# tomasjakab/imm

Hardware: AMD Instinct MI355X
Metric: training images/sec at 128x128 K=10 (higher is better)
Workload: dtype bf16; 1 GPU; BASELINE configs[1] (N>1: configs[2]): CelebA-shape 128x128 K=10 IMM training step (fwd + VGG16 perceptual loss + bwd + clip + Adam), batch 32 per GPU; global_batch=32, image_size=128, n_maps=10, parallelism=dp1, hip_graph=True, weights=seeded random init; synthetic VGG16 (vgg16.caffemodel.h5 unavailable offline)

## Files before the change

### imm_amd/_lib.py

```python
import ctypes as C
import os

import torch

_HERE = os.path.dirname(os.path.abspath(__file__))
LIB_PATH = os.environ.get('IMM_HIP_LIB') or os.path.join(_HERE, 'libimm_hip.so')

IMM_BF16, IMM_F16, IMM_F32 = 0, 1, 2
CONV_BIAS, CONV_RELU, CONV_STATS, CONV_MASK, CONV_OUT_F32 = 1, 2, 4, 8, 16
SSE_BLOCKS = 512
OPTIMIZERS = {'adam': 0, 'adadelta': 1, 'adagrad': 2}
GAUSS_MODES = {'rot': 0, 'flat': 1, 'ankush': 2}
ABI_VERSION = 35


class ImmHipError(RuntimeError):
    pass


class ConvDesc(C.Structure):
    _fields_ = [(n, C.c_int32) for n in (
        'batch', 'hi', 'wi', 'ci', 'ldx', 'ho', 'wo', 'co', 'ldy', 'kh', 'kw', 'stride', 'pad_t', 'pad_l',
        'updiv', 'kpad', 'flags', 'ldmask', 'out_scale', 'out_off_y', 'out_off_x')]


class WgradJob(C.Structure):
    _fields_ = [('desc', ConvDesc), ('x', C.c_void_p), ('dy', C.c_void_p), ('slab', C.c_void_p), ('lddy', C.c_int32),
                ('nsplit', C.c_int32), ('x_scale', C.c_void_p), ('x_shift', C.c_void_p), ('x_relu', C.c_int32),
                ('reserved', C.c_int32)]


class OptHParams(C.Structure):
    _fields_ = [('lr_start', C.c_float), ('lr_decay', C.c_float), ('lr_step', C.c_int32), ('lr_multiple', C.c_float),
                ('beta1', C.c_float), ('beta2', C.c_float), ('eps', C.c_float), ('clip', C.c_float),
                ('grad_scale', C.c_float), ('optim', C.c_int32),
                ('scale_growth_interval', C.c_int32), ('scale_max', C.c_float)]


class KeypointDesc(C.Structure):
    _fields_ = [('w', C.c_void_p), ('b', C.c_void_p), ('geom', C.c_void_p), ('keypoints', C.c_void_p), ('m', C.c_int32),
                ('image_size', C.c_int32)]


_P, _I, _L, _F, _D = C.c_void_p, C.c_int, C.c_int64, C.c_float, C.c_double
ABI = {}


def _header(name, sigs):
    ABI[name] = {n: s if isinstance(s, tuple) else (C.c_int, s) for n, s in sigs.items()}


_header('imm_hip.h', {
    'imm_abi_version': [],
    'imm_last_error': (C.c_char_p, []),
    'imm_source_digest': (C.c_char_p, []),
    'imm_device_info': [_P],
    'imm_set_cu_limit': [_I],
    'imm_get_cu_limit': [],
    'imm_graph_begin': [_P],
    'imm_graph_end': [_P, C.POINTER(C.c_void_p)],
    'imm_graph_launch': [_P, _P],
    'imm_graph_destroy': [_P],
    'imm_pack_weights': [_P, _P, _I, _I, _I, _I, _I, _I, _I, _I, _I, _P],
    'imm_pack_weights_multi': [_P, _P, _I, _I, _I, _P],
    'imm_pack_weights_multi_blocks': [_I, _I, _I],
    'imm_wgrad_reduce_multi': [_P, _P, _I, _I, _P],
    'imm_conv2d': [C.POINTER(ConvDesc), _I, _P, _P, _P, _P, _P, _P, _P],
    'imm_conv_stats_blocks': [C.POINTER(ConvDesc)],
    'imm_conv2d_variant': [C.POINTER(ConvDesc), _I],
    'imm_conv2d_tap_supported': [C.POINTER(ConvDesc)],
    'imm_conv2d_tap': [C.POINTER(ConvDesc), _I, _P, _P, _P, _P, _P, _I, _P, _I, _P, _I, _I, _P],
    'imm_conv2d_wgrad': [C.POINTER(ConvDesc), _I, _P, _P, _I, _P, _I, _P],
    'imm_conv2d_wgrad_splits': [C.POINTER(ConvDesc), _I],
    'imm_conv2d_wgrad_variant': [C.POINTER(ConvDesc), _I, _I, C.POINTER(C.c_int), C.POINTER(C.c_int), C.POINTER(C.c_int)],
    'imm_conv2d_wgrad_multi_plan': [_P, _I, _I, _P],
    'imm_conv2d_wgrad_multi': [_P, _P, _P],
    'imm_conv2d_wgrad_reduce': [_P, _I, _I, _I, _I, _I, _I, _I, _P, _P],
    'imm_colsum': [_P, _I, _L, _I, _I, _I, _P, _P, _P],
    'imm_colsum_blocks': [_L, _I],
    'imm_bn_finalize': [_P, _I, _I, _L, _P, _P, _F, _F, _I, _P, _P, _P, _P, _P, _P, _P],
    'imm_bn_apply_relu': [_P, _I, _L, _I, _I, _P, _P, _I, _P, _I, _P],
    'imm_bn_apply_fused': [_P, _I, _I, _L, _P, _P, _F, _F, _I, _P, _P, _P, _P, _P, _P, _P, _I, _I, _I, _P, _I, _P, _I, _I, _I, _P],
    'imm_bn_bwd_apply_fused': [_P, _I, _I, _L, _P, _P, _I, _P, _I, _I, _P, _P, _P, _P, _I, _P, _P, _P, _I, _P],
    'imm_rows_reduce': [_P, _I, _I, _I, _P, _P],
    'imm_bn_bwd_reduce': [_P, _I, _P, _I, _I, _L, _I, _P, _P, _P, _P, _I, _P, _P],
    'imm_bn_bwd_blocks': [_L, _I],
    'imm_bn_bwd_reduce_up': [_P, _I, _P, _I, _P, _I, _I, _I, _I, _I, _I, _P, _P, _P, _P, _I, _P, _P],
    'imm_bn_bwd_finalize': [_P, _I, _I, _I, _L, _P, _P, _P, _I, _P, _P, _P, _P],
    'imm_bn_bwd_apply': [_P, _I, _P, _I, _I, _L, _I, _P, _P, _P, _P, _I, _P, _P, _I, _P],
    'imm_upsample2x_fwd': [_P, _P, _I, _I, _I, _I, _I, _I, _I, _P],
    'imm_upsample2x_bwd': [_P, _P, _I, _I, _I, _I, _I, _I, _I, _P],
    'imm_resize_ac_fwd': [_P, _P, _I, _I, _I, _I, _I, _I, _I, _I, _I, _P],
    'imm_resize_ac_bwd': [_P, _P, _I, _I, _I, _I, _I, _I, _I, _I, _I, _P],
    'imm_maxpool2_fwd': [_P, _P, _I, _I, _I, _I, _I, _P],
    'imm_maxpool2_bwd': [_P, _P, _P, _I, _I, _I, _I, _I, _I, _P],
    'imm_pack_image': [_P, _P, _I, _L, _P],
    'imm_pack_image_taps': [_P, _P, _I, _I, _I, _I, _I, _I, _I, _P],
    'imm_softargmax_gauss_fwd': [_P, _I, _I, _I, _I, _I, _F, _I, _P, _P, _P, _P, _I, _I, _I, _P],
    'imm_softargmax_gauss_bwd': [_P, _I, _I, _I, _I, _I, _I, _F, _I, _P, _P, _P, _P, _I, _I, _P],
    'imm_gauss_render_f32': [_P, _I, _I, _F, _I, _P, _I, _P],
    'imm_pose_head_fwd': [_P, _I, _I, _P, _I, _P, _I, _I, _I, _I, _I, _F, _I, _P, _I, _P, _P, _P, _P, _I, _I,
                          C.POINTER(KeypointDesc), _P],
    'imm_pose_head_bwd': [_P, _I, _I, _I, _I, _I, _I, _F, _I, _P, _P, _P, _P, _I, _I, _P, _I, _I, _P, _I, _P, _P],
    'imm_vgg_conv1_1_fwd': [_P, _P, _I, _I, _I, _P, _P, _P, _I, _I, _P],
    'imm_vgg_head_supported': [_I, _I, _I],
    'imm_vgg_head_fwd': [_P, _P, _I, _I, _I, _P, _P, _P, _I, _P, _P, _I, _P, _P, _I, _P],
    'imm_vgg_conv1_1_bwd': [_P, _I, _I, _I, _P, _P, _P, _I, _P, _P, _I, _I, _P, _I, _P],
    'imm_image_loss_grad': [_P, _P, _I, _I, _I, _P, _P, _I, _I, _P, _I, _I, _P],
    'imm_copy_f32': [_P, _P, _L, _P],
    'imm_debug_stamp': [_P, _I, _P],
    'imm_tps_warp': [_P, _I, _I, _I, _I, _I, _P, _I, _P, _P, _I, _P, _P, _I, _P],
    'imm_tps_warp_pad': [_P, _I, _I, _I, _I, _I, _I, _I, _I, _I, _I, _I, _I, _I, _P, _I, _P, _P, _I, _P],
    'imm_conv2d_group': [_P, _I, _I, _P, _P, _P, _P, _P, _P],
    'imm_conv_first_supported': [_I, _I, _I, _I],
    'imm_conv_first_stats_blocks': [_I, _I],
    'imm_conv_first': [_P, _P, _I, _P, _P, _I, _P, _I, _I, _I, _I, _I, _P],
    'imm_conv2d_nol_supported': [C.POINTER(ConvDesc)],
    'imm_conv2d_nol_stats_blocks': [C.POINTER(ConvDesc)],
    'imm_conv2d_nol': [C.POINTER(ConvDesc), _I, _P, _P, _P, _I, _P, _P, _P, _P, _P],
    'imm_conv2d_dgrad_s2_supported': [_I, _I, _I, _I, _I, _I],
    'imm_conv2d_dgrad_s2': [_P, _I, _P, _I, _P, _I, _I, _I, _I, _I, _I, _P],
    'imm_conv2d_group_stats_blocks': [_P, _I],
    'imm_upsample2x_bwd_bn': [_P, _P, _I, _I, _I, _I, _I, _I, _I, _P, _I, _P, _P],
    'imm_upsample2x_bwd_bn_blocks': [_I, _I, _I, _I],
    'imm_crc32c': [_P, C.c_uint64, C.POINTER(C.c_uint32)],
    'imm_rccl_unique_id': [_P],
    'imm_rccl_init': [_I, _I, _P, C.POINTER(C.c_void_p)],
    'imm_rccl_allreduce': [_P, _P, _L, _P],
    'imm_rccl_destroy': [_P],
    'imm_resize_crop_u8': [_P, _P, _P, _P, _I, _I, _I, _I, _I, _I, _I, _I, _P, _I, _P],
    'imm_unpool_tap_grad': [_P, _P, _P, _P, _I, _I, _I, _I, _P, _I, _P, _I, _P],
    'imm_masked_sse_pool': [_P, _P, _I, _I, _I, _I, _P, _I, _P, _P, _P, _P],
    'imm_masked_sse_multi': [_I, _P, _P, _P, _P, _P, _I, _I, _P, _I, _I, _P],
    'imm_masked_sse_all': [_I, _P, _P, _P, _P, _P, _I, _I, _P, _I, _I, _P, _I, _P, _I, _I, _P, _P],
    'imm_masked_sse': [_P, _P, _I, _I, _I, _I, _P, _I, _I, _P, _P],
    'imm_masked_sse_f32': [_P, _I, _P, _I, _I, _I, _I, _P, _I, _P, _P],
    'imm_perceptual_finalize': [_P, _I, _P, _P, _I, _P, _I, _I, _P, _P, _P],
    'imm_cost_ema': [_P, _P, _F, _P],
    'imm_rms16': [_P, _L, _I, _P, _I, _P, _P],
    'imm_tap_grad': [_P, _I, _P, _P, _I, _I, _I, _I, _P, _I, _P, _I, _I, _I, _P],
    'imm_weight_decay_loss': [_P, _P, _P, _P, _I, _P, _P, _P, _P],
    'imm_clip_adam_step': [_P, _P, _P, _P, _P, _P, _P, _I, _I, _P, _P, _P, _P, _P, _P, _P, C.POINTER(OptHParams), _P, _P],
    'imm_conv2d_workspace_bytes': (_L, [C.POINTER(ConvDesc)]),
    'imm_conv2d_group_workspace_bytes': (_L, [_P, _I]),
    'imm_conv2d_wgrad_workspace_bytes': (_L, [C.POINTER(ConvDesc), _I, _I]),
    'imm_conv2d_wgrad_multi_table_bytes': (_L, [_I]),
    'imm_colsum_workspace_bytes': (_L, [_L, _I]),
    'imm_bn_bwd_workspace_bytes': (_L, [_L, _I]),
    'imm_upsample2x_bwd_bn_workspace_bytes': (_L, [_I, _I, _I, _I]),
    'imm_masked_sse_workspace_bytes': (_L, [_I]),
    'imm_vgg_head_scratch_bytes': (_L, [_I, _I]),
})

_header('imm_align.h', {
    'imm_align_coeffs': [_P, _P, _I, _I, _I, _P, _P],
    'imm_align_warp_u8': [_P, _I, _P, _P, _I, _P, _P, _P, _P, _I, _I, _I, _I, _P, _I, _P],
})

_header('imm_compose.h', {
    'imm_compose_u8': [_P, _P, _P, _I, _P, _P, _P, _P, _I, _I, _I, _I, _P],
})

_header('imm_unalign.h', {
    'imm_unalign_maps': [_P, _P, _P, _P, _I, _I, _I, _I, _P, _P, _P],
    'imm_unalign_u8': [_P, _P, _P, _I, _P, _P, _P, _P, _F, _P, _I, _I, _I, _I, _P],
})

_header('imm_track.h', {
    'imm_track_step': [_P, _P, _P, _P, _I, _I, _I, _I, _I, _I, _D, _D, _D, _D, _D, _D, _I, _P, _P, _P, _P, _P, _P],
})

_header('imm_retarget.h', {
    'imm_retarget': [_P, _P, _P, _P, _P, _I, _I, _I, _I, _I, _D, _P, _P, _P],
})

_header('imm_warp.h', {
    'imm_warp_fit': [_P, _P, _P, _I, _I, _I, _D, _D, _P, _P, _P, _P],
    'imm_warp_u8': [_P, _P, _P, _P, _I, _P, _P, _P, _P, _P, _I, _I, _I, _P],
})

_header('imm_morph.h', {
    'imm_morph_poses': [_P, _P, _P, _I, _I, _P, _P, _P],
    'imm_morph_u8': [_P, _P, _P, _P, _I, _P, _P, _P, _I, _P, _P, _P, _P, _P, _P, _P, _P, _I, _I, _I, _P],
})

_header('imm_colour.h', {
    'imm_colour_stats_u8': [_P, _P, _P, _I, _P, _I, _I, _P, _P],
    'imm_colour_gain': [_P, _P, _P, _D, _I, _P, _P, _P],
    'imm_morph_colour_u8': [_P, _P, _P, _P, _I, _P, _P, _P, _I, _P, _P, _P, _P, _P, _P, _P, _P, _P, _I, _I, _I, _P],
})

_header('imm_hull.h', {
    'imm_hull_fit': [_P, _P, _P, _I, _I, _P, _P, _P],
    'imm_morph_hull_u8': [_P, _P, _P, _P, _I, _P, _P, _P, _I, _P, _P, _P, _P, _P, _P, _P, _P, _P, _P, _P, _I, _I, _I, _I, _P],
})

_header('imm_seam.h', {
    'imm_seam_fit': [_P, _P, _P, _P, _P, _P, _P, _P, _P, _I, _P, _P, _P, _I, _P, _P, _P, _P, _P, _P, _I, _I, _I, _I, _P, _P, _P, _P],
    'imm_morph_seam_u8': [_P, _P, _P, _P, _I, _P, _P, _P, _I, _P, _P, _P, _P, _P, _P, _P, _P, _P, _P, _P, _P, _P, _P, _I, _I, _I, _I, _I, _P],
})

_header('imm_clip.h', {
    'imm_clip_rows': [_P, _P, _P, _P, _I, _I, _I, _D, _P, _P, _P, _P, _P],
    'imm_clip_ema': [_P, _P, _P, _P, _P, _I, _I, _F, _P],
})

_lib = None


def symbols(header=None):
    return sorted(ABI[header]) if header else sorted(n for block in ABI.values() for n in block)


def signature(name):
    for block in ABI.values():
        if name in block:
            return block[name]
    raise KeyError(name)


def load():
    global _lib
    if _lib is not None:
        return _lib
    if not os.path.exists(LIB_PATH):
        raise ImmHipError('libimm_hip.so not found at %s: build it with `python imm_amd/build.py` '
                          '(there is no CPU fallback for the product path)' % LIB_PATH)
    if 'IMM_HIP_LIB' not in os.environ and os.path.isdir(os.path.join(_HERE, 'csrc')):
        from . import build as _b
        want, have = _b.source_digest(), _b.library_digest(LIB_PATH)
        if want != have:
            if not _b.have_compiler():
                raise ImmHipError('libimm_hip.so is stale (built from sources %s.., checkout is %s..) and hipcc is not '
                                  'available to rebuild it' % (have[:12] or '?', want[:12]))
            _b.build(verbose=False)
    lib = C.CDLL(LIB_PATH)
    for block in ABI.values():
        for name, (restype, argtypes) in block.items():
            fn = getattr(lib, name)
            fn.restype, fn.argtypes = restype, argtypes
    v = lib.imm_abi_version()
    if v != ABI_VERSION:
        raise ImmHipError('libimm_hip.so ABI %d != expected %d' % (v, ABI_VERSION))
    _lib = lib
    return lib


def call(name, *args):
    rc = getattr(load(), name)(*args)
    if rc != 0:
        raise ImmHipError('%s failed (%d): %s' % (name, rc, load().imm_last_error().decode()))
```

### imm_amd/csrc/conv_wgrad.hip

```cpp
#include "common.h"
#include "conv_dispatch.h"
#include "gfx950.h"
#include <stdlib.h>
#include <string.h>

struct WgradArgs {
  const uint16_t* x;
  const uint16_t* dy;
  float* slab;
  int P;
  int hi, wi, ci8, ldx;
  int ho, wo, co, lddy;
  int kh, kw, stride, pad_t, pad_l;
  int kpad, ntaps;
  int n_kblk, n_nblk, nsplit, p_per_split;
  uint32_t x_bytes, dy_bytes;
};

template <int PSUB>
__device__ __forceinline__ int wg_swz(int row) { return PSUB == 1 ? (((row >> 3) & 1) * 3) : (row & (4 * PSUB - 1)); }
template <int PSUB>
__device__ __forceinline__ int wg_dword_idx(int row, int u, int pp) {
  return row * (16 * PSUB) + (((u * 4 + (pp >> 2)) ^ wg_swz<PSUB>(row)) << 2) + (pp & 3);
}
// ... 130 lines not shown
          Bb[wg_dword_idx<PSUB>(row, u, pp)] = (lo[j] & 0xffffu) | (hi[j] << 16);
          Bb[wg_dword_idx<PSUB>(row + 1, u, pp)] = (lo[j] >> 16) | (hi[j] & 0xffff0000u);
        }
      }
    }
  };

  f32x4_t acc[KT_][NT];
#pragma unroll
  for (int i = 0; i < KT_; ++i)
#pragma unroll
    for (int j = 0; j < NT; ++j) acc[i][j] = f32x4_t{0.f, 0.f, 0.f, 0.f};

  const int nsteps = (p_end - p_begin + 32 * PSUB - 1) / (32 * PSUB);
  if (nsteps > 0) {
    load_tile();
    store_tile(0);
  }
  __syncthreads();
  const int frow = lane & 15, fchunk = lane >> 4;
  for (int st = 0; st < nsteps; ++st) {
    const int buf = st & 1;
    const bool more = (st + 1) < nsteps;
    if (more) load_tile();
    const uint4* Ab = smem + buf * BUF;
    const uint4* Bb = Ab + BK * 4 * PSUB;
#pragma unroll
    for (int u = 0; u < PSUB; ++u) {
      uint4 af[KT_], bf[NT];
#pragma unroll
      for (int i = 0; i < KT_; ++i) af[i] = Ab[wg_chunk_idx<PSUB>(wk * TK + i * 16 + frow, u * 4 + fchunk)];
#pragma unroll
      for (int j = 0; j < NT; ++j) bf[j] = Bb[wg_chunk_idx<PSUB>(wn * TN + j * 16 + frow, u * 4 + fchunk)];
#pragma unroll
      for (int i = 0; i < KT_; ++i)
#pragma unroll
        for (int j = 0; j < NT; ++j) acc[i][j] = ET::mfma(bf[j], af[i], acc[i][j]);
    }
    if (more) store_tile(buf ^ 1);
    __syncthreads();
  }

  float* out = a.slab + (int64_t)split * a.kpad * a.co;
#pragma unroll
  for (int i = 0; i < KT_; ++i) {
    const int kk = k0 + wk * TK + i * 16 + (lane & 15);
    if (kk >= a.kpad) continue;
#pragma unroll
    for (int j = 0; j < NT; ++j) {
      const int n = n0 + wn * TN + j * 16 + 4 * (lane >> 4);
      float* op = out + (int64_t)kk * a.co + n;
      if (n + 3 < a.co && (a.co & 3) == 0) {
        *(float4*)op = make_float4(acc[i][j][0], acc[i][j][1], acc[i][j][2], acc[i][j][3]);
      } else {
#pragma unroll
        for (int r = 0; r < 4; ++r) if (n + r < a.co) op[r] = acc[i][j][r];
      }
    }
  }
}

template <typename ET, int BK, int BN, int WGK, int WGN, bool FAST, int PSUB>
static void wg_launch_one(const WgradArgs& a, hipStream_t s) {
  constexpr int lds = 2 * (BK + BN) * 64 * PSUB;
  imm_launch<conv_wgrad_kernel<ET, BK, BN, WGK, WGN, FAST, PSUB>>(dim3(a.n_kblk * a.n_nblk * a.nsplit), dim3(256), lds, s, a);
}

template <typename ET, int BK, int BN, int WGK, int WGN>
static void wg_launch_cfg(const WgradArgs& a, bool fast, int psub, hipStream_t s) {
  if (fast && psub == 4) wg_launch_one<ET, BK, BN, WGK, WGN, true, 4>(a, s);
  else if (fast) wg_launch_one<ET, BK, BN, WGK, WGN, true, 1>(a, s);
  else wg_launch_one<ET, BK, BN, WGK, WGN, false, 1>(a, s);
}

static int wgrad_bn(int co) { return co > 64 ? 128 : co > 32 ? 64 : co > 16 ? 32 : 16; }

template <typename ET>
static int wgrad_launch(const imm_conv_desc* d, const void* x, const void* dy, int lddy, float* slab, int nsplit,
                        hipStream_t s) {
  WgradArgs a;
  a.x = (const uint16_t*)x; a.dy = (const uint16_t*)dy; a.slab = slab;
  a.P = d->batch * d->ho * d->wo;
  a.hi = d->hi; a.wi = d->wi; a.ci8 = d->ci / 8; a.ldx = d->ldx;
  a.ho = d->ho; a.wo = d->wo; a.co = d->co; a.lddy = lddy;
  a.kh = d->kh; a.kw = d->kw; a.stride = d->stride; a.pad_t = d->pad_t; a.pad_l = d->pad_l;
  a.kpad = d->kpad; a.ntaps = d->kh * d->kw;
  const int bn = wgrad_bn(d->co);
  a.n_kblk = (d->kpad + 127) / 128;
  a.n_nblk = (d->co + bn - 1) / bn;
  a.nsplit = nsplit;
  const int hw = d->ho * d->wo;
  const int64_t xb = (int64_t)d->batch * d->hi * d->wi * d->ldx * 2, db = (int64_t)a.P * lddy * 2;
  const bool fast = (hw % 32 == 0) && (d->wo % 32 == 0 || 32 % d->wo == 0) && xb < (1LL << 31) && db < (1LL << 31);
  constexpr int psub_env = 1;
  int pps = (a.P + nsplit - 1) / nsplit;
  const int psub = (fast && psub_env == 4 && a.P % 128 == 0 && pps >= 512 && bn <= 64) ? 4 : 1;
  pps = (pps + 32 * psub - 1) / (32 * psub) * (32 * psub);
  a.p_per_split = pps;
  a.x_bytes = (uint32_t)(fast ? xb : 0);
  a.dy_bytes = (uint32_t)(fast ? db : 0);
  if (bn == 128) wg_launch_cfg<ET, 128, 128, 2, 2>(a, fast, psub, s);
  else if (bn == 64) wg_launch_cfg<ET, 128, 64, 2, 2>(a, fast, psub, s);
  else if (bn == 32) wg_launch_cfg<ET, 128, 32, 4, 1>(a, fast, psub, s);
  else wg_launch_cfg<ET, 128, 16, 4, 1>(a, fast, psub, s);
  IMM_CHECK_LAUNCH("imm_conv2d_wgrad");
  return 0;
}

extern "C" int imm_conv2d_wgrad_splits(const imm_conv_desc* d, int lddy) {
  if (!d) return IMM_E_INVALID;
  return imm_wgrad_halo_applicable(d, lddy) ? imm_wgrad_halo_splits(d, lddy) : 0;
}

enum { WGM_SINGLE = 0, WGM_TR = 1, WGM_HALO = 2 };
static void wgm_classify(const imm_conv_desc* d, int lddy, int dtype, bool halo_ok, int* kind, int* variant) {
  const bool fast_dt = dtype == IMM_BF16 || dtype == IMM_F16;
  const int hv = fast_dt && halo_ok ? imm_wgrad_halo_variant(d, lddy) : 0;
  if (hv) { *kind = WGM_HALO; *variant = hv; return; }
  if (fast_dt && imm_wgrad_tr_applicable(d, lddy)) { *kind = WGM_TR; *variant = imm_wgrad_tr_variant(d); return; }
  *kind = WGM_SINGLE; *variant = 0;
}

extern "C" int imm_conv2d_wgrad(const imm_conv_desc* d, int dtype, const void* x, const void* dy, int lddy,
                                float* slab, int nsplit, void* stream) {
  IMM_REQUIRE(d && x && dy && slab, "wgrad: null");
  IMM_REQUIRE(d->ci > 0 && d->ci % 8 == 0 && d->ldx % 8 == 0 && d->ldx >= d->ci, "wgrad: ci/ldx must be multiples of 8");
  IMM_REQUIRE(lddy % 8 == 0 && lddy >= d->co, "wgrad: lddy=%d must be a multiple of 8 and >= co", lddy);
  IMM_REQUIRE(d->updiv == 1, "wgrad: desc must be the forward convolution");
  IMM_REQUIRE(d->kpad % 32 == 0 && d->kpad >= d->kh * d->kw * d->ci, "wgrad: kpad");
  IMM_REQUIRE(nsplit >= 1, "wgrad: nsplit");
  IMM_REQUIRE(d->wo % 2 == 0, "wgrad: output width must be even (pixel pairs)");
  IMM_REQUIRE(((uintptr_t)x % 16 == 0) && ((uintptr_t)dy % 16 == 0) && ((uintptr_t)slab % 16 == 0), "wgrad: alignment");
  if (dtype == IMM_F32) return imm_conv_f32_wgrad(d, x, dy, lddy, slab, nsplit, (hipStream_t)stream);
  int kind, variant;
  wgm_classify(d, lddy, dtype, nsplit == imm_conv2d_wgrad_splits(d, lddy), &kind, &variant);
  if (kind == WGM_HALO) {
    imm_wgrad_halo_launch(dtype, d, x, dy, lddy, slab, nsplit, (hipStream_t)stream, nullptr, nullptr, 0);
    IMM_CHECK_LAUNCH("imm_conv2d_wgrad(halo)");
    return 0;
  }
  if (kind == WGM_TR) {
    imm_wgrad_tr_launch(dtype, d, x, dy, lddy, slab, nsplit, (hipStream_t)stream);
    IMM_CHECK_LAUNCH("imm_conv2d_wgrad(tr)");
    return 0;
  }
  IMM_DISPATCH_DTYPE(dtype, return wgrad_launch<ET>(d, x, dy, lddy, slab, nsplit, (hipStream_t)stream));
  return 0;
}

namespace {
constexpr uint32_t WGM_MAGIC = 0x57474d31u;
constexpr int WGM_MAX_LAUNCH = 16, WGM_MAX_JOBS = 64, WGM_ARG_STRIDE = 192, WGM_HEADER = 1024;
struct WgmLaunch { int32_t kind, variant, n, arg_off, first_off, blocks, job0, pad; };
struct WgmHeader { uint32_t magic; int32_t dtype, n_jobs, n_launch; WgmLaunch launch[WGM_MAX_LAUNCH]; };
static_assert(sizeof(WgmHeader) <= WGM_HEADER, "header");

int wgm_check_job(const imm_wgrad_job* j) {
  const imm_conv_desc* d = &j->desc;
  IMM_REQUIRE(j->x && j->dy && j->slab, "wgrad_multi: null");
  IMM_REQUIRE(d->ci > 0 && d->ci % 8 == 0 && d->ldx % 8 == 0 && d->ldx >= d->ci, "wgrad_multi: ci/ldx must be multiples of 8");
  IMM_REQUIRE(j->lddy % 8 == 0 && j->lddy >= d->co, "wgrad_multi: lddy=%d must be a multiple of 8 and >= co", j->lddy);
  IMM_REQUIRE(d->updiv == 1 && d->kpad % 32 == 0 && d->kpad >= d->kh * d->kw * d->ci && j->nsplit >= 1 && d->wo % 2 == 0,
              "wgrad_multi: desc");
  IMM_REQUIRE(((uintptr_t)j->x % 16 == 0) && ((uintptr_t)j->dy % 16 == 0) && ((uintptr_t)j->slab % 16 == 0), "wgrad_multi: alignment");
  return 0;
}
}

extern "C" int64_t imm_conv2d_wgrad_multi_table_bytes(int n) {
  if (n < 1 || n > WGM_MAX_JOBS) return IMM_E_INVALID;
  return WGM_HEADER + (int64_t)n * (WGM_ARG_STRIDE + (int64_t)sizeof(imm_wgrad_job)) + WGM_MAX_LAUNCH * (WGM_MAX_JOBS + 1) * 4;
}

extern "C" int imm_conv2d_wgrad_variant(const imm_conv_desc* d, int lddy, int dtype, int* wg_per_split, int* units, int* wg_per_cu) {
  IMM_REQUIRE(d && lddy >= d->co, "wgrad_variant: args");
  int kind, variant;
  wgm_classify(d, lddy, dtype, true, &kind, &variant);
  int wps = 1, un = 1, pcu = 2;
  if (kind == WGM_HALO) {
    wps = imm_wgrad_halo_blocks(d, lddy, &un);
    pcu = imm_wgrad_halo_per_cu(variant);
  } else {
    const int bn = wgrad_bn(d->co);
    wps = ((d->kpad + 127) / 128) * ((d->co + bn - 1) / bn);
    un = (d->batch * d->ho * d->wo + 31) / 32;
  }
  if (wg_per_split) *wg_per_split = wps;
  if (units) *units = un;
  if (wg_per_cu) *wg_per_cu = pcu;
  return kind * 100000 + variant;
}

extern "C" int imm_conv2d_wgrad_multi_plan(const imm_wgrad_job* jobs, int n, int dtype, void* table_host) {
  IMM_REQUIRE(jobs && table_host && n >= 1 && n <= WGM_MAX_JOBS, "wgrad_multi_plan: args");
  IMM_REQUIRE(imm_wgrad_tr_args_bytes() <= WGM_ARG_STRIDE && imm_wgrad_halo_args_bytes() <= WGM_ARG_STRIDE, "wgrad_multi_plan: arg stride");
  char* base = (char*)table_host;
  memset(base, 0, (size_t)imm_conv2d_wgrad_multi_table_bytes(n));
  WgmHeader* h = (WgmHeader*)base;
  h->magic = WGM_MAGIC; h->dtype = dtype; h->n_jobs = n; h->n_launch = 0;
  int kind[WGM_MAX_JOBS], variant[WGM_MAX_JOBS];
  bool done[WGM_MAX_JOBS];
  for (int i = 0; i < n; ++i) {
    if (wgm_check_job(&jobs[i])) return IMM_E_INVALID;
    wgm_classify(&jobs[i].desc, jobs[i].lddy, dtype, true, &kind[i], &variant[i]);
    IMM_REQUIRE((jobs[i].x_scale == nullptr) == (jobs[i].x_shift == nullptr), "wgrad_multi_plan: job %d: x_scale / x_shift come together", i);
    IMM_REQUIRE(jobs[i].x_scale == nullptr || kind[i] == WGM_HALO,
                "wgrad_multi_plan: job %d: normalise-on-load (x_scale) is served by the LDS-halo filter-gradient kernels only "
                "(imm_conv2d_wgrad_variant / 100000 == 2)", i);
    done[i] = false;
  }
  int64_t off = WGM_HEADER;
  int job_slot = 0;
  for (int i = 0; i < n; ++i) {
    if (done[i]) continue;
    IMM_REQUIRE(h->n_launch < WGM_MAX_LAUNCH, "wgrad_multi_plan: more than %d kernel variants", WGM_MAX_LAUNCH);
    WgmLaunch* L = &h->launch[h->n_launch++];
    L->kind = kind[i]; L->variant = variant[i];
    int idx[WGM_MAX_JOBS], m = 0;
    for (int k = i; k < n; ++k)
      if (!done[k] && kind[k] == kind[i] && variant[k] == variant[i] && (kind[i] != WGM_SINGLE || k == i)) { idx[m++] = k; done[k] = true; }
    L->n = m;
    L->arg_off = (int32_t)off;
    if (kind[i] == WGM_SINGLE) {
      memcpy(base + off, &jobs[i], sizeof(imm_wgrad_job));
      off += (int64_t)sizeof(imm_wgrad_job);
      off = (off + 15) / 16 * 16;
      L->first_off = 0; L->blocks = 0; L->job0 = job_slot++;
      continue;
    }
    int steps[WGM_MAX_JOBS], blocks[WGM_MAX_JOBS];
    char tmp[WGM_MAX_JOBS][WGM_ARG_STRIDE];
    for (int k = 0; k < m; ++k) {
      const imm_wgrad_job* j = &jobs[idx[k]];
      blocks[k] = kind[i] == WGM_TR ? imm_wgrad_tr_fill(&j->desc, j->x, j->dy, j->lddy, j->slab, j->nsplit, tmp[k], &steps[k])
                                    : imm_wgrad_halo_fill(&j->desc, j->x, j->dy, j->lddy, j->slab, j->nsplit, tmp[k], &steps[k], j->x_scale,
                                                          j->x_shift, j->x_relu);
    }
    int order[WGM_MAX_JOBS];
    for (int k = 0; k < m; ++k) order[k] = k;
    for (int a = 1; a < m; ++a)
      for (int b = a; b > 0 && steps[order[b]] > steps[order[b - 1]]; --b) { const int t = order[b]; order[b] = order[b - 1]; order[b - 1] = t; }
    const int stride = kind[i] == WGM_TR ? imm_wgrad_tr_args_bytes() : imm_wgrad_halo_args_bytes();
    for (int k = 0; k < m; ++k) memcpy(base + off + (int64_t)k * stride, tmp[order[k]], (size_t)stride);
    off += (int64_t)m * stride;
    off = (off + 15) / 16 * 16;
    L->first_off = (int32_t)off;
    int32_t* first = (int32_t*)(base + off);
    first[0] = 0;
    for (int k = 0; k < m; ++k) first[k + 1] = first[k] + blocks[order[k]];
    L->blocks = first[m];
    off += (int64_t)(m + 1) * 4;
    off = (off + 15) / 16 * 16;
    L->job0 = job_slot; job_slot += m;
  }
  IMM_REQUIRE(off <= imm_conv2d_wgrad_multi_table_bytes(n), "wgrad_multi_plan: table overflow");
  return 0;
}

extern "C" int imm_conv2d_wgrad_multi(const void* table_host, const void* table_dev, void* stream) {
  IMM_REQUIRE(table_host && table_dev, "wgrad_multi: null");
  const char* hb = (const char*)table_host;
  const char* db = (const char*)table_dev;
  const WgmHeader* h = (const WgmHeader*)hb;
  IMM_REQUIRE(h->magic == WGM_MAGIC && h->n_launch >= 1 && h->n_launch <= WGM_MAX_LAUNCH, "wgrad_multi: not a planned table");
  for (int l = 0; l < h->n_launch; ++l) {
    const WgmLaunch* L = &h->launch[l];
    if (L->kind == WGM_SINGLE) {
      const imm_wgrad_job* j = (const imm_wgrad_job*)(hb + L->arg_off);
      const int rc = imm_conv2d_wgrad(&j->desc, h->dtype, j->x, j->dy, j->lddy, j->slab, j->nsplit, stream);
      if (rc) return rc;
    } else if (L->kind == WGM_TR) {
      imm_wgrad_tr_launch_multi(h->dtype, L->variant, db + L->arg_off, (const int*)(db + L->first_off), L->n, L->blocks, (hipStream_t)stream);
    } else {
      imm_wgrad_halo_launch_multi(h->dtype, L->variant, db + L->arg_off, (const int*)(db + L->first_off), L->n, L->blocks, (hipStream_t)stream);
    }
  }
  IMM_CHECK_LAUNCH("imm_conv2d_wgrad_multi");
  return 0;
}

__global__ void wgrad_reduce_kernel(const float* __restrict__ slab, int nsplit, int ntaps, int ci_pad, int ci_real,
                                    int co, int kpad, float* __restrict__ dw) {
  const int64_t total = (int64_t)ntaps * ci_real * co;
  const int64_t sstride = (int64_t)kpad * co;
  for (int64_t idx = (int64_t)blockIdx.x * blockDim.x + threadIdx.x; idx < total;
       idx += (int64_t)gridDim.x * blockDim.x) {
    const int n = (int)(idx % co);
    const int64_t tc = idx / co;
    const int c = (int)(tc % ci_real), tap = (int)(tc / ci_real);
    const float* sp = slab + ((int64_t)tap * ci_pad + c) * co + n;
    float acc = 0.f;
    for (int s = 0; s < nsplit; ++s) acc += sp[s * sstride];
    dw[idx] = acc;
  }
}

extern "C" int imm_conv2d_wgrad_reduce(const float* slab, int nsplit, int kh, int kw, int ci_pad, int ci_real, int co,
                                       int kpad, float* dw, void* stream) {
  IMM_REQUIRE(slab && dw && nsplit >= 1, "wgrad_reduce: args");
  IMM_REQUIRE(ci_real <= ci_pad && kpad >= kh * kw * ci_pad, "wgrad_reduce: padding");
  const int64_t total = (int64_t)kh * kw * ci_real * co;
  const int blocks = (int)((total + 255) / 256 > 2048 ? 2048 : (total + 255) / 256);
  hipLaunchKernelGGL(wgrad_reduce_kernel, dim3(blocks), dim3(256), 0, (hipStream_t)stream, slab, nsplit, kh * kw,
                     ci_pad, ci_real, co, kpad, dw);
  IMM_CHECK_LAUNCH("imm_conv2d_wgrad_reduce");
  return 0;
}
```

### imm_amd/csrc/loss_optim.hip

```cpp
#include "common.h"

#define LO_THREADS 256
#define IMM_NORM2_SANE 1e30f

template <typename ET>
__global__ __launch_bounds__(LO_THREADS) void masked_sse_kernel(const typename ET::T* __restrict__ a, const typename ET::T* __restrict__ b,
                                                                int batch, int s, int c8n, const float* __restrict__ mask,
                                                                int S, int l1, float* __restrict__ partial) {
  __shared__ float red[4];
  const int r = S / s;
  const int64_t total = (int64_t)batch * s * s * c8n;
  float acc = 0.f;
  for (int64_t idx = (int64_t)blockIdx.x * blockDim.x + threadIdx.x; idx < total;
       idx += (int64_t)gridDim.x * blockDim.x) {
    const int64_t p = idx / c8n;
    float mk = 1.f;
    if (mask) {
      const int xx = (int)(p % s);
      const int64_t t = p / s;
      const int yy = (int)(t % s);
      const int64_t bi = t / s;
      mk = mask[(bi * S + (int64_t)yy * r) * S + (int64_t)xx * r];
    }
    float fa[8], fb[8];
// ... 406 lines not shown
  IMM_DISPATCH_DTYPE_F32(dtype, hipLaunchKernelGGL((unpool_tap_grad_kernel<ET>), dim3((int)blocks), dim3(LO_THREADS), 0,
                                               (hipStream_t)stream, (typename ET::T*)da, (const typename ET::T*)dpool,
                                               (const typename ET::T*)a_pred, (const typename ET::T*)a_gt, batch, s, c / 8, mask, S, coef, idx));
  IMM_CHECK_LAUNCH("imm_unpool_tap_grad");
  return 0;
}

extern "C" int imm_tap_grad(void* da, int has_in, const void* a_pred, const void* a_gt, int dtype, int batch, int s, int c,
                            const float* mask, int S, const float* coef, int idx, int relu, int l1, void* stream) {
  IMM_REQUIRE(da && a_pred && a_gt && coef && batch > 0 && s > 0 && c > 0 && c % 8 == 0 && idx >= 0, "tap_grad: args");
  IMM_REQUIRE(mask == nullptr || (S >= s && S % s == 0), "tap_grad: mask side");
  const int64_t total = (int64_t)batch * s * s * (c / 8);
  int64_t blocks = (total + LO_THREADS - 1) / LO_THREADS;
  if (blocks > 16384) blocks = 16384;
  IMM_DISPATCH_DTYPE_F32(dtype, hipLaunchKernelGGL((tap_grad_kernel<ET>), dim3((int)blocks), dim3(LO_THREADS), 0,
                                               (hipStream_t)stream, (typename ET::T*)da, has_in, (const typename ET::T*)a_pred,
                                               (const typename ET::T*)a_gt, batch, s, c / 8, mask, S, coef, idx, relu, l1));
  IMM_CHECK_LAUNCH("imm_tap_grad");
  return 0;
}

template <typename ET>
__global__ void image_loss_grad_kernel(const float* __restrict__ gt, const float* __restrict__ pred, int ldp, int64_t npix,
                                       const float* __restrict__ mask, const float* __restrict__ coef, int idx, int l1,
                                       typename ET::T* __restrict__ dpred, int lddp) {
  const int nvec = lddp / 8;
  const float ck = coef[idx];
  for (int64_t i = (int64_t)blockIdx.x * blockDim.x + threadIdx.x; i < npix * nvec; i += (int64_t)gridDim.x * blockDim.x) {
    const int64_t p = i / nvec;
    const int cg = (int)(i - p * nvec);
    float o[8] = {0.f, 0.f, 0.f, 0.f, 0.f, 0.f, 0.f, 0.f};
    if (cg == 0) {
      const float cm = ck * (mask ? mask[p] : 1.f);
#pragma unroll
      for (int ch = 0; ch < 3; ++ch) {
        float d = pred[p * ldp + ch] - gt[p * 3 + ch];
        if (l1) d = d > 0.f ? 1.f : (d < 0.f ? -1.f : 0.f);
        o[ch] = cm * d;
      }
    }
    st8<ET>(dpred + p * lddp + cg * 8, pack8<ET>(o));
  }
}

extern "C" int imm_image_loss_grad(const float* gt, const float* pred, int ldp, int batch, int s, const float* mask,
                                   const float* coef, int idx, int l1, void* dpred, int lddp, int dtype, void* stream) {
  IMM_REQUIRE(gt && pred && coef && dpred && batch > 0 && s > 0 && ldp >= 3 && idx >= 0, "image_loss_grad: args");
  IMM_REQUIRE(lddp >= 8 && lddp % 8 == 0, "image_loss_grad: lddp=%d must be a multiple of 8", lddp);
  const int64_t npix = (int64_t)batch * s * s;
  int64_t blocks = (npix * (lddp / 8) + LO_THREADS - 1) / LO_THREADS;
  if (blocks > 8192) blocks = 8192;
  IMM_DISPATCH_DTYPE_F32(dtype, hipLaunchKernelGGL((image_loss_grad_kernel<ET>), dim3((int)blocks), dim3(LO_THREADS), 0,
                                               (hipStream_t)stream, gt, pred, ldp, npix, mask, coef, idx, l1,
                                               (typename ET::T*)dpred, lddp));
  IMM_CHECK_LAUNCH("imm_image_loss_grad");
  return 0;
}

__global__ __launch_bounds__(LO_THREADS) void wd_partial_kernel(const float* __restrict__ params,
                                                                const int32_t* __restrict__ blk_seg,
                                                                const int32_t* __restrict__ blk_begin,
                                                                const int32_t* __restrict__ blk_end,
                                                                const float* __restrict__ seg_wd,
                                                                float* __restrict__ blk_partial) {
  __shared__ float red[4];
  const int blk = blockIdx.x;
  const float wd = seg_wd[blk_seg[blk]];
  float acc = 0.f;
  if (wd != 0.f)
    for (int i = blk_begin[blk] + threadIdx.x; i < blk_end[blk]; i += LO_THREADS) { const float w = params[i]; acc += w * w; }
  acc = block_sum_256(acc, red);
  if (threadIdx.x == 0) blk_partial[blk] = 0.5f * wd * acc;
}

__global__ __launch_bounds__(LO_THREADS) void sum_partials_kernel(const float* __restrict__ partial, int n, float* out) {
  __shared__ double dred[LO_THREADS];
  double v = 0.0;
  for (int i = threadIdx.x; i < n; i += LO_THREADS) v += (double)partial[i];
  dred[threadIdx.x] = v;
  __syncthreads();
  for (int o = LO_THREADS / 2; o > 0; o >>= 1) {
    if (threadIdx.x < o) dred[threadIdx.x] += dred[threadIdx.x + o];
    __syncthreads();
  }
  if (threadIdx.x == 0) out[0] = (float)dred[0];
}

extern "C" int imm_weight_decay_loss(const float* params, const int32_t* blk_seg, const int32_t* blk_begin,
                                     const int32_t* blk_end, int nblk, const float* seg_wd, float* blk_partial, float* out,
                                     void* stream) {
  IMM_REQUIRE(params && blk_seg && blk_begin && blk_end && seg_wd && blk_partial && out && nblk > 0, "weight_decay_loss: args");
  hipLaunchKernelGGL(wd_partial_kernel, dim3(nblk), dim3(LO_THREADS), 0, (hipStream_t)stream, params, blk_seg, blk_begin,
                     blk_end, seg_wd, blk_partial);
  hipLaunchKernelGGL(sum_partials_kernel, dim3(1), dim3(LO_THREADS), 0, (hipStream_t)stream, blk_partial, nblk, out);
  IMM_CHECK_LAUNCH("imm_weight_decay_loss");
  return 0;
}

__global__ void cost_ema_kernel(const float* __restrict__ cost3, float* __restrict__ state, float decay) {
  if (threadIdx.x < 3) state[threadIdx.x] = decay * state[threadIdx.x] + (1.f - decay) * cost3[threadIdx.x];
  if (threadIdx.x == 3) state[3] += 1.f;
}

extern "C" int imm_cost_ema(const float* cost3, float* state4, float decay, void* stream) {
  IMM_REQUIRE(cost3 && state4 && decay >= 0.f && decay < 1.f, "cost_ema: args");
  hipLaunchKernelGGL(cost_ema_kernel, dim3(1), dim3(64), 0, (hipStream_t)stream, cost3, state4, decay);
  IMM_CHECK_LAUNCH("imm_cost_ema");
  return 0;
}

template <typename ET>
__global__ __launch_bounds__(LO_THREADS) void sumsq16_kernel(const typename ET::T* __restrict__ x, int64_t n8, float* __restrict__ partial) {
  __shared__ float red[4];
  float acc = 0.f;
  for (int64_t i = (int64_t)blockIdx.x * LO_THREADS + threadIdx.x; i < n8; i += (int64_t)gridDim.x * LO_THREADS) {
    float f[8];
    unpack8<ET>(ld8<ET>(x + i * 8), f);
#pragma unroll
    for (int e = 0; e < 8; ++e) acc = fmaf(f[e], f[e], acc);
  }
  acc = block_sum_256(acc, red);
  if (threadIdx.x == 0) partial[blockIdx.x] = acc;
}

__global__ __launch_bounds__(LO_THREADS) void rms_finish_kernel(const float* __restrict__ partial, int n, double count, float* out) {
  __shared__ double dred[LO_THREADS];
  double v = 0.0;
  for (int i = threadIdx.x; i < n; i += LO_THREADS) v += (double)partial[i];
  dred[threadIdx.x] = v;
  __syncthreads();
  for (int o = LO_THREADS / 2; o > 0; o >>= 1) {
    if (threadIdx.x < o) dred[threadIdx.x] += dred[threadIdx.x + o];
    __syncthreads();
  }
  if (threadIdx.x == 0) out[0] = (float)sqrt(dred[0] / count);
}

extern "C" int imm_rms16(const void* x, int64_t n, int dtype, float* partial, int nblk, float* out, void* stream) {
  IMM_REQUIRE(x && partial && out && n > 0 && n % 8 == 0 && nblk > 0 && nblk <= 4096, "rms16: args (n must be a multiple of 8)");
  IMM_REQUIRE(((uintptr_t)x % 16) == 0, "rms16: 16-byte alignment");
  IMM_DISPATCH_DTYPE_F32(dtype, hipLaunchKernelGGL((sumsq16_kernel<ET>), dim3(nblk), dim3(LO_THREADS), 0, (hipStream_t)stream,
                                              (const typename ET::T*)x, n / 8, partial));
  hipLaunchKernelGGL(rms_finish_kernel, dim3(1), dim3(LO_THREADS), 0, (hipStream_t)stream, partial, nblk, (double)n, out);
  IMM_CHECK_LAUNCH("imm_rms16");
  return 0;
}

__device__ __forceinline__ void opt_learning_rate(const imm_opt_hparams& hp, int gs, int tt, float* lr_t, float* lr) {
  const double l = (double)hp.lr_multiple * (double)hp.lr_start * pow((double)hp.lr_decay, (double)(gs / hp.lr_step));
  *lr_t = (float)(l * sqrt(1.0 - pow((double)hp.beta2, (double)tt)) / (1.0 - pow((double)hp.beta1, (double)tt)));
  *lr = (float)l;
}

__global__ __launch_bounds__(LO_THREADS) void grad_prepare_kernel(const float* __restrict__ params, float* __restrict__ grads,
                                                                  const int32_t* __restrict__ blk_seg,
                                                                  const int32_t* __restrict__ blk_begin,
                                                                  const int32_t* __restrict__ blk_end,
                                                                  const float* __restrict__ seg_wd, float grad_scale,
                                                                  const float* __restrict__ loss_scale,
                                                                  float* __restrict__ blk_partial, int nblk,
                                                                  const int32_t* __restrict__ step_count,
                                                                  const int32_t* __restrict__ adam_t, float* __restrict__ lr_state,
                                                                  imm_opt_hparams hp) {
  __shared__ float red[4];
  const int blk = blockIdx.x;
  if (blk == nblk) {
    if (threadIdx.x == 0) opt_learning_rate(hp, step_count[0], adam_t[0] + 1, lr_state, lr_state + 1);
    return;
  }
  if (loss_scale) grad_scale *= 1.f / loss_scale[0];
  const float wd = seg_wd[blk_seg[blk]];
  float acc = 0.f;
  const int b0 = blk_begin[blk], b1 = blk_end[blk];
  const int a0 = min((b0 + 3) & ~3, b1), a1 = max(a0, b1 & ~3);
  for (int i = b0 + threadIdx.x; i < a0; i += LO_THREADS) {
    const float g = grads[i] * grad_scale + wd * params[i];
    grads[i] = g; acc += g * g;
  }
  for (int i = a0 + 4 * threadIdx.x; i < a1; i += 4 * LO_THREADS) {
    float4 g = *(const float4*)(grads + i);
    const float4 w = *(const float4*)(params + i);
    g.x = g.x * grad_scale + wd * w.x; g.y = g.y * grad_scale + wd * w.y;
    g.z = g.z * grad_scale + wd * w.z; g.w = g.w * grad_scale + wd * w.w;
    *(float4*)(grads + i) = g;
    acc += (g.x * g.x + g.y * g.y) + (g.z * g.z + g.w * g.w);
  }
  for (int i = a1 + threadIdx.x; i < b1; i += LO_THREADS) {
    const float g = grads[i] * grad_scale + wd * params[i];
    grads[i] = g; acc += g * g;
  }
  acc = block_sum_256(acc, red);
  if (threadIdx.x == 0) blk_partial[blk] = acc;
}

__global__ __launch_bounds__(LO_THREADS) void clip_adam_kernel(float* __restrict__ params, const float* __restrict__ grads,
                                                               float* __restrict__ m, float* __restrict__ v,
                                                               const int32_t* __restrict__ blk_seg,
                                                               const int32_t* __restrict__ blk_begin,
                                                               const int32_t* __restrict__ blk_end,
                                                               const int32_t* __restrict__ seg_first_blk,
                                                               const float* __restrict__ blk_partial, int nblk,
                                                               float* __restrict__ seg_norm2, int32_t* __restrict__ step_count,
                                                               int32_t* __restrict__ adam_t, const float* __restrict__ lr_state,
                                                               float* __restrict__ ls, imm_opt_hparams hp) {
  __shared__ double dred[LO_THREADS / 64];
  const int blk = blockIdx.x, tid = threadIdx.x;
  const bool extra = blk == nblk;
  const int seg = extra ? 0 : blk_seg[blk];
  const int b0 = extra ? 0 : blk_begin[blk], b1 = extra ? 0 : blk_end[blk];
  const int a0 = min((b0 + 3) & ~3, b1), a1 = max(a0, b1 & ~3);
  const int i0 = a0 + 4 * tid;
  const bool first = i0 < a1;
  float4 g0 = {0.f, 0.f, 0.f, 0.f}, m0 = g0, v0 = g0, w0 = g0;
  if (first) { g0 = *(const float4*)(grads + i0); m0 = *(const float4*)(m + i0); v0 = *(const float4*)(v + i0); w0 = *(const float4*)(params + i0); }

  const int f0 = seg_first_blk[seg], f1 = seg_first_blk[seg + 1];
  double ps = 0.0;
  int bad = 0;
  const int sb1 = ls != nullptr ? nblk : f1;
  int sb0 = tid;
  if (ls == nullptr && f0 > tid) sb0 = tid + (f0 - tid + LO_THREADS - 1) / LO_THREADS * LO_THREADS;
  for (int b = sb0; b < sb1; b += LO_THREADS) {
    const float p = blk_partial[b];
    bad |= !(p <= IMM_NORM2_SANE);
    if (b >= f0 && b < f1) ps += (double)p;
  }
#pragma unroll
  for (int o = 32; o > 0; o >>= 1) ps += __shfl_xor(ps, o, 64);
  if ((tid & 63) == 0) dred[tid >> 6] = ps;
  bad = __syncthreads_or(bad);
  const bool skip = ls != nullptr && bad != 0;
  double t = 0.0;
#pragma unroll
  for (int w = 0; w < LO_THREADS / 64; ++w) t += dred[w];
  const float norm2 = (float)t;
  if (tid == 0 && !extra && blk == f0) seg_norm2[seg] = norm2;
  if (extra) {
    if (tid == 0) {
      if (ls) {
        float S = ls[0], clean = ls[1];
        if (skip) { S = fmaxf(S * 0.5f, 1.f); clean = 0.f; ls[2] += 1.f; }
        else if (hp.scale_growth_interval > 0 && clean + 1.f >= (float)hp.scale_growth_interval) {
          S = fminf(S * 2.f, hp.scale_max > 0.f ? hp.scale_max : S * 2.f); clean = 0.f;
        } else clean += 1.f;
        ls[0] = S; ls[1] = clean; ls[3] = skip ? 1.f : 0.f;
      }
      if (!skip) {
        step_count[0] += 1;
        adam_t[0] += 1;
      }
    }
    return;
  }
  if (skip) return;
  float factor = 1.f;
  if (hp.clip > 0.f) factor = hp.clip / fmaxf(sqrtf(norm2), hp.clip);
  const float lr_t = lr_state[0], lr = lr_state[1];
  auto one = [&](float g, float& mi, float& vi, float& w) {
    g *= factor;
    if (hp.optim == IMM_OPT_ADAM) {
      mi = hp.beta1 * mi + (1.f - hp.beta1) * g;
      vi = hp.beta2 * vi + (1.f - hp.beta2) * g * g;
      w -= lr_t * mi / (sqrtf(vi) + hp.eps);
    } else if (hp.optim == IMM_OPT_ADADELTA) {
      vi = hp.beta1 * vi + (1.f - hp.beta1) * g * g;
      const float u = sqrtf(mi + hp.eps) / sqrtf(vi + hp.eps) * g;
      mi = hp.beta1 * mi + (1.f - hp.beta1) * u * u;
      w -= lr * u;
    } else {
      vi += g * g;
      w -= lr * g / sqrtf(vi);
    }
  };
  for (int i = b0 + tid; i < a0; i += LO_THREADS) one(grads[i], m[i], v[i], params[i]);
  if (first) {
    one(g0.x, m0.x, v0.x, w0.x); one(g0.y, m0.y, v0.y, w0.y); one(g0.z, m0.z, v0.z, w0.z); one(g0.w, m0.w, v0.w, w0.w);
    *(float4*)(m + i0) = m0; *(float4*)(v + i0) = v0; *(float4*)(params + i0) = w0;
  }
  for (int i = i0 + 4 * LO_THREADS; i < a1; i += 4 * LO_THREADS) {
    const float4 g = *(const float4*)(grads + i);
    float4 mi = *(const float4*)(m + i), vi = *(const float4*)(v + i), w = *(const float4*)(params + i);
    one(g.x, mi.x, vi.x, w.x); one(g.y, mi.y, vi.y, w.y); one(g.z, mi.z, vi.z, w.z); one(g.w, mi.w, vi.w, w.w);
    *(float4*)(m + i) = mi; *(float4*)(v + i) = vi; *(float4*)(params + i) = w;
  }
  for (int i = a1 + tid; i < b1; i += LO_THREADS) one(grads[i], m[i], v[i], params[i]);
}

extern "C" int imm_clip_adam_step(float* params, float* grads, float* m, float* v, const int32_t* blk_seg,
                                  const int32_t* blk_begin, const int32_t* blk_end, int nblk, int nseg,
                                  const int32_t* seg_first_blk, const float* seg_wd, float* blk_partial, float* seg_norm2,
                                  int32_t* step_count, int32_t* adam_t, float* lr_state, const imm_opt_hparams* hp,
                                  float* loss_scale_state, void* stream) {
  IMM_REQUIRE(params && grads && m && v && blk_seg && blk_begin && blk_end && seg_first_blk && seg_wd && blk_partial &&
                  seg_norm2 && step_count && adam_t && lr_state && hp, "clip_adam_step: null");
  IMM_REQUIRE(nblk > 0 && nseg > 0 && hp->lr_step > 0, "clip_adam_step: dims");
  IMM_REQUIRE(hp->optim >= IMM_OPT_ADAM && hp->optim <= IMM_OPT_ADAGRAD, "clip_adam_step: optim %d", hp->optim);
  hipStream_t s = (hipStream_t)stream;
  hipLaunchKernelGGL(grad_prepare_kernel, dim3(nblk + 1), dim3(LO_THREADS), 0, s, params, grads, blk_seg, blk_begin, blk_end,
                     seg_wd, hp->grad_scale, loss_scale_state, blk_partial, nblk, step_count, adam_t, lr_state, *hp);
  hipLaunchKernelGGL(clip_adam_kernel, dim3(nblk + 1), dim3(LO_THREADS), 0, s, params, grads, m, v, blk_seg, blk_begin, blk_end,
                     seg_first_blk, blk_partial, nblk, seg_norm2, step_count, adam_t, lr_state, loss_scale_state, *hp);
  IMM_CHECK_LAUNCH("imm_clip_adam_step");
  return 0;
}
```

### imm_amd/engine.py

```python
import math
import os
from collections import OrderedDict

import numpy as np
import torch

from . import _lib as L
from . import ops

BN_EPS = 1e-3
BN_MOMENTUM = 0.99
BN_DIRECT_ROWS = int(os.environ.get('IMM_BN_DIRECT_ROWS', '512'))
WEIGHT_DECAY = 1e-5
INIT_STD = 0.01
PERCEPTUAL_WS = [100.0, 1.6, 2.3, 1.8, 2.8, 100.0]
SUPPORTED_COMP = ['input', 'conv1_2', 'conv2_2', 'conv3_2', 'conv4_2', 'conv5_2']
VGG_LAYERS = [('conv1_1', 1, 64), ('conv1_2', 64, 64), ('conv2_1', 64, 128), ('conv2_2', 128, 128),
              ('conv3_1', 128, 256), ('conv3_2', 256, 256), ('conv3_3', 256, 256),
              ('conv4_1', 256, 512), ('conv4_2', 512, 512), ('conv4_3', 512, 512),
              ('conv5_1', 512, 512), ('conv5_2', 512, 512)]
VGG_POOL_AFTER = ('conv1_2', 'conv2_2', 'conv3_3', 'conv4_3')
WGRAD_MULTI_MAX_JOBS, WGRAD_MULTI_MAX_VARIANTS = 64, 16


def plan_wgrad_chunks(groups, max_jobs, max_slots):
    chunks, cur, cur_jobs, cur_slots = [], [], 0, 0
    for gk, members in groups.items():
        generic = gk[0] // 100000 == 0
        members = list(members)
        while members:
            room_jobs, room_slots = max_jobs - cur_jobs, max_slots - cur_slots
            take = min(len(members), room_jobs, room_slots) if generic else (min(len(members), room_jobs) if room_slots >= 1 else 0)
            if take <= 0:
                chunks.append(cur); cur, cur_jobs, cur_slots = [], 0, 0
                continue
            part, members = members[:take], members[take:]
            cur.append((gk, part)); cur_jobs += len(part); cur_slots += len(part) if generic else 1
    if cur:
        chunks.append(cur)
    return chunks
COST_EMA_STATE = 'summaries/cost_movavg'
VGG_TAPS = {'conv1_2': 1, 'conv2_2': 2, 'conv3_2': 3, 'conv4_2': 4, 'conv5_2': 5}


def encoder_spec(n_filters):
    f = n_filters
    return [(7, 3, f, 1), (3, f, f, 1), (3, f, 2 * f, 2), (3, 2 * f, 2 * f, 1), (3, 2 * f, 4 * f, 2),
            (3, 4 * f, 4 * f, 1), (3, 4 * f, 8 * f, 2), (3, 8 * f, 8 * f, 1)]


def renderer_spec(cfg, image_size, n_out):
    filters = cfg.n_filters_render * 8
    cin = cfg.n_filters * 8 + cfg.n_maps
    size, spec = 16, []
    while size <= image_size:
        spec.append((3, cin, filters, True, False))
        if size == image_size:
            spec.append((3, filters, n_out, False, False))
            break
        spec.append((3, filters, filters, True, True))
        cin = filters
        size *= 2
        if filters >= 8:
            filters //= 2
    return spec


def render_sizes(cfg, max_size):
    sizes, size = [], max_size
    while True:
        sizes.append(size)
        if size <= cfg.min_res:
            break
        size = size // cfg.renderer_stride
    return sizes


def n_renderer_out(cfg):
    extra = len(cfg.perceptual.comp) if getattr(cfg, 'channels_bug_fix', False) else 0
    return 3 + extra


def trainable_spec(cfg, image_size):
    out = []

    def add(scope, k, cin, cout, bn):
        out.append((scope + '/w', (k, k, cin, cout), WEIGHT_DECAY))
        out.append((scope + '/b', (cout,), 0.0))
        if bn:
            out.append((scope + '/gamma', (cout,), 0.0))
            out.append((scope + '/beta', (cout,), 0.0))

    for enc in ('image_encoder', 'pose_encoder'):
        for i, (k, ci, co, _s) in enumerate(encoder_spec(cfg.n_filters)):
            add('model/%s/encoder/conv_%d' % (enc, i + 1), k, ci, co, True)
        if enc == 'pose_encoder':
            add('model/pose_encoder/conv_1', 1, cfg.n_filters * 8, cfg.n_maps, False)
    for i, (k, ci, co, bn, _u) in enumerate(renderer_spec(cfg, image_size, n_renderer_out(cfg))):
        add('model/renderer/conv_%d' % (i + 1), k, ci, co, bn)
    return out


def truncated_normal(rng, shape, std):
    z = rng.standard_normal(shape)
    bad = np.abs(z) > 2.0
    while bad.any():
        z[bad] = rng.standard_normal(int(bad.sum()))
        bad = np.abs(z) > 2.0
    return (z * std).astype(np.float32)


def synthetic_vgg_weights(seed=2):
    rng = np.random.default_rng(seed)
    w = OrderedDict()
    for name, cin, cout in VGG_LAYERS:
        w['vgg16/%s/weights' % name] = torch.from_numpy(
            (rng.standard_normal((3, 3, cin, cout)) * math.sqrt(2.0 / (9 * cin))).astype(np.float32))
        w['vgg16/%s/biases' % name] = torch.from_numpy((rng.standard_normal(cout) * 0.1).astype(np.float32))
    return w


class _Launch:
    __slots__ = ('fn', 'tag', 'flops', 'bytes', 'name', 'lane', 'variant', 'cus', 'group')

    def __init__(self, fn, tag, flops=0.0, nbytes=0.0, name='', lane=0, variant='', cus=0, group=''):
        self.fn, self.tag, self.flops, self.bytes, self.name, self.lane, self.variant = fn, tag, flops, nbytes, name, lane, variant
        self.cus, self.group = cus, group


class _ConvLayer:
    pass


class IMMEngine:
    def __init__(self, cfg, batch, image_size, device='cuda:0', act_dtype=torch.bfloat16, seed=1, vgg_weights=None,
                 hparams=None, world_size=1, dp_buckets=None):
        if cfg.gauss_mode not in L.GAUSS_MODES:
            raise ValueError('Unknown mode: ' + str(cfg.gauss_mode))
        if cfg.reconstruction_loss not in ('perceptual', 'l2'):
            raise ValueError('Reconsutruction loss-type: ' + str(cfg.reconstruction_loss) + ' not understood')
        self.loss_kind = cfg.reconstruction_loss
        self.comp = list(cfg.perceptual.comp) if self.loss_kind == 'perceptual' else ['input']
        if self.loss_kind == 'perceptual':
            if not self.comp or len(set(self.comp)) != len(self.comp) or len(self.comp) > len(PERCEPTUAL_WS):
                raise ValueError('perceptual.comp must name 1..%d distinct features, got %r' % (len(PERCEPTUAL_WS), self.comp))
            if any(n not in SUPPORTED_COMP for n in self.comp):
                raise NotImplementedError('perceptual.comp entries must come from %r (the layers the shipped configs tap), got %r'
                                          % (SUPPORTED_COMP, self.comp))
        self.l1 = self.loss_kind == 'perceptual' and not cfg.perceptual.l2
        if image_size % 16 or image_size < 64:
            raise ValueError('image side must be a multiple of 16 and >= 64')
        L.load()
        self.cfg, self.B, self.S, self.dev, self.dt = cfg, int(batch), int(image_size), torch.device(device), act_dtype
        self.f32 = act_dtype == torch.float32
        self.K = int(cfg.n_maps)
        self.world_size = world_size
        self.dp_buckets = int(dp_buckets if dp_buckets is not None else os.environ.get('IMM_DP_BUCKETS', '1'))
        self.use_mask = bool(cfg.loss_mask)
        self.n_cu, self.arch = ops.device_info()
        self._alloc_bytes = 0

        self.spec = trainable_spec(cfg, self.S)
        sizes = [int(np.prod(s)) for _n, s, _w in self.spec]
        self.tab = ops.SegmentTable(sizes, [w for _n, _s, w in self.spec], self.dev)
        self.params = self._zeros(self.tab.total)
        self.grads = self._zeros(self.tab.total)
        self.adam_m = self._zeros(self.tab.total)
        self.adam_v = self._zeros(self.tab.total)
        self.pview, self.gview = OrderedDict(), OrderedDict()
        for i, (name, shape, _wd) in enumerate(self.spec):
            o0, o1 = self.tab.offsets[i], self.tab.offsets[i + 1]
            self.pview[name] = self.params[o0:o1].view(shape)
            self.gview[name] = self.grads[o0:o1].view(shape)
        self.opt_blk_partial = self._zeros(self.tab.nblk)
        self.seg_norm2 = self._zeros(self.tab.nseg)
# ... 246 lines not shown
        if needs_dgrad:
            assert kw == k
            lddy = ldy if not out_f32 else ops.round_up(co, 32)
            lay.lddy = lddy
            lay.dd = None
            rows_d = ops.round_up(ci_real, 128)
            lay.s2 = ops.dgrad_s2_class_descs(B, H, W, ci_real, 0, lddy, lddy, k) if stride == 2 else None
            lay.s2_fused = (lay.s2 is not None and k == 3 and lddy % 64 == 0 and ci_real % 8 == 0 and not self.f32 and
                            ops.conv2d_dgrad_s2_supported(B, fd.ho, fd.wo, lddy, ci_real, ci_real))
            if lay.s2 is not None and not lay.s2_fused:
                lay.wt_s2 = []
                for dd, mode in lay.s2:
                    wt_c = self._zeros(rows_d, dd.kpad, dtype=dt)
                    lay.wt_s2.append(wt_c)
                    self._pack_jobs.append(((w.data_ptr(), wt_c.data_ptr(), mode, k, k, ci_real, co, lddy, rows_d, dd.kpad),
                                            rows_d * dd.kpad))
                lay.wt_d = None
            else:
                kpad_d = ops.round_up(k * k * lddy, 32)
                lay.wt_d = self._zeros(rows_d, kpad_d, dtype=dt)
                self._pack_jobs.append(((w.data_ptr(), lay.wt_d.data_ptr(), 1, k, k, ci_real, co, lddy, rows_d, kpad_d),
                                        rows_d * kpad_d))
        else:
            lay.lddy = ldy if not out_f32 else ops.round_up(co, 32)
        if bn:
            lay.coef = self._zeros(3, co)
            lay.dy = self._act(B, fd.ho, fd.wo, ldy)
        else:
            lay.cs_partial = self._zeros(ops.colsum_blocks(npix, lay.lddy), lay.lddy)
        return lay

    def _conv_backward(self, lay, d_out, ldd, dx, lddx, up_src=None):
        B, co, k = self.B, lay.co, lay.k
        npix = lay.npix
        scope = lay.scope
        self._cur_scope = scope
        gw, gb = self.gview[scope + '/w'], self.gview[scope + '/b']
        if lay.bn:
            gg, gbeta = self.gview[scope + '/gamma'], self.gview[scope + '/beta']
            gamma, beta = self.pview[scope + '/gamma'], self.pview[scope + '/beta']
            nblk = ops.bn_bwd_blocks(npix, co)
            lay.bwd_partial = self._zeros(nblk, 2, co)
            if up_src is not None:
                self._add(self.prog_bwd, lambda: ops.bn_bwd_reduce_up(up_src[0], up_src[1], d_out, ldd, lay.y, lay.ldy, B, lay.Ho, lay.Wo,
                                                                      co, lay.scale, lay.shift, lay.mean, lay.rstd, lay.relu,
                                                                      lay.bwd_partial), 'bn_bwd_reduce', 0.0, npix * co * 12.0)
            else:
                self._add(self.prog_bwd, lambda: ops.bn_bwd_reduce(d_out, ldd, lay.y, lay.ldy, npix, co, lay.scale, lay.shift,
                                                                   lay.mean, lay.rstd, lay.relu, lay.bwd_partial),
                          'bn_bwd_reduce', 0.0, npix * co * 4.0)
            if co % 32 == 0:
                rows, nrows = lay.bwd_partial, nblk
                if nblk > BN_DIRECT_ROWS:
                    g = max(32, -(-nblk // 32))
                    nrows = -(-nblk // g)
                    lay.bwd_red = rows_red = self._zeros(nrows, 2, co)
                    self._add(self.prog_bwd, lambda: ops.rows_reduce(lay.bwd_partial, nblk, 2 * co, g, rows_red), 'bn_bwd_finalize')
                    rows = rows_red
                self._add(self.prog_bwd, lambda: ops.bn_bwd_apply_fused(rows, nrows, co, npix, gamma, d_out, ldd,
                                                                        lay.y, lay.ldy, lay.scale, lay.shift, lay.mean, lay.rstd,
                                                                        lay.relu, gg, gbeta, lay.dy, lay.ldy),
                          'bn_bwd_apply', 0.0, npix * co * 6.0)
            else:
                self._add(self.prog_bwd, lambda: ops.bn_bwd_finalize(lay.bwd_partial, nblk, co, npix, gamma, beta, lay.rstd,
                                                                     gg, gbeta, lay.coef), 'bn_bwd_finalize')
                self._add(self.prog_bwd, lambda: ops.bn_bwd_apply(d_out, ldd, lay.y, lay.ldy, npix, co, lay.scale, lay.shift,
                                                                  lay.mean, lay.rstd, lay.relu, lay.coef, lay.dy, lay.ldy),
                          'bn_bwd_apply', 0.0, npix * co * 6.0)
            dy, lddy = lay.dy, lay.ldy
        else:
            dy, lddy = d_out, ldd
            self._colsum_pending.append((scope, lambda: ops.colsum(dy, npix, lddy, co, lddy, lay.cs_partial, gb)))
        fd = lay.fd
        flops = 2.0 * npix * k * lay.kw * lay.ci_real * co
        self._wgrad_pending.append((lay, dy, lddy, flops))
        if lay.needs_dgrad and dx is not None and getattr(lay, 's2_fused', False):
            assert lddx % 8 == 0 and lddx >= lay.ci_real, (lddx, lay.ci_real)
            self._add(self.prog_bwd, lambda: ops.conv2d_dgrad_s2(dy, lddy, lay.wt_d, dx, lddx, lay.ci_real, B, lay.Ho, lay.Wo),
                      'conv_dgrad', flops, 2.0 * (npix * lddy + 4 * npix * lay.ci_real + 9 * lddy * lay.ci_real), variant='s2d')
        elif lay.needs_dgrad and dx is not None and getattr(lay, 's2', None) is not None:
            classes = ops.dgrad_s2_class_descs(B, lay.H, lay.W, lay.ci_real, lddx, lddy, lddy, k)
            grp = ops.ConvGroup([dd0 for dd0, _m in classes], list(lay.wt_s2))
            ntaps = sum(dd0.kh * dd0.kw for dd0, _m in classes)
            self._add(self.prog_bwd, (lambda grp=grp: ops.conv2d_group(grp, dy, dx, None, None)), 'conv_dgrad',
                      2.0 * npix * ntaps * lay.ci_real * co,
                      2.0 * (4 * npix * lddy + 4 * npix * lay.ci_real + sum(dd0.kpad for dd0, _m in classes) * lay.ci_real), variant='group')
        elif lay.needs_dgrad and dx is not None:
            co_dx = lay.ci_pad if (lay.ci_pad != lay.ci_real and lay.ci_pad % 64 == 0 and lddx >= lay.ci_pad
                                   and lay.wt_d.shape[0] >= lay.ci_pad) else lay.ci_real
            dd = ops.dgrad_desc(B, lay.H, lay.W, co_dx, lddx, lddy, lddy, k, lay.stride, 0)
            assert dd.kpad == lay.wt_d.shape[1], (dd.kpad, lay.wt_d.shape)
            self._add(self.prog_bwd, lambda: ops.conv2d(dd, dy, lay.wt_d, None, dx), 'conv_dgrad', flops,
                      2.0 * (npix * lddy + B * lay.H * lay.W * lay.ci_real + dd.kpad * lay.ci_real), desc=dd)

    def _flush_wgrads(self, name, cus=0):
        jobs, self._wgrad_pending = self._wgrad_pending, []
        if not jobs:
            return
        groups = OrderedDict()
        for lay, dy, lddy, flops in jobs:
            key, wps, units, pcu = ops.conv2d_wgrad_variant(lay.fd, lddy, self.dt)
            groups.setdefault((key, pcu), []).append((lay, dy, lddy, wps, units, flops))
        chunks = plan_wgrad_chunks(groups, WGRAD_MULTI_MAX_JOBS, WGRAD_MULTI_MAX_VARIANTS)
        for ci_, chunk in enumerate(chunks):
            self._issue_wgrad_chunk(chunk, name if len(chunks) == 1 else '%s [%d/%d]' % (name, ci_ + 1, len(chunks)), cus)

    def _issue_wgrad_chunk(self, chunk, name, cus=0):
        n_lanes = int(os.environ.get('IMM_WG_LANES', '1'))
        if n_lanes > 1 and len(chunk) > 1 and not cus and self._cur_lane == 0:
            share = float(os.environ.get('IMM_WG_LANE_SHARE', '1.0'))
            groups = sorted(chunk, key=lambda g: -sum(m[5] for m in g[1]))
            lanes = sorted(set(1 + (i - 1) % (n_lanes - 1) for i in range(1, len(groups))))
            for ln in lanes:
                self._mark(self.prog_bwd, 'fork', lane=ln)
            for i, g in enumerate(groups):
                self._cur_lane = 0 if i == 0 else 1 + (i - 1) % (n_lanes - 1)
                self._issue_wgrad_chunk([g], '%s [variant %d]' % (name, g[0][0]),
                                        cus=0 if i == 0 else max(8, int(self.n_cu * share) // 8 * 8) if share < 1.0 else 0)
            self._cur_lane = 0
            for ln in lanes:
                self._mark(self.prog_bwd, 'join', lane=ln)
            return
        multi_jobs, flops_total = [], 0.0
        for (key, pcu), members in chunk:
            kind = key // 100000
            target = pcu * (cus or self.n_cu)
            floor_units = [16 if kind != 2 else (2 if wps > 1 else 4) for _l, _d, _ld, wps, _u, _f in members]

            def splits(u):
                return [max(1, min(-(-units // u), max(1, units // fl))) for (_l, _d, _ld, _w, units, _f), fl in zip(members, floor_units)]
            if kind == 0:
                ns = [max(1, min(-(-target // wps), max(1, units // 16))) for _l, _d, _ld, wps, units, _f in members]
            else:
                u = max(units for _l, _d, _ld, _w, units, _f in members)
                ns = splits(u)
                while u > 1:
                    u2 = max(1, int(u / 1.05)) if u > 64 else u - 1
                    ns2 = splits(u2)
                    if sum(n * m[3] for n, m in zip(ns2, members)) > target:
                        break
                    u, ns = u2, ns2
            for (lay, dy, lddy, wps, units, flops), nsplit in zip(members, ns):
                lay.nsplit = nsplit
                flops_total += flops
                lay.slab = self._zeros(nsplit, lay.fd.kpad, lay.co)
                ns_ = getattr(lay, 'nol_src', None)
                multi_jobs.append((lay.fd, lay.x, dy, lddy, lay.slab, nsplit,
                                   None if ns_ is None else (ns_.scale, ns_.shift, ns_.relu)))
                gw = self.gview[lay.scope + '/w']
                job = (lay.slab.data_ptr(), gw.data_ptr(), nsplit, lay.k * lay.kw, lay.ci_pad, lay.ci_real, lay.co, lay.fd.kpad)
                self._reduce_jobs.append((job, lay.k * lay.kw * lay.ci_real * lay.co))
        multi = ops.WgradMulti(multi_jobs, self.dt)
        self._wgrad_multis = getattr(self, '_wgrad_multis', []) + [multi]
        self._cur_scope = name
        self._add(self.prog_bwd, lambda: ops.conv2d_wgrad_multi(multi), 'conv_wgrad', flops_total, name=name)

    def _build_network(self):
        cfg, B, S, K, dt = self.cfg, self.B, self.S, self.K, self.dt
        nf = cfg.n_filters
        self.in_image = self._zeros(B, S, S, 3)
        self.in_future = self._zeros(B, S, S, 3)
        self.in_mask = self._zeros(B, S, S) if self.use_mask else None
        sizes = render_sizes(cfg, S)
        s16 = sizes[-1]
        if s16 != 16:
            raise NotImplementedError('renderer starts at 16x16 (min_res 16, renderer_stride 2): got %d' % s16)
        He = S // 8
        Cj = ops.round_up(8 * nf + K, 64)
        self.Cj, self.He = Cj, He
        self.joint = self._act(B, 16, 16, Cj)
        self.d_joint = self._act(B, 16, 16, Cj)

        def build_encoder(scope, src):
            k1 = encoder_spec(nf)[0][0]
            ld1 = ops.round_up(3 * k1, 32)
            xin = self._act(B, S, S, ld1)
            f_pack = (lambda: ops.pack_image_taps(src, xin, B, S, S, k1, (k1 - 1) // 2, ld1), 'pack_image',
                      0.0, B * S * S * (12.0 + 2.0 * ld1), scope + '/pack')
            co1 = encoder_spec(nf)[0][2]
            direct = (os.environ.get('IMM_CONV_FIRST', '0') != '0' and not self.f32 and k1 == 7 and ld1 == 32 and
                      ops.conv_first_supported(B, S, co1, ops.round_up(co1, 8)))
            if direct:
                self._deferred_packs.append(f_pack)
            else:
                self._add(self.prog_fwd, f_pack[0], f_pack[1], f_pack[2], f_pack[3], name=f_pack[4])
            layers, x, H, ci_real, ci_pad, ldx = [], xin, S, 3 * k1, ld1, ld1
            spec = encoder_spec(nf)
            hs, h_ = [], S
            for (_k, _ci, _co, st) in spec:
                hs.append(h_); h_ = -(-h_ // st)
            defer = [i + 1 < len(spec) and self._nol_consumer_ok(hs[i + 1], hs[i + 1], spec[i][2], ops.round_up(spec[i][2], 8),
                                                               spec[i + 1][2], spec[i + 1][0], spec[i + 1][3], True, False)
                     for i in range(len(spec))]
            prev = None
            for i, (k, ci, co, stride) in enumerate(spec):
                last = i == len(spec) - 1
                out, ldo = (None, None)
                if last and scope == 'model/image_encoder' and He == 16:
                    out, ldo = self.joint, Cj
                nol_src = prev if (prev is not None and getattr(prev, 'nol', False)) else None
                lay = self._conv_block('%s/encoder/conv_%d' % (scope, i + 1), x, H, H, ci_real, ci_pad, ldx, co, k,
                                       stride, True, True, needs_dgrad=(i > 0), out=out, ldo=ldo, kw=(1 if i == 0 else None),
                                       nol_src=nol_src, defer_apply=defer[i], first_src=(src if (i == 0 and direct) else None))
                layers.append(lay)
                prev = lay
                if lay.nol:
                    x, H, ci_real, ci_pad, ldx = lay.y, lay.Ho, co, co, lay.ldy
                else:
                    x, H, ci_real, ci_pad, ldx = lay.out, lay.Ho, co, co, lay.ldo
            return layers

        self._deferred_packs = []
        self._mark(self.prog_fwd, 'fork')
        self._cur_lane = 1
        self._add(self.prog_fwd, lambda: ops.weight_decay_loss(self.params, self.tab, self.opt_blk_partial, self.wd_loss),
                  'wd_loss', name='loss/weight_decay')
        self.enc_im = build_encoder('model/image_encoder', self.in_image)
        if He != 16:
            e = self.enc_im[-1]
            self._add(self.prog_fwd, lambda: ops.resize_ac_fwd(e.out, self.joint, B, He, He, 16, 16, 8 * nf, e.ldo, Cj),
                      'resize_ac')
        self._cur_lane = 0
        self.enc_pose = build_encoder('model/pose_encoder', self.in_future)
        pe = self.enc_pose[-1]
        lddy_h = ops.round_up(K, 32)
        self.fused_head = (not self.f32 and (8 * nf) % 32 == 0 and K <= 64 and (He * He) % 16 == 0 and lddy_h in (32, 64) and
                           4 * (He * He * K + 2 * He * K + 2 * K) <= 158 * 1024 and
                           4 * ((2 + 2 * He) * K + 516) + He * He * lddy_h * 2 <= 158 * 1024)
        self.pose_head = self._conv_block('model/pose_encoder/conv_1', pe.out, He, He, 8 * nf, 8 * nf, pe.ldo, K, 1, 1,
                                          False, False, needs_dgrad=True, out_f32=True, fwd_launch=not self.fused_head)
        ph = self.pose_head
        assert ph.lddy == lddy_h
        self.heat, self.ldh = ph.y, ph.ldy
        self.mu = self._zeros(B, K, 2)
        self.py = self._zeros(B, He, K)
        self.px = self._zeros(B, He, K)
        self.inv_std = 1.0 / float(cfg.gauss_std)
        gview = self.joint[..., 8 * nf:]
        if self.fused_head:
            bias_h = self.pview['model/pose_encoder/conv_1/b']
            self._add(self.prog_fwd, lambda: ops.pose_head_fwd(pe.out, pe.ldo, 8 * nf, ph.wt, bias_h, B, He, He, K, self.inv_std, 16,
                                                               self.heat, self.ldh, self.mu, self.py, self.px, gview, Cj, dt,
                                                               cfg.gauss_mode), 'bottleneck', ph.fwd_flops)
        else:
            self._add(self.prog_fwd, lambda: ops.softargmax_gauss_fwd(self.heat, self.ldh, B, He, He, K, self.inv_std, 16,
                                                                      self.mu, self.py, self.px, gview, Cj, dt, cfg.gauss_mode), 'bottleneck')

        if self._deferred_packs:
            self._cur_lane = 1
            for fn, tag, fl, nb, nm in self._deferred_packs:
                self._cur_scope = nm
                self._add(self.prog_fwd, fn, tag, fl, nb, name=nm)
            self._cur_lane = 0
        self._mark(self.prog_fwd, 'join')
        self.ren, self.ren_up = [], []
        x, H, ci_real, ci_pad, ldx = self.joint, 16, 8 * nf + K, Cj, Cj
        rspec = renderer_spec(cfg, S, n_renderer_out(cfg))
        prev = None
        for i, (k, ci, co, bn, up) in enumerate(rspec):
            assert ci == ci_real, (ci, ci_real)
            defer = False
            if bn and not up and i + 1 < len(rspec) and co % 8 == 0:
                k2, _ci2, co2, bn2, _up2 = rspec[i + 1]
                defer = self._nol_consumer_ok(H, H, co, co, co2, k2, 1, bn2, not bn2)
            nol_src = prev if (prev is not None and prev.bn and getattr(prev, 'nol', False)) else None
            lay = self._conv_block('model/renderer/conv_%d' % (i + 1), x, H, H, ci_real, ci_pad, ldx, co, k, 1, bn, bn,
                                   needs_dgrad=True, out_f32=not bn, up2x=bool(up and bn), nol_src=nol_src, defer_apply=defer)
            self.ren.append(lay)
            prev = lay
            if lay.bn and lay.nol:
                x, ci_real, ci_pad, ldx = lay.y, co, co, lay.ldy
            else:
                x, ci_real, ci_pad, ldx = lay.out, co, co, (lay.ldo if lay.out is not None else co)
            if up:
                ub = getattr(lay, 'up', None)
                if ub is None:
                    ub = self._act(B, 2 * H, 2 * H, co)
                    src = lay.out
                    assert src is not None, 'up-sampling pass without a stored normalised tensor'

                    self._add(self.prog_fwd, (lambda src=src, ub=ub, H=H, co=co: ops.upsample2x_fwd(src, ub, B, H, H, co, co, co)),
                              'upsample', 0.0, B * H * H * co * 10.0)
                self.ren_up.append((len(self.ren) - 1, ub, H, co))
                x, H = ub, 2 * H
        self.pred = self.ren[-1].y
        self.ldp = self.ren[-1].ldy

        self.n_fwd_model = len(self.prog_fwd)

        self.vgg_act, self.vgg_wt, self.vgg_wtd, self.vgg_desc = OrderedDict(), {}, {}, {}
        self.vgg_pool = {}
        self.tap_idx = {n: k for k, n in enumerate(self.comp)}
        vnames = [n for n, _ci, _co in VGG_LAYERS]
        taps = [n for n in self.comp if n != 'input'] if self.loss_kind == 'perceptual' else []
        self.vgg_layers = VGG_LAYERS[:max(vnames.index(n) for n in taps) + 1] if taps else []
        nfeat = self.nfeat
        self.sse_partial = self._zeros(nfeat, L.SSE_BLOCKS)
        fuse_ok = not self.l1
        fused_sse = set()
        self._sse_input_early = ('input' in self.tap_idx and bool(self.vgg_layers) and
                                 os.environ.get('IMM_SSE_INPUT_LANE', '0') != '0')
        if self._sse_input_early:
            idx0 = self.tap_idx['input']
            self._cur_scope = 'loss'
            self._mark(self.prog_fwd, 'fork', lane=1)
            self._cur_lane = 1
            self._add(self.prog_fwd, lambda: ops.masked_sse_f32(self.in_future, 3, self.pred, self.ldp, B, S, 3, self.in_mask,
                                                                self.sse_partial[idx0], self.l1), 'sse')
            self._cur_lane = 0
        split = bool(self.vgg_layers) and os.environ.get('IMM_VGG_SPLIT', '0') != '0'
        self.vgg_split = split
        self.gt_cus = int(os.environ.get('IMM_GT_CUS', '128')) if split else 0
        halves = ([('gt', slice(0, B), 2, self.gt_cus), ('pred', slice(B, 2 * B), 0, 0)] if split else
                  [('', slice(0, 2 * B), 0, 0)])
        gt_prog = []
        for hname, hs, lane, cus in halves:
            if not self.vgg_layers:
                break
            prog = gt_prog if hname == 'gt' else self.prog_fwd
            self._cur_lane, self._cur_cus, self._cur_group = lane, cus, ('gt' if hname == 'gt' else '')
            sfx = ' [%s]' % hname if hname else ''
            nb = hs.stop - hs.start
            if hname != 'pred':
                self.w11 = self._zeros(9, 64); self.b11 = self._zeros(64)
                a = self._act(2 * B, S, S, 64)
                self.vgg_act['conv1_1'] = (a, S)
            a = self.vgg_act['conv1_1'][0]
            hv = {'': 3, 'gt': 1, 'pred': 2}[hname]
            head_fused = (not split and len(self.vgg_layers) > 1 and not self.f32 and os.environ.get('IMM_VGG_HEAD', '1') != '0'
                          and ops.vgg_head_supported(B, S, dt))
            self.vgg_head_fused = head_fused
            if head_fused:
                self.vgg_gray = torch.empty(ops.vgg_head_scratch_bytes(B, S), dtype=torch.uint8, device=self.dev)
            else:
                self._add(prog, (lambda a=a, hv=hv: ops.vgg_conv1_1_fwd(self.in_future, self.pred, self.ldp, B, S, self.w11, self.b11, a, hv)),
                          'vgg_conv1_1', 2.0 * nb * S * S * 9 * 64, nb * S * S * 128.0, name='vgg16/conv1_1' + sfx)
            x, H = a, S
            for li, (name, cin, cout) in enumerate(self.vgg_layers[1:], start=1):
                fd = ops.fwd_desc(nb, H, H, cin, cin, cout, cout, 3, 1, L.CONV_BIAS | L.CONV_RELU)
                if hname != 'pred':
                    wt = self._zeros(ops.round_up(cout, 128), fd.kpad, dtype=dt)
                    wtd = self._zeros(ops.round_up(cin, 128), ops.round_up(9 * cout, 32), dtype=dt)
                    y = self._act(2 * B, H, H, cout)
                    self.vgg_wt[name], self.vgg_wtd[name], self.vgg_desc[name] = wt, wtd, fd
                    self.vgg_act[name] = (y, H)
                wt, y = self.vgg_wt[name], self.vgg_act[name][0]
                bias = self.vgg_w['vgg16/%s/biases' % name]
                if li == 1 and head_fused:
                    self._add(prog, (lambda a=a, wt=wt, bias=bias, y=y: ops.vgg_head_fwd(
                        self.in_future, self.pred, self.ldp, B, S, self.w11, self.b11, wt, bias, a, B, y, self.vgg_gray)),
                              'vgg_fwd', 2.0 * nb * S * S * 9 * (64 + cin * cout),
                              nb * S * S * 12.0 + 2.0 * (B * S * S * 64 + nb * S * S * cout + 9 * cin * cout),
                              name='vgg16/conv1_1+' + name, variant='vgg_head')
                else:
                    self._add(prog, (lambda fd=fd, x=x, wt=wt, bias=bias, y=y, hs=hs: ops.conv2d(fd, x[hs], wt, bias, y[hs])),
                              'vgg_fwd', 2.0 * nb * H * H * 9 * cin * cout, 2.0 * (nb * H * H * (cin + cout) + 9 * cin * cout),
                              name='vgg16/' + name + sfx, desc=fd)
                if hname == 'gt' and name in taps:
                    self._signal(prog, 'gt:' + name)
                x = y
                if name in VGG_POOL_AFTER and li < len(self.vgg_layers) - 1:
                    if hname != 'pred':
                        self.vgg_pool[name] = self._act(2 * B, H // 2, H // 2, cout)
                    p = self.vgg_pool[name]
                    if name in taps and fuse_ok and hname != 'gt':
                        idx = self.tap_idx[name]
                        fused_sse.add(name)
                        if hname == 'pred':
                            self._wait(prog, 'gt:' + name, lane=0)
                        pa = None if hname == 'pred' else p[:B]
                        self._add(prog, (lambda x=x, p=p, pa=pa, H=H, cout=cout, idx=idx: ops.masked_sse_pool(
                            x[:B], x[B:], B, H, cout, self.in_mask, S, self.sse_partial[idx], pa, p[B:])), 'sse',
                                  0.0, 2 * B * H * H * cout * 2.5, name='vgg16/%s+pool' % name)
                    else:
                        self._add(prog, (lambda x=x, p=p, H=H, cout=cout, hs=hs, nb=nb: ops.maxpool2_fwd(x[hs], p[hs], nb, H, H, cout)),
                                  'maxpool', 0.0, nb * H * H * cout * 2.5, name='vgg16/pool_' + name + sfx)
                    x, H = p, H // 2
        self._cur_lane, self._cur_cus, self._cur_group = 0, 0, ''
        if gt_prog:
            self._cur_group = 'gt'
            head = []
            self._mark(head, 'fork', lane=2)
            self._cur_group = ''
            self.prog_fwd[0:0] = head + gt_prog
            self.n_fwd_model += len(head) + len(gt_prog)
        if self.vgg_layers:
            self._pack_vgg()

        nel = []
        for name in self.comp:
            if name == 'input':
                nel.append(float(B * S * S * 3))
            else:
                y, H = self.vgg_act[name]
                nel.append(float(B * H * H * y.shape[-1]))
        self.nel = torch.tensor(nel, dtype=torch.float32, device=self.dev)
        self.loss_out = self._zeros(3 * nfeat + 3)
        self.cost_ema = self._zeros(4)
        mask = self.in_mask
        l1 = self.l1
        self._cur_scope = 'loss'
        if self._sse_input_early:
            self._mark(self.prog_fwd, 'join', lane=1)
        tail = [name for name in taps if name not in fused_sse]
        sse_all = ('input' in self.tap_idx and not self._sse_input_early and len(tail) > 1 and
                   os.environ.get('IMM_SSE_ALL', '1') != '0')
        if 'input' in self.tap_idx and not self._sse_input_early and not sse_all:
            idx0 = self.tap_idx['input']
            self._add(self.prog_fwd, lambda: ops.masked_sse_f32(self.in_future, 3, self.pred, self.ldp, B, S, 3, mask,
                                                                self.sse_partial[idx0], l1), 'sse')
        if self.vgg_split:
            self._cur_group = 'gt'
            self._mark(self.prog_fwd, 'join', lane=2)
            self._cur_group = ''
        if len(tail) > 1:
            feats = []
            for name in tail:
                y, H = self.vgg_act[name]
                feats.append((y[:B], y[B:], H, y.shape[-1], self.sse_partial[self.tap_idx[name]]))
            self.sse_multi = ops.SseMulti(feats)
            if sse_all:
                idx0 = self.tap_idx['input']
                self._add(self.prog_fwd, lambda: ops.masked_sse_all(self.sse_multi, B, mask, S, self.in_future, 3, self.pred, self.ldp, 3,
                                                                    self.sse_partial[idx0], l1), 'sse', 0.0,
                          sum(2 * B * f[2] * f[2] * f[3] * 2.0 for f in feats) + B * S * S * (3 + self.ldp + 1) * 4.0)
            else:
                self._add(self.prog_fwd, lambda: ops.masked_sse_multi(self.sse_multi, B, mask, S, l1), 'sse', 0.0,
                          sum(2 * B * f[2] * f[2] * f[3] * 2.0 for f in feats))
            tail = []
        for name in tail:
            idx = self.tap_idx[name]
            y, H = self.vgg_act[name]
            c = y.shape[-1]
            self._add(self.prog_fwd, (lambda y=y, H=H, c=c, idx=idx: ops.masked_sse(y[:B], y[B:], B, H, c, mask, S,
                                                                                  self.sse_partial[idx], l1)), 'sse',
                      0.0, 2 * B * H * H * c * 2.0)
        mode = ops.LOSS_L2 if self.loss_kind == 'l2' else ops.LOSS_PERCEPTUAL
        self._add(self.prog_fwd, lambda: ops.perceptual_finalize(self.sse_partial, nfeat, self.nel, self.loss_agg,
                                                                 self._training, self.wd_loss, self.loss_out, l1, mode,
                                                                 self.loss_scale_state), 'loss_finalize')
        self.coef = self.loss_out[2 * nfeat:3 * nfeat]

        self._build_backward()
        self.pack_tab = ops.pack_table([j for j, _n in self._pack_jobs], self.dev)
        self._add(self.prog_pack, lambda: ops.pack_weights_multi(self.pack_tab, dt), 'pack')

        self._add(self.prog_opt, lambda: ops.clip_adam_step(self.params, self.grads, self.adam_m, self.adam_v, self.tab,
                                                            self.opt_blk_partial, self.seg_norm2, self.step_count,
                                                            self.adam_t, self.lr_state, self.hp, self.loss_scale_state),
                  'clip_adam', 0.0, self.tab.total * 36.0)
        self.prog_opt.extend(self.prog_pack)

    def _pack_vgg(self):
        if not self.vgg_layers:
            return
        w = self.vgg_w
        self.w11.copy_(w['vgg16/conv1_1/weights'].reshape(9, 64))
        self.b11.copy_(w['vgg16/conv1_1/biases'])
        for name, cin, cout in self.vgg_layers[1:]:
            fd = self.vgg_desc[name]
            wm = w['vgg16/%s/weights' % name]
            ops.pack_weights(wm, self.vgg_wt[name], 0, 3, 3, cin, cout, cin, self.vgg_wt[name].shape[0], fd.kpad)
            wtd = self.vgg_wtd[name]
            ops.pack_weights(wm, wtd, 1, 3, 3, cin, cout, cout, wtd.shape[0], wtd.shape[1])

    def _build_backward(self):
        B, S, K, dt, Cj = self.B, self.S, self.K, self.dt, self.Cj
        mask = self.in_mask
        acts = self.vgg_act
        l1 = self.l1
        names = [n for n, _ci, _co in self.vgg_layers]
        taps = self.tap_idx
        dbuf = {n: self._act(B, acts[n][1], acts[n][1], acts[n][0].shape[-1]) for n in names}
        dpool = {n: self._act(B, acts[n][1] // 2, acts[n][1] // 2, acts[n][0].shape[-1]) for n in self.vgg_pool}

        def pred_half(t):
            return t[B:]

        def tap(name, has_in):
            y, H = acts[name]
            c = y.shape[-1]
            self._add(self.prog_bwd, lambda: ops.tap_grad(dbuf[name], has_in, y[B:], y[:B], B, H, c, mask, S, self.coef,
                                                          taps[name], True, l1), 'tap_grad', 0.0, B * H * H * c * 8.0)

        fused_taps = set()

        def dgrad(name, dst, mask_ref, tap_of=None):
            cin, cout = [(ci, co) for n, ci, co in VGG_LAYERS if n == name][0]
            H = acts[name][1]
            wtd = self.vgg_wtd[name]
            src = dbuf[name]
            flops = 2.0 * B * H * H * 9 * cin * cout
            if tap_of is not None:
                dt0 = ops.dgrad_desc(B, H, H, cin, cin, cout, cout, 3, 1, 0)
                if not self.f32 and ops.conv2d_tap_supported(dt0):
                    ya = acts[tap_of][0]
                    self._add(self.prog_bwd, lambda: ops.conv2d_tap(dt0, src, wtd, dst, ya[B:], ya[:B], cin, mask, S, self.coef,
                                                                    taps[tap_of], l1), 'vgg_dgrad', flops,
                              2.0 * (B * H * H * (3 * cin + cout) + 9 * cin * cout), name='vgg16/%s+tap(%s)' % (name, tap_of), desc=dt0)
                    fused_taps.add(tap_of)
                    return
            flags = L.CONV_MASK if mask_ref is not None else 0
            dd = ops.dgrad_desc(B, H, H, cin, cin, cout, cout, 3, 1, flags, ldmask=cin)
            self._add(self.prog_bwd, lambda: ops.conv2d(dd, src, wtd, None, dst, None, mask_ref), 'vgg_dgrad', flops,
                      2.0 * (B * H * H * (cin + cout + (cin if mask_ref is not None else 0)) + 9 * cin * cout), name='vgg16/' + name,
                      desc=dd)

        def unpool(src_name, dy, relu_mask):
            y, H = acts[src_name]
            c = y.shape[-1]
            self._add(self.prog_bwd, lambda: ops.maxpool2_bwd(y[B:], dy, dbuf[src_name], B, H, H, c, relu_mask), 'maxpool_bwd',
                      0.0, B * H * H * c * 5.0)

        def unpool_tap(name, dy):
            if l1:
                unpool(name, dy, 0); tap(name, True)
                return
            y, H = acts[name]
            c = y.shape[-1]
            self._add(self.prog_bwd, lambda: ops.unpool_tap_grad(dbuf[name], dy, y[B:], y[:B], B, H, c, mask, S, self.coef,
                                                                 taps[name]), 'tap_grad', 0.0, B * H * H * c * 8.5)

        for i in range(len(names) - 1, 0, -1):
            name, prev = names[i], names[i - 1]
            deepest = i == len(names) - 1
            if name in self.vgg_pool:
                if name in taps:
                    unpool_tap(name, dpool[name])
                else:
                    unpool(name, dpool[name], 1)
            elif name in taps and name not in fused_taps:
                tap(name, not deepest)
            if prev in self.vgg_pool:
                dgrad(name, dpool[prev], None)
            elif prev in taps:
                dgrad(name, dbuf[prev], None, tap_of=prev)
            else:
                dgrad(name, dbuf[prev], pred_half(acts[prev][0]))
        last = self.ren[-1]
        self.d_pred = self._act(B, S, S, last.lddy)
        in_idx = taps.get('input', -1)
        if names:
            self._add(self.prog_bwd, lambda: ops.vgg_conv1_1_bwd(dbuf['conv1_1'], B, S, self.w11, self.in_future, self.pred,
                                                                 self.ldp, mask, self.coef, self.d_pred, last.lddy, in_idx, l1),
                      'vgg_conv1_1_bwd', 2.0 * B * S * S * 9 * 64)
        else:
            self._add(self.prog_bwd, lambda: ops.image_loss_grad(self.in_future, self.pred, self.ldp, B, S, mask, self.coef, in_idx,
                                                                 self.d_pred, last.lddy, l1), 'image_loss_grad')

        ups = {idx: (ub, H, co) for idx, ub, H, co in self.ren_up}
        d_out, ldd = self.d_pred, last.lddy
        up_src = None
        for i in range(len(self.ren) - 1, -1, -1):
            lay = self.ren[i]
            if i == 0:
                dx, lddx = self.d_joint, Cj
            else:
                prev = self.ren[i - 1]
                if (i - 1) in ups:
                    _ub, Hp, cp = ups[i - 1]
                    dx, lddx = self._act(B, 2 * Hp, 2 * Hp, cp), cp
                else:
                    dx, lddx = self._act(B, prev.Ho, prev.Wo, prev.co), prev.co
            self._conv_backward(lay, d_out, ldd, dx, lddx, up_src=up_src)
            up_src = None
            if i > 0:
                if (i - 1) in ups:
                    _ub, Hp, cp = ups[i - 1]
                    d_prev = self._act(B, Hp, Hp, cp)
                    if prev.bn:
                        up_src = (dx, lddx)
                    else:
                        self._add(self.prog_bwd, (lambda dx=dx, d_prev=d_prev, Hp=Hp, cp=cp:
                                                  ops.upsample2x_bwd(dx, d_prev, B, Hp, Hp, cp, cp, cp)), 'upsample_bwd',
                                  0.0, B * Hp * Hp * cp * 10.0)
                    d_out, ldd = d_prev, cp
                else:
                    d_out, ldd = dx, lddx

        self.n_bwd_bucket0 = None
        if self.dp_buckets >= 2:
            for scope, fn in self._colsum_pending:
                self._add(self.prog_bwd, fn, 'colsum', name=scope)
            self._colsum_pending = []
            self._flush_wgrads('renderer')
            self.reduce_tab_ren = ops.reduce_table([j for j, _n in self._reduce_jobs], [n for _j, n in self._reduce_jobs], self.dev)
            self._add(self.prog_bwd, lambda: ops.wgrad_reduce_multi(self.reduce_tab_ren), 'wgrad_reduce', name='renderer')
            self._reduce_jobs = []
            self.n_bwd_bucket0 = len(self.prog_bwd)
        self.wg_cus = int(os.environ.get('IMM_WG_CUS', '0')) if self.dp_buckets < 2 else 0
        if self.wg_cus:
            self._mark(self.prog_bwd, 'fork', lane=2)
            self._cur_lane = 2
            self._flush_wgrads('renderer', cus=self.wg_cus)
            self.reduce_tab_ren = ops.reduce_table([j for j, _n in self._reduce_jobs], [n for _j, n in self._reduce_jobs], self.dev)
            self._add(self.prog_bwd, lambda: ops.wgrad_reduce_multi(self.reduce_tab_ren), 'wgrad_reduce', name='renderer')
            self._reduce_jobs = []
            self._cur_lane = 0
        self.bucket0_offset = self.tab.offsets[[n for n, _s, _w in self.spec].index('model/renderer/conv_1/w')]
        self._mark(self.prog_bwd, 'fork')
        nf8 = 8 * self.cfg.n_filters
        He = self.He
        ph = self.pose_head
        self.d_heat = self._act(B, He, He, ph.lddy)
        dg = self.d_joint[..., nf8:]
        d_feat = self._act(B, He, He, nf8)
        self._colsum_needs_dheat = False
        if self.fused_head:
            self.head_bias_partial = self._zeros(B, K)
            flops_h = 2.0 * B * He * He * nf8 * K
            self._add(self.prog_bwd, lambda: ops.pose_head_bwd(dg, Cj, B, He, He, K, self.inv_std, 16, self.mu, self.py, self.px,
                                                               self.d_heat, ph.lddy, ph.wt_d, nf8, d_feat, nf8,
                                                               self.head_bias_partial, self.cfg.gauss_mode), 'bottleneck_bwd', flops_h)
            self._wgrad_pending.append((ph, self.d_heat, ph.lddy, flops_h))
            gb_h = self.gview['model/pose_encoder/conv_1/b']
            self._reduce_jobs.append(((self.head_bias_partial.data_ptr(), gb_h.data_ptr(), B, 1, 1, 1, K, 1), K))
        else:
            self._add(self.prog_bwd, lambda: ops.softargmax_gauss_bwd(dg, Cj, B, He, He, K, self.inv_std, 16, self.mu, self.py,
                                                                      self.px, self.d_heat, ph.lddy, self.cfg.gauss_mode), 'bottleneck_bwd')
            if self.two_streams:
                self._signal(self.prog_bwd, 'd_heat', lane=0)
                self._colsum_needs_dheat = True
            self._conv_backward(ph, self.d_heat, ph.lddy, d_feat, nf8)
        self._encoder_backward(self.enc_pose, d_feat, nf8)

        self._cur_lane = 1
        self._cur_scope = 'loss'
        self._add(self.prog_bwd, lambda: ops.cost_ema(self.loss_out[3 * self.nfeat:], self.cost_ema, 0.99), 'cost_ema')
        if He == 16:
            self._encoder_backward(self.enc_im, self.d_joint, Cj)
        else:
            e = self.enc_im[-1]
            d_e = self._act(B, He, He, nf8)
            self._add(self.prog_bwd, lambda: ops.resize_ac_bwd(self.d_joint, d_e, B, He, He, 16, 16, nf8, Cj, nf8), 'resize_ac_bwd')
            self._encoder_backward(self.enc_im, d_e, nf8)
        if self._colsum_needs_dheat:
            self._wait(self.prog_bwd, 'd_heat', lane=1)
        for scope, fn in self._colsum_pending:
            self._add(self.prog_bwd, fn, 'colsum', name=scope)
        self._colsum_pending = []
        self._cur_lane = 0
        self._mark(self.prog_bwd, 'join')
        if self.wg_cus:
            self._mark(self.prog_bwd, 'join', lane=2)
        self._flush_wgrads('encoders' if (self.n_bwd_bucket0 is not None or self.wg_cus) else 'all layers')
        if self._reduce_jobs:
            self.reduce_tab = ops.reduce_table([j for j, _n in self._reduce_jobs], [n for _j, n in self._reduce_jobs], self.dev)
            self._add(self.prog_bwd, lambda: ops.wgrad_reduce_multi(self.reduce_tab), 'wgrad_reduce',
                      name='encoders' if (self.n_bwd_bucket0 is not None or self.wg_cus) else 'all layers')

    def _encoder_backward(self, layers, d_out, ldd):
        B = self.B
        for i in range(len(layers) - 1, -1, -1):
            lay = layers[i]
            if i > 0:
                prev = layers[i - 1]
                dx, lddx = self._act(B, prev.Ho, prev.Wo, prev.co), prev.co
            else:
                dx, lddx = None, 0
            self._conv_backward(lay, d_out, ldd, dx, lddx)
            d_out, ldd = dx, lddx

    def run(self, prog):
        if not self.two_streams:
            for l in prog:
                if l.fn is not None:
                    self._issue(l)
            return
        main = torch.cuda.current_stream(self.dev)
        streams = {0: main}
        events = {}
        joined = {0}

        def lane_stream(i):
            if i not in streams:
                streams[i] = self._side_stream(i)
            return streams[i]
        pname = ('fwd' if prog is self.prog_fwd else 'opt' if (prog is self.prog_opt or not prog) else
                 'bwd' if (prog is self.prog_bwd or prog[0] is self.prog_bwd[0]) else
                 'bwd2' if prog[-1] is self.prog_bwd[-1] else 'opt')
        if self._stamp_mode and prog is self.prog_fwd:
            self._stamp_names = []

        def stamp(lane, label):
            if not self._stamp_mode or len(self._stamp_names) >= self._stamp_buf.numel():
                return
            with torch.cuda.stream(lane_stream(lane)):
                ops.debug_stamp(self._stamp_buf, len(self._stamp_names))
            self._stamp_names.append((lane, '%s:%s' % (pname, label)))
        stamp(0, 'start')
        for l in prog:
            if l.fn is not None and l.tag in self._skip_tags:
                continue
            if l.fn is not None:
                if l.lane == 0:
                    self._issue(l)
                else:
                    with torch.cuda.stream(lane_stream(l.lane)):
                        self._issue(l)
                if self._stamp_mode == 'all':
                    stamp(l.lane, '%s %s' % (l.tag, l.name))
            elif l.tag == 'fork':
                stamp(0, 'fork' if l.lane == 1 else 'fork%d' % l.lane)
                ev = torch.cuda.Event(); ev.record(main); lane_stream(l.lane).wait_event(ev)
                stamp(l.lane, 'fork: lane %d released' % l.lane)
            elif l.tag == 'join':
                stamp(l.lane, 'join: lane %d done' % l.lane)
                stamp(0, 'join: lane 0 arrives' if l.lane == 1 else 'join%d: lane 0 arrives' % l.lane)
                ev = torch.cuda.Event(); ev.record(lane_stream(l.lane)); main.wait_event(ev)
                stamp(0, 'join: lane 0 resumes' if l.lane == 1 else 'join%d: lane 0 resumes' % l.lane)
            elif l.tag.startswith('record:'):
                stamp(l.lane, l.tag)
                ev = torch.cuda.Event(); ev.record(lane_stream(l.lane)); events[l.tag[7:]] = ev
            elif l.tag.startswith('wait:'):
                stamp(l.lane, l.tag + ' arrives')
                lane_stream(l.lane).wait_event(events[l.tag[5:]])
                stamp(l.lane, l.tag + ' resumes')
        stamp(0, 'end')

    @staticmethod
    def _issue(l):
        if l.cus:
            ops.set_cu_limit(l.cus)
            try:
                l.fn()
            finally:
                ops.set_cu_limit(0)
        else:
            l.fn()

    def stamp_report(self):
        torch.cuda.synchronize(self.dev)
        t = self._stamp_buf[:len(self._stamp_names)].cpu().tolist()
        return [((v - t[0]) / 100.0, lane, label) for v, (lane, label) in zip(t, self._stamp_names)]

    def _side_stream(self, i=1):
        if self._side is None:
            self._side = {}
        if i not in self._side:
            self._side[i] = torch.cuda.Stream(device=self.dev)
        return self._side[i]

    def run_timed(self, prog):
        evs = []
        for l in prog:
            if l.fn is None:
                continue
            e0, e1 = torch.cuda.Event(enable_timing=True), torch.cuda.Event(enable_timing=True)
            e0.record()
            self._issue(l)
            e1.record()
            evs.append((l, e0, e1))
        torch.cuda.synchronize()
        self.last_variants = [l.variant for l, _e0, _e1 in evs]
        return [(l.tag, e0.elapsed_time(e1), l.flops, l.bytes, l.name) for l, e0, e1 in evs]

    def set_inputs(self, image, future_image, mask=None):
        if getattr(self, '_stager', None) is None:
            self._stager = ops.PinnedStager()
        self._stager.copy(self.in_image, image, 'image')
        self._stager.copy(self.in_future, future_image, 'future_image')
        if self.use_mask:
            if mask is None:
                raise RuntimeError('No loss mask recieved but is required.')
            self._stager.copy(self.in_mask, mask, 'mask')

    def forward(self, training=True):
        self._training = bool(training)
        self.run(self.prog_fwd)

    def forward_model_only(self, training=False):
        self._training = bool(training)
        self.run([l for l in self.prog_fwd[:self.n_fwd_model] if l.group != 'gt'])

    def backward(self):
        self.run(self.prog_bwd)

    def snapshot(self):
        return {'params': self.params.clone(), 'm': self.adam_m.clone(), 'v': self.adam_v.clone(),
                'step': self.step_count.clone(), 'adam_t': self.adam_t.clone(), 'agg': self.loss_agg.clone(), 'grads': self.grads.clone(), 'cost_ema': self.cost_ema.clone(),
                'state': {k: v.clone() for k, v in self.state.items()},
                'loss_scale': None if self.loss_scale_state is None else self.loss_scale_state.clone()}

    def restore(self, snap):
        self.params.copy_(snap['params']); self.adam_m.copy_(snap['m']); self.adam_v.copy_(snap['v'])
        self.step_count.copy_(snap['step']); self.adam_t.copy_(snap['adam_t']); self.loss_agg.copy_(snap['agg']); self.grads.copy_(snap['grads']); self.cost_ema.copy_(snap['cost_ema'])
        for k, v in snap['state'].items():
            self.state[k].copy_(v)
        if self.loss_scale_state is not None:
            self.loss_scale_state.copy_(snap['loss_scale'])
        self.run(self.prog_pack)

    def optimizer_step(self):
        self.run(self.prog_opt)

    @property
    def loss(self):
        return self.loss_out[3 * self.nfeat + 2]

    @property
    def loss_terms(self):
        return self.loss_out[:self.nfeat]

    @property
    def loss_scale(self):
        return 1.0 if self.loss_scale_state is None else float(self.loss_scale_state[0])

    def cost_summaries(self):
        raw = [float(v) for v in self.loss_out[3 * self.nfeat:3 * self.nfeat + 3]]
        ema = [float(v) for v in self.cost_ema]
        out = {}
        for i, name in enumerate(('reconstruction_loss', 'weights_loss', 'loss_total')):
            out[name + '_raw'] = raw[i]
            out[name + '_avg'] = ema[i]
        return out

    def vgg_activations(self):
        if getattr(self, 'vgg_head_fused', False) and 'conv1_1' in self.vgg_act:
            a = self.vgg_act['conv1_1'][0]
            ops.vgg_conv1_1_fwd(self.in_future, self.pred, self.ldp, self.B, self.S, self.w11, self.b11, a, 1)
        return self.vgg_act

    def vgg_activation_rms(self):
        if not getattr(self, 'vgg_act', None):
            return {}
        if getattr(self, '_rms_scratch', None) is None:
            self._rms_scratch = (self._zeros(1024), self._zeros(1))
        part, out = self._rms_scratch
        res = {}
        for name, (y, _h) in self.vgg_activations().items():
            ops.rms16(y, part, out)
            res['activation/' + name] = float(out)
        return res

    def named_gradients(self):
        inv = 1.0 / self.loss_scale
        return OrderedDict((k, v.detach() * inv) for k, v in self.gview.items())

    @property
    def future_im_pred(self):
        return self.pred[..., :3]

    def memory_bytes(self):
        return self._alloc_bytes

    def step_flops(self):
        return sum(l.flops for p in (self.prog_fwd, self.prog_bwd) for l in p if l.fn is not None)
```

### imm_amd/ops.py

```python
import ctypes as C

import torch

from . import _lib as L
from ._lib import ConvDesc, OptHParams, call


def _s():
    return C.c_void_p(torch.cuda.current_stream().cuda_stream)


def _p(t):
    if t is None:
        return None
    return C.c_void_p(t.data_ptr())


def dtype_enum(dt):
    if dt == torch.bfloat16:
        return L.IMM_BF16
    if dt == torch.float16:
        return L.IMM_F16
    if dt == torch.float32:
        return L.IMM_F32
# ... 37 lines not shown
            ny, nx = (k - py + 1) // 2, (k - px + 1) // 2
            d = ConvDesc(batch=batch, hi=ho, wi=wo, ci=co_pad, ldx=lddy, ho=ho, wo=wo, co=ci_out, ldy=lddx, kh=ny, kw=nx,
                         stride=1, pad_t=ny - 1, pad_l=nx - 1, updiv=1, kpad=round_up(ny * nx * co_pad, 32), flags=flags,
                         ldmask=ldmask, out_scale=2, out_off_y=py, out_off_x=px)
            out.append((d, 4 + 2 * py + px))
    return out


def device_info():
    out = (C.c_int32 * 2)()
    call('imm_device_info', C.cast(out, C.c_void_p))
    return int(out[0]), int(out[1])


def set_cu_limit(cus):
    call('imm_set_cu_limit', int(cus))


class Graph:

    def __init__(self):
        self._exec = C.c_void_p()

    def capture_begin(self):
        call('imm_graph_begin', _s())

    def capture_end(self):
        call('imm_graph_end', _s(), C.byref(self._exec))

    def launch(self):
        call('imm_graph_launch', self._exec, _s())

    def __del__(self):
        try:
            if self._exec:
                L.load().imm_graph_destroy(self._exec)
        except Exception:
            pass


def pack_weights(w, wt, mode, kh, kw, ci_real, co_real, c_pad, rows, kpad):
    call('imm_pack_weights', _p(w), _p(wt), dtype_enum(wt.dtype), mode, kh, kw, ci_real, co_real, c_pad, rows, kpad, _s())


class JobTable:

    def __init__(self, jobs, items_per_job, items_per_block, device, blocks_per_job=None):
        first = [0]
        if blocks_per_job is None:
            blocks_per_job = [max(1, -(-int(n) // items_per_block)) for n in items_per_job]
        for n in blocks_per_job:
            first.append(first[-1] + int(n))
        rows = [list(j) + [0] * (12 - len(j)) for j in jobs]
        self.jobs = torch.tensor(rows, dtype=torch.int64, device=device)
        self.blk_first = torch.tensor(first, dtype=torch.int32, device=device)
        self.n_jobs, self.n_blocks = len(jobs), first[-1]


def pack_table(jobs, device):
    blocks = []
    for j in jobs:
        n = L.load().imm_pack_weights_multi_blocks(int(j[2]), int(j[8]), int(j[9]))
        if n <= 0:
            raise L.ImmHipError('imm_pack_weights_multi_blocks(%d, %d, %d) failed' % (j[2], j[8], j[9]))
        blocks.append(n)
    return JobTable(jobs, None, None, device, blocks_per_job=blocks)


def pack_weights_multi(tab, dtype):
    call('imm_pack_weights_multi', _p(tab.jobs), _p(tab.blk_first), tab.n_jobs, tab.n_blocks, dtype_enum(dtype), _s())


def reduce_table(jobs, outputs_per_job, device):
    rows, blocks = [], []
    for j, n in zip(jobs, outputs_per_job):
        lanes = 1
        while lanes < min(16, int(j[2])):
            lanes *= 2
        rows.append(tuple(j[:8]) + (lanes,))
        blocks.append(max(1, -(-int(n) // (1024 // lanes))))
    return JobTable(rows, None, None, device, blocks_per_job=blocks)


def wgrad_reduce_multi(tab):
    call('imm_wgrad_reduce_multi', _p(tab.jobs), _p(tab.blk_first), tab.n_jobs, tab.n_blocks, _s())


def conv2d(desc, x, wt, bias, y, stats=None, mask=None):
    call('imm_conv2d', C.byref(desc), dtype_enum(x.dtype), _p(x), _p(wt), _p(bias), _p(y), _p(stats), _p(mask), _s())


def conv2d_tap_supported(desc):
    return bool(L.load().imm_conv2d_tap_supported(C.byref(desc)))


def conv2d_tap(desc, x, wt, y, a_pred, a_gt, lda, loss_mask, S, coef, idx, l1=False):
    call('imm_conv2d_tap', C.byref(desc), dtype_enum(x.dtype), _p(x), _p(wt), _p(y), _p(a_pred), _p(a_gt), lda, _p(loss_mask), S,
         _p(coef), idx, int(l1), _s())


def conv_stats_blocks(desc):
    n = L.load().imm_conv_stats_blocks(C.byref(desc))
    if n <= 0:
        raise L.ImmHipError('imm_conv_stats_blocks: ' + L.load().imm_last_error().decode())
    return n


def conv2d_wgrad(desc, x, dy, lddy, slab, nsplit):
    call('imm_conv2d_wgrad', C.byref(desc), dtype_enum(x.dtype), _p(x), _p(dy), lddy, _p(slab), nsplit, _s())


CONV_FAMILIES = {1: 'igemm', 2: 'igemm64', 3: 'halo', 4: 'halo2', 5: 'hdeep', 6: 'hdeep6', 7: 's2f', 8: 'f32'}


def conv2d_variant(desc, dtype):
    key = L.load().imm_conv2d_variant(C.byref(desc), dtype_enum(dtype))
    if key < 0:
        raise L.ImmHipError('imm_conv2d_variant: ' + L.load().imm_last_error().decode())
    return CONV_FAMILIES[key // 100000], key


def conv2d_wgrad_variant(desc, lddy, dtype):
    wps, units, pcu = C.c_int(0), C.c_int(0), C.c_int(0)
    key = L.load().imm_conv2d_wgrad_variant(C.byref(desc), lddy, dtype_enum(dtype), C.byref(wps), C.byref(units), C.byref(pcu))
    if key < 0:
        raise L.ImmHipError('imm_conv2d_wgrad_variant: ' + L.load().imm_last_error().decode())
    return key, wps.value, units.value, pcu.value


class WgradMulti(object):

    def __init__(self, jobs, dtype):
        n = len(jobs)
        self.keep = [t for j in jobs for t in (j[1], j[2], j[4])] + [t for j in jobs if len(j) > 6 and j[6] for t in j[6][:2]]
        arr = (L.WgradJob * n)()
        for i, job in enumerate(jobs):
            desc, x, dy, lddy, slab, nsplit = job[:6]
            arr[i].desc = desc
            arr[i].x, arr[i].dy, arr[i].slab = x.data_ptr(), dy.data_ptr(), slab.data_ptr()
            arr[i].lddy, arr[i].nsplit = int(lddy), int(nsplit)
            if len(job) > 6 and job[6]:
                arr[i].x_scale, arr[i].x_shift, arr[i].x_relu = job[6][0].data_ptr(), job[6][1].data_ptr(), int(bool(job[6][2]))
        nbytes = L.load().imm_conv2d_wgrad_multi_table_bytes(n)
        if nbytes <= 0:
            raise L.ImmHipError('imm_conv2d_wgrad_multi_table_bytes(%d)' % n)
        self.host = (C.c_ubyte * nbytes)()
        call('imm_conv2d_wgrad_multi_plan', C.cast(arr, C.c_void_p), n, dtype_enum(dtype), C.cast(self.host, C.c_void_p))
        self.dev = torch.frombuffer(self.host, dtype=torch.uint8).clone().to(jobs[0][1].device)
        self.n = n


def conv2d_wgrad_multi(multi):
    call('imm_conv2d_wgrad_multi', C.cast(multi.host, C.c_void_p), _p(multi.dev), _s())


def conv2d_wgrad_splits(desc, lddy):
    n = L.load().imm_conv2d_wgrad_splits(C.byref(desc), lddy)
    if n < 0:
        raise L.ImmHipError('imm_conv2d_wgrad_splits failed')
    return n


def conv2d_wgrad_reduce(slab, nsplit, kh, kw, ci_pad, ci_real, co, kpad, dw):
    call('imm_conv2d_wgrad_reduce', _p(slab), nsplit, kh, kw, ci_pad, ci_real, co, kpad, _p(dw), _s())


def colsum_blocks(npix, c):
    n = L.load().imm_colsum_blocks(npix, c)
    if n <= 0:
        raise L.ImmHipError('imm_colsum_blocks(%d,%d) unsupported' % (npix, c))
    return n


def colsum(dy, npix, c, c_out, ld, partial, out):
    call('imm_colsum', _p(dy), dtype_enum(dy.dtype), npix, c, c_out, ld, _p(partial), _p(out), _s())


def bn_finalize(partial, nblk, c, count, gamma, beta, eps, momentum, training, mm, mv, scale, shift, mean, rstd):
    call('imm_bn_finalize', _p(partial), nblk, c, count, _p(gamma), _p(beta), eps, momentum, int(training), _p(mm),
         _p(mv), _p(scale), _p(shift), _p(mean), _p(rstd), _s())


def bn_apply_relu(y, npix, c, ldy, scale, shift, relu, x_out, ldx):
    call('imm_bn_apply_relu', _p(y), dtype_enum(y.dtype), npix, c, ldy, _p(scale), _p(shift), int(relu), _p(x_out), ldx, _s())


def bn_apply_fused(partial, nblk, c, count, gamma, beta, eps, momentum, training, mm, mv, scale, shift, mean, rstd, y, ldy,
                   relu, x_out, ldx, up2x=None, ldu=0, h=0, w=0):
    call('imm_bn_apply_fused', _p(partial), nblk, c, count, _p(gamma), _p(beta), eps, momentum, int(training), _p(mm), _p(mv),
         _p(scale), _p(shift), _p(mean), _p(rstd), _p(y), dtype_enum(y.dtype), ldy, int(relu), _p(x_out), ldx,
         _p(up2x), ldu, h, w, _s())


def bn_bwd_apply_fused(partial, nblk, c, count, gamma, dout, lddo, y, ldy, scale, shift, mean, rstd, relu, dgamma, dbeta,
                       dy_out, lddy):
    call('imm_bn_bwd_apply_fused', _p(partial), nblk, c, count, _p(gamma), _p(dout), lddo, _p(y), ldy, dtype_enum(y.dtype),
         _p(scale), _p(shift), _p(mean), _p(rstd), int(relu), _p(dgamma), _p(dbeta), _p(dy_out), lddy, _s())


def bn_bwd_blocks(npix, c):
    n = L.load().imm_bn_bwd_blocks(npix, c)
    if n <= 0:
        raise L.ImmHipError('imm_bn_bwd_blocks(%d,%d) unsupported' % (npix, c))
    return n


def rows_reduce(src, rows, width, group, dst):
    call('imm_rows_reduce', _p(src), rows, width, group, _p(dst), _s())


def bn_bwd_reduce(dout, lddo, y, ldy, npix, c, scale, shift, mean, rstd, relu, partial):
    call('imm_bn_bwd_reduce', _p(dout), lddo, _p(y), ldy, dtype_enum(y.dtype), npix, c, _p(scale), _p(shift), _p(mean),
         _p(rstd), int(relu), _p(partial), _s())


def bn_bwd_reduce_up(dy_up, lddy, dprev, lddp, y, ldy, batch, h, w, c, scale, shift, mean, rstd, relu, partial):
    call('imm_bn_bwd_reduce_up', _p(dy_up), lddy, _p(dprev), lddp, _p(y), ldy, dtype_enum(y.dtype), batch, h, w, c, _p(scale),
         _p(shift), _p(mean), _p(rstd), int(relu), _p(partial), _s())


def bn_bwd_finalize(partial, nblk, c, count, gamma, beta, rstd, dgamma, dbeta, coef, from_out=False, ldp=None):
    call('imm_bn_bwd_finalize', _p(partial), nblk, c, c if ldp is None else ldp, count, _p(gamma), _p(beta), _p(rstd),
         int(from_out), _p(dgamma), _p(dbeta), _p(coef), _s())


def bn_bwd_apply(dout, lddo, y, ldy, npix, c, scale, shift, mean, rstd, relu, coef, dy_out, lddy):
    call('imm_bn_bwd_apply', _p(dout), lddo, _p(y), ldy, dtype_enum(y.dtype), npix, c, _p(scale), _p(shift), _p(mean),
         _p(rstd), int(relu), _p(coef), _p(dy_out), lddy, _s())


def upsample2x_fwd(x, y, batch, h, w, c, ldx, ldy):
    call('imm_upsample2x_fwd', _p(x), _p(y), dtype_enum(x.dtype), batch, h, w, c, ldx, ldy, _s())


def upsample2x_bwd(dy, dx, batch, h, w, c, lddy, lddx):
    call('imm_upsample2x_bwd', _p(dy), _p(dx), dtype_enum(dy.dtype), batch, h, w, c, lddy, lddx, _s())


def upsample2x_bwd_bn_blocks(batch, h, w, c):
    n = L.load().imm_upsample2x_bwd_bn_blocks(batch, h, w, c)
    if n <= 0:
        raise L.ImmHipError('imm_upsample2x_bwd_bn_blocks(%d,%d,%d,%d) unsupported' % (batch, h, w, c))
    return n


def upsample2x_bwd_bn(dy, dx, batch, h, w, c, lddy, lddx, out, ldo, partial):
    call('imm_upsample2x_bwd_bn', _p(dy), _p(dx), dtype_enum(dy.dtype), batch, h, w, c, lddy, lddx, _p(out), ldo, _p(partial), _s())


def resize_ac_fwd(x, y, batch, hi, wi, ho, wo, c, ldx, ldy):
    call('imm_resize_ac_fwd', _p(x), _p(y), dtype_enum(x.dtype), batch, hi, wi, ho, wo, c, ldx, ldy, _s())


def resize_ac_bwd(dy, dx, batch, hi, wi, ho, wo, c, lddy, lddx):
    call('imm_resize_ac_bwd', _p(dy), _p(dx), dtype_enum(dy.dtype), batch, hi, wi, ho, wo, c, lddy, lddx, _s())


def maxpool2_fwd(x, y, batch, h, w, c):
    call('imm_maxpool2_fwd', _p(x), _p(y), dtype_enum(x.dtype), batch, h, w, c, _s())


def maxpool2_bwd(x, dy, dx, batch, h, w, c, relu_mask):
    call('imm_maxpool2_bwd', _p(x), _p(dy), _p(dx), dtype_enum(x.dtype), batch, h, w, c, int(relu_mask), _s())


def pack_image_taps(src, dst, batch, h, w, kw, pad_l, ld):
    call('imm_pack_image_taps', _p(src), _p(dst), dtype_enum(dst.dtype), batch, h, w, kw, pad_l, ld, _s())


def pack_image(src, dst, npix):
    call('imm_pack_image', _p(src), _p(dst), dtype_enum(dst.dtype), npix, _s())


def gauss_mode_enum(mode):
    if mode not in L.GAUSS_MODES:
        raise ValueError('Unknown mode: ' + str(mode))
    return L.GAUSS_MODES[mode]


def softargmax_gauss_fwd(heat, ldh, batch, h, w, k, inv_std, s, mu, py, px, gauss_out, ldg, dtype, mode='rot'):
    call('imm_softargmax_gauss_fwd', _p(heat), ldh, batch, h, w, k, float(inv_std), s, _p(mu), _p(py), _p(px),
         _p(gauss_out), ldg, dtype_enum(dtype), gauss_mode_enum(mode), _s())


def gauss_render_fwd(mu, batch, k, inv_std, s, gauss_out, ldg, dtype, mode='rot'):
    call('imm_softargmax_gauss_fwd', None, 0, batch, 0, 0, k, float(inv_std), s, _p(mu), None, None, _p(gauss_out), ldg,
         dtype_enum(dtype), gauss_mode_enum(mode), _s())


def softargmax_gauss_bwd(dgauss, ldg, batch, h, w, k, inv_std, s, mu, py, px, dheat, lddh, mode='rot'):
    call('imm_softargmax_gauss_bwd', _p(dgauss), ldg, dtype_enum(dheat.dtype), batch, h, w, k, float(inv_std), s, _p(mu),
         _p(py), _p(px), _p(dheat), lddh, gauss_mode_enum(mode), _s())


MAX_KEYPOINTS = 16


def keypoint_desc(w, b, geom, keypoints, image_size):
    m = int(keypoints.shape[1])
    if not 1 <= m <= MAX_KEYPOINTS:
        raise ValueError('the keypoint epilogue serves 1..%d annotated points, got %d' % (MAX_KEYPOINTS, m))
    if tuple(w.shape[1:]) != (2 * m,) or tuple(b.shape) != (2 * m,) or geom.shape[1:] != (4,) or keypoints.shape[2:] != (2,):
        raise ValueError('keypoint descriptor shapes: w %s, b %s, geom %s, keypoints %s' % (
            tuple(w.shape), tuple(b.shape), tuple(geom.shape), tuple(keypoints.shape)))
    for t in (w, b, geom, keypoints):
        if t.dtype != torch.float32 or not t.is_contiguous():
# ... 43 lines not shown
    call('imm_vgg_conv1_1_bwd', _p(dz), dtype_enum(dz.dtype), batch, s, _p(w), _p(gt), _p(pred), ldp, _p(mask), _p(coef),
         int(input_idx), int(l1), _p(dpred), lddp, _s())


def image_loss_grad(gt, pred, ldp, batch, s, mask, coef, idx, dpred, lddp, l1=False):
    call('imm_image_loss_grad', _p(gt), _p(pred), ldp, batch, s, _p(mask), _p(coef), int(idx), int(l1), _p(dpred), lddp,
         dtype_enum(dpred.dtype), _s())


def masked_sse(a, b, batch, s, c, mask, S, partial, l1=False):
    call('imm_masked_sse', _p(a), _p(b), dtype_enum(a.dtype), batch, s, c, _p(mask), S, int(l1), _p(partial), _s())


class SseMulti:

    def __init__(self, feats):
        n = len(feats)
        self.n = n
        self.keep = feats
        self.a = (C.c_void_p * n)(*[f[0].data_ptr() for f in feats])
        self.b = (C.c_void_p * n)(*[f[1].data_ptr() for f in feats])
        self.s = (C.c_int32 * n)(*[int(f[2]) for f in feats])
        self.c = (C.c_int32 * n)(*[int(f[3]) for f in feats])
        self.p = (C.c_void_p * n)(*[f[4].data_ptr() for f in feats])
        self.dtype = feats[0][0].dtype


def masked_sse_multi(g, batch, mask, S, l1=False):
    call('imm_masked_sse_multi', g.n, C.cast(g.a, C.c_void_p), C.cast(g.b, C.c_void_p), C.cast(g.s, C.c_void_p), C.cast(g.c, C.c_void_p),
         C.cast(g.p, C.c_void_p), dtype_enum(g.dtype), batch, _p(mask), S, int(l1), _s())


def masked_sse_all(g, batch, mask, S, img_a, lda, img_b, ldb, img_c, img_partial, l1=False):
    call('imm_masked_sse_all', g.n, C.cast(g.a, C.c_void_p), C.cast(g.b, C.c_void_p), C.cast(g.s, C.c_void_p), C.cast(g.c, C.c_void_p),
         C.cast(g.p, C.c_void_p), dtype_enum(g.dtype), batch, _p(mask), S, int(l1), _p(img_a), lda, _p(img_b), ldb, img_c,
         _p(img_partial), _s())


def masked_sse_f32(a, lda, b, ldb, batch, s, c, mask, partial, l1=False):
    call('imm_masked_sse_f32', _p(a), lda, _p(b), ldb, batch, s, c, _p(mask), int(l1), _p(partial), _s())


LOSS_PERCEPTUAL, LOSS_L2 = 0, 1


def perceptual_finalize(partial, nfeat, nel, agg, training, wd_loss, out, l1=False, mode=LOSS_PERCEPTUAL, loss_scale=None):
    call('imm_perceptual_finalize', _p(partial), nfeat, _p(nel), _p(agg), int(training), _p(wd_loss), int(l1), int(mode),
         _p(loss_scale), _p(out), _s())


def tap_grad(da, has_in, a_pred, a_gt, batch, s, c, mask, S, coef, idx, relu, l1=False):
    call('imm_tap_grad', _p(da), int(has_in), _p(a_pred), _p(a_gt), dtype_enum(da.dtype), batch, s, c, _p(mask), S,
         _p(coef), idx, int(relu), int(l1), _s())


def copy_f32(dst, src):
    assert dst.dtype == torch.float32 and src.dtype == torch.float32 and dst.numel() == src.numel()
    assert dst.is_contiguous() and src.is_contiguous() and (dst.is_cuda or dst.is_pinned()) and (src.is_cuda or src.is_pinned())
    call('imm_copy_f32', _p(dst), _p(src), dst.numel(), _s())


def upload(dst, src, what='tensor'):
    if not dst.is_cuda:
        dst.copy_(torch.as_tensor(src).reshape(dst.shape))
        return
    src = torch.as_tensor(src)
    if src.is_cuda:
        dst.copy_(src.reshape(dst.shape))
        return
    stage = torch.empty(dst.shape, dtype=dst.dtype, pin_memory=True)
    stage.copy_(src.reshape(dst.shape))
    back = torch.empty(dst.shape, dtype=dst.dtype, pin_memory=True)
    stream = torch.cuda.current_stream(dst.device)
    dst.copy_(stage, non_blocking=True)
    back.copy_(dst, non_blocking=True)
    stream.synchronize()
    if not torch.equal(back.reshape(-1).view(torch.uint8), stage.reshape(-1).view(torch.uint8)):
        nbad = int((back.reshape(-1).view(torch.uint8) != stage.reshape(-1).view(torch.uint8)).sum())
        raise RuntimeError('imm_amd: host-to-device upload of %s (%d bytes) does not read back as written (%d bytes differ)'
                           % (what, stage.numel() * stage.element_size(), nbad))


class PinnedStager:

    def __init__(self):
        self._slots = {}

    def copy(self, dst, src, key=None):
        src = torch.as_tensor(src)
        if not dst.is_cuda or src.is_cuda:
            dst.copy_(src.reshape(dst.shape))
            return
        key = dst.data_ptr() if key is None else key
        ent = self._slots.get(key)
        if ent is None or ent['bufs'][0].shape != dst.shape or ent['bufs'][0].dtype != dst.dtype:
            ent = {'bufs': [torch.empty(dst.shape, dtype=dst.dtype, pin_memory=True) for _ in range(2)], 'evs': [None, None], 'i': 0}
            self._slots[key] = ent
        i = ent['i']
        ent['i'] = 1 - i
        if ent['evs'][i] is not None:
            ent['evs'][i].synchronize()
        ent['bufs'][i].copy_(src.reshape(dst.shape))
        dst.copy_(ent['bufs'][i], non_blocking=True)
        ev = torch.cuda.Event()
        ev.record(torch.cuda.current_stream(dst.device))
        ent['evs'][i] = ev


def to_device_pinned(src, device, dtype=None):
    src = torch.as_tensor(src)
    device = torch.device(device)
    dtype = src.dtype if dtype is None else dtype
    if device.type != 'cuda' or src.is_cuda:
        return src.to(device=device, dtype=dtype)
    stage = torch.empty(src.shape, dtype=dtype, pin_memory=True)
    stage.copy_(src)
    dst = torch.empty(src.shape, dtype=dtype, device=device)
    dst.copy_(stage, non_blocking=True)
    ev = torch.cuda.Event()
    ev.record(torch.cuda.current_stream(device))
    ev.synchronize()
    return dst


def download(src):
    if not src.is_cuda:
        return src.detach().clone()
    back = torch.empty(src.shape, dtype=src.dtype, pin_memory=True)
    back.copy_(src.detach(), non_blocking=True)
    torch.cuda.current_stream(src.device).synchronize()
    return back.clone()


def cost_ema(cost3, state4, decay=0.99):
    call('imm_cost_ema', _p(cost3), _p(state4), float(decay), _s())


def rms16(x, partial, out):
    assert x.is_contiguous() and x.numel() % 8 == 0
    call('imm_rms16', _p(x), x.numel(), dtype_enum(x.dtype), _p(partial), min(int(partial.numel()), 4096), _p(out), _s())


def weight_decay_loss(params, tab, blk_partial, out):
    call('imm_weight_decay_loss', _p(params), _p(tab.blk_seg), _p(tab.blk_begin), _p(tab.blk_end), tab.nblk, _p(tab.seg_wd),
         _p(blk_partial), _p(out), _s())


def clip_adam_step(params, grads, m, v, tab, blk_partial, seg_norm2, step_count, adam_t, lr_state, hp, loss_scale_state=None):
    call('imm_clip_adam_step', _p(params), _p(grads), _p(m), _p(v), _p(tab.blk_seg), _p(tab.blk_begin), _p(tab.blk_end),
         tab.nblk, tab.nseg, _p(tab.seg_first_blk), _p(tab.seg_wd), _p(blk_partial), _p(seg_norm2), _p(step_count),
         _p(adam_t), _p(lr_state), C.byref(hp), _p(loss_scale_state), _s())


class SegmentTable:
    CHUNK = 2048

    def __init__(self, sizes, wds, device):
        offs = [0]
        for n in sizes:
            offs.append(offs[-1] + int(n))
        blk_seg, blk_begin, blk_end, first = [], [], [], [0]
        for s, n in enumerate(sizes):
            for b0 in range(0, int(n), self.CHUNK):
                blk_seg.append(s)
                blk_begin.append(offs[s] + b0)
                blk_end.append(offs[s] + min(int(n), b0 + self.CHUNK))
            first.append(len(blk_seg))
        self.offsets = offs
        self.nseg, self.nblk, self.total = len(sizes), len(blk_seg), offs[-1]
        i32 = dict(dtype=torch.int32, device=device)
        self.blk_seg = torch.tensor(blk_seg, **i32)
        self.blk_begin = torch.tensor(blk_begin, **i32)
        self.blk_end = torch.tensor(blk_end, **i32)
        self.seg_first_blk = torch.tensor(first, **i32)
        self.seg_wd = torch.tensor([float(w) for w in wds], dtype=torch.float32, device=device)


def debug_stamp(slots, index):
    call('imm_debug_stamp', _p(slots), int(index), _s())


def _check_pixels(name, t, shape, c_min, ld=None):
    b, h, w = shape
    ld = t.stride(2) if ld is None and t.dim() == 4 else ld
    if (t.dtype != torch.float32 or t.dim() != 4 or t.shape[0] != b or tuple(t.shape[1:3]) != (h, w) or t.shape[3] < c_min or
            ld < t.shape[3] or any(n > 1 and st != want for n, st, want in zip(t.shape, t.stride(), (h * w * ld, w * ld, ld, 1)))):
        raise ValueError('%s must be f32 [%d, %d, %d, >= %d] with dense pixels of one stride%s, got %s %s strides %s' % (
            name, b, h, w, c_min, '' if ld is None else ' %d' % ld, t.dtype, tuple(t.shape), tuple(t.stride())))
    return ld


def _check_tps(src, basis_t, w_tps, grid_pixels):
    if src.dim() != 4:
        raise ValueError('src must be f32 [B, H, W, C], got %s %s' % (src.dtype, tuple(src.shape)))
    b, h, w, c = src.shape
    ld_src = _check_pixels('src', src, (b, h, w), c)
    m3 = w_tps.shape[1] if w_tps.dim() == 3 else -1
    _check_tensors([('w_tps', w_tps, torch.float32, (b, None, 2)), ('basis_t', basis_t, torch.float32, (m3, grid_pixels))])
    return b, h, w, c, ld_src, m3


def tps_warp(src, basis_t, w_tps, dst=None, dst_c0=None, dst_rest=None):
    b, h, w, c, ld_src, m3 = _check_tps(src, basis_t, w_tps, src.shape[1] * src.shape[2] if src.dim() == 4 else 0)
    c_out = c if 1 <= c <= 8 else 0
    ld_dst = _check_pixels('dst', dst, (b, h, w), c_out) if dst is not None else 0
    ld_rest = _check_pixels('dst_rest', dst_rest, (b, h, w), max(c_out - 1, 0)) if dst_rest is not None else 0
    if dst_c0 is not None:
        _check_tensors([('dst_c0', dst_c0, torch.float32, (b, h, w))])
    call('imm_tps_warp', _p(src), ld_src, b, h, w, c, _p(basis_t), m3, _p(w_tps), _p(dst), ld_dst, _p(dst_c0), _p(dst_rest), ld_rest, _s())


def tps_warp_pad(src, basis_t, w_tps, pad_yx, grid_hw, crop_yx, dst):
    b, h, w, c, ld_src, m3 = _check_tps(src, basis_t, w_tps, int(grid_hw[0]) * int(grid_hw[1]))
    if dst.dim() != 4:
        raise ValueError('dst must be f32 [B, oh, ow, >= C], got %s %s' % (dst.dtype, tuple(dst.shape)))
    ld_dst = _check_pixels('dst', dst, (b, dst.shape[1], dst.shape[2]), c if 1 <= c <= 8 else 0)
    call('imm_tps_warp_pad', _p(src), ld_src, b, h, w, c, pad_yx[0], pad_yx[1], grid_hw[0], grid_hw[1], crop_yx[0], crop_yx[1],
         dst.shape[1], dst.shape[2], _p(basis_t), m3, _p(w_tps), _p(dst), ld_dst, _s())


def resize_crop_u8(src_u8, offsets, hw, c, resize_hw, crop_yx, out_hw, dst, ld_dst=None, boxes=None):
    if boxes is not None and (boxes.dtype != torch.int32 or boxes.dim() != 2 or boxes.shape[1] != 5 or not boxes.is_contiguous()):
        raise ValueError('boxes must be contiguous int32 [n, 5], got %s %s' % (boxes.dtype, tuple(boxes.shape)))
    _check_tensors([('src_u8', src_u8, torch.uint8, (None,)), ('hw', hw, torch.int32, (None, 2))])
    _check_tensors([('offsets', offsets, torch.int64, (hw.shape[0],))])
    batch = hw.shape[0] if boxes is None else boxes.shape[0]
    if dst.dim() != 4 or dst.shape[0] < batch:
        raise ValueError('dst must be f32 [>= %d, %d, %d, >= c], got %s %s' % (batch, out_hw[0], out_hw[1], dst.dtype, tuple(dst.shape)))
    ld_dst = _check_pixels('dst', dst, (dst.shape[0], int(out_hw[0]), int(out_hw[1])), c if 1 <= c <= 4 else 0, ld_dst)
    call('imm_resize_crop_u8', _p(src_u8), _p(offsets), _p(hw), _p(boxes), batch, c, resize_hw[0], resize_hw[1], crop_yx[0],
         crop_yx[1], out_hw[0], out_hw[1], _p(dst), ld_dst, _s())


MAX_ALIGN_M3 = 67


def align_coeffs(mu, ft, k, m3, coef):
    if ft.dtype != torch.float32 or ft.numel() != 4 * k * m3 or not ft.is_contiguous():
        raise ValueError('ft must be contiguous f32 [2K, 2 m3] = [%d, %d], got %s %s' % (2 * k, 2 * m3, ft.dtype, tuple(ft.shape)))
    n = mu.shape[0]
    assert mu.is_contiguous() and coef.is_contiguous() and mu.numel() == n * 2 * k and coef.numel() == n * 2 * m3
    call('imm_align_coeffs', _p(mu), _p(ft), n, int(k), int(m3), _p(coef), _s())


def align_warp_u8(src, offsets, hw, boxes, geom, coef, basis_t, image_size, dst, ld_dst=None):
    n, So = dst.shape[0], dst.shape[1]
    m3 = coef.shape[1]
    f32 = src.dtype == torch.float32
    if f32:
        if tuple(src.shape) != (n, image_size, image_size, 3) or not src.is_contiguous():
            raise ValueError('an f32 source must be contiguous [n, S, S, 3], got %s' % (tuple(src.shape),))
        n_images = n
    else:
        if src.dtype != torch.uint8 or offsets is None or hw is None or boxes is None:
            raise ValueError('a u8 source needs offsets, hw and boxes')
        if boxes.dtype != torch.int32 or tuple(boxes.shape) != (n, 5) or not boxes.is_contiguous():
            raise ValueError('boxes must be contiguous int32 [n, 5], got %s %s' % (boxes.dtype, tuple(boxes.shape)))
        n_images = hw.shape[0]
    if dst.shape[2] != So or tuple(geom.shape) != (n, 4) or tuple(coef.shape) != (n, m3, 2) or not (geom.is_contiguous() and coef.is_contiguous()):
        raise ValueError('dst [n, So, So, c], geom [n, 4], coef [n, m3, 2] (contiguous)')
    if (m3 > 3) != (basis_t is not None) or (basis_t is not None and (tuple(basis_t.shape) != (m3, So * So) or not basis_t.is_contiguous())):
        raise ValueError('basis_t must be contiguous f32 [m3, So * So] for m3 > 3 and None for m3 == 3')
    call('imm_align_warp_u8', _p(src), int(f32), _p(offsets), _p(hw), int(n_images), _p(boxes), _p(geom), _p(coef), _p(basis_t), int(m3),
         n, int(image_size), So, _p(dst), dst.stride(2) if ld_dst is None else ld_dst, _s())


def _check_tensors(specs):
    for name, t, dt, shape in specs:
        if (t.dtype != dt or t.dim() != len(shape) or any(s is not None and s != d for s, d in zip(shape, t.shape)) or
                not t.is_contiguous()):
            raise ValueError('%s must be contiguous %s [%s], got %s %s' % (name, str(dt).replace('torch.', ''), ', '.join(
                'any' if s is None else str(s) for s in shape), t.dtype, tuple(t.shape)))


def _check_faces(faces, n):
    S, ld = faces.shape[1], faces.stride(2)
    if (faces.dtype != torch.float32 or faces.dim() != 4 or faces.shape[0] != n or faces.shape[2] != S or faces.shape[3] < 3 or
            faces.stride(3) != 1 or faces.stride(1) != S * ld or faces.stride(0) != S * S * ld):
        raise ValueError('faces must be f32 [n, S, S, >= 3] with dense pixels of one stride, got %s %s strides %s' % (
            faces.dtype, tuple(faces.shape), tuple(faces.stride())))
    return S, ld


def compose_u8(photos, offsets, hw, boxes, links, inv_ramp, faces, max_box_pixels):
    n = boxes.shape[0]
    _check_tensors([('photos', photos, torch.uint8, (None,)), ('boxes', boxes, torch.int32, (n, 5)), ('links', links, torch.int32, (n, 2)),
                    ('inv_ramp', inv_ramp, torch.float32, (n, 2))])
    S, ld = _check_faces(faces, n)
    call('imm_compose_u8', _p(photos), _p(offsets), _p(hw), int(hw.shape[0]), _p(boxes), _p(links), _p(inv_ramp), _p(faces), int(ld), n,
         int(S), int(max_box_pixels), _s())


def unalign_maps(coef, geom, boxes, hw, image_size, out_size, fwd, bbox):
    n = boxes.shape[0]
    _check_tensors([('boxes', boxes, torch.int32, (n, 5)), ('coef', coef, torch.float32, (n, 3, 2)), ('geom', geom, torch.float32, (n, 4)),
                    ('hw', hw, torch.int32, (None, 2)), ('fwd', fwd, torch.float32, (n, 6)), ('bbox', bbox, torch.int32, (n, 4))])
    call('imm_unalign_maps', _p(coef), _p(geom), _p(boxes), _p(hw), int(hw.shape[0]), n, int(image_size), int(out_size), _p(fwd),
         _p(bbox), _s())


def unalign_u8(photos, offsets, hw, boxes, links, fwd, bbox, inv_ramp, faces, max_pixels):
    n = boxes.shape[0]
    _check_tensors([('photos', photos, torch.uint8, (None,)), ('boxes', boxes, torch.int32, (n, 5)), ('links', links, torch.int32, (n, 2)),
                    ('fwd', fwd, torch.float32, (n, 6)), ('bbox', bbox, torch.int32, (n, 4))])
    So, ld = _check_faces(faces, n)
    call('imm_unalign_u8', _p(photos), _p(offsets), _p(hw), int(hw.shape[0]), _p(boxes), _p(links), _p(fwd), _p(bbox), float(inv_ramp),
         _p(faces), int(ld), n, int(So), int(max_pixels), _s())


def track_step(mu, boxes, hw, state, image_size, next_image, init, box_smooth, min_cutoff, beta, d_cutoff, c, te, filter_off, points,
               points_smooth, boxes_next, geom_next, flags):
    F, K = mu.shape[0], mu.shape[1]
    _check_tensors([('mu', mu, torch.float32, (F, K, 2)), ('boxes', boxes, torch.int32, (F, 5)), ('state', state, torch.float64, (F, 5 + 6 * K)),
                    ('points', points, torch.float32, (F, K, 2)), ('points_smooth', points_smooth, torch.float32, (F, K, 2)),
                    ('boxes_next', boxes_next, torch.int32, (F, 5)), ('geom_next', geom_next, torch.float32, (F, 4)),
                    ('flags', flags, torch.int32, (F,)), ('hw', hw, torch.int32, (None, 2))])
    call('imm_track_step', _p(mu), _p(boxes), _p(hw), _p(state), int(K), int(image_size), int(F), int(hw.shape[0]), int(next_image),
         int(init), float(box_smooth), float(min_cutoff), float(beta), float(d_cutoff), float(c), float(te), int(bool(filter_off)),
         _p(points), _p(points_smooth), _p(boxes_next), _p(geom_next), _p(flags), _s())


def retarget(q, anchor, driver_flags, m, prev, init, relative, rigid, gain, out, flags):
    n, K = m.shape[0], m.shape[1]
    _check_tensors([('q', q, torch.float32, (K, 2)), ('anchor', anchor, torch.float64, (K, 2)), ('driver_flags', driver_flags, torch.int32, (1,)),
                    ('m', m, torch.float32, (n, K, 2)), ('prev', prev, torch.float32, (n, K, 2)), ('out', out, torch.float32, (n, K, 2)),
                    ('flags', flags, torch.int32, (n,))])
    call('imm_retarget', _p(q), _p(anchor), _p(driver_flags), _p(m), _p(prev), int(K), int(n), int(init), int(bool(relative)),
# ... 389 lines not shown
```

### imm_amd/train/cnn_train_multi.py

```python
import json
import os
import time

import torch
import torch.distributed as dist

from .. import ops


def split_inputs(inputs, num_splits, index):
    out = {}
    for k, v in inputs.items():
        n = v.shape[0]
        assert n % num_splits == 0, 'Batch size must be divisible by number of GPUs'
        per = n // num_splits
        out[k] = v[index * per:(index + 1) * per]
    return out


def average_gradients(flat_grads, world_size, group=None, force=False, async_op=False):
    if world_size > 1 or (force and dist.is_initialized()):
        if flat_grads.is_cuda and dist.get_backend(group) == 'gloo':
            host = _pinned_like(flat_grads)
            stream = torch.cuda.current_stream(flat_grads.device)
            ops.copy_f32(host, flat_grads.detach())
            stream.synchronize()
            dist.all_reduce(host, op=dist.ReduceOp.SUM, group=group)
            ops.copy_f32(flat_grads, host)
            stream.synchronize()
            return None
        return dist.all_reduce(flat_grads, op=dist.ReduceOp.SUM, group=group, async_op=async_op)
    return None


_PINNED = {}


def _pinned_like(t):
    key = (t.numel(), t.dtype)
    if key not in _PINNED:
        _PINNED[key] = torch.empty(t.numel(), dtype=t.dtype).pin_memory()
    return _PINNED[key].view(t.shape)


def mean_tower_loss(loss, world_size, group=None):
    if world_size > 1 and dist.is_initialized():
        t = loss.detach().reshape(1).to(torch.float32).clone()
        if t.is_cuda and dist.get_backend(group) == 'gloo':
            t = t.cpu()
        dist.all_reduce(t, op=dist.ReduceOp.SUM, group=group)
        return float(t) / world_size
    return float(loss)


class TrainStep:

    COLLECTIVES = ('pg', 'native', 'graph')

    def __init__(self, model, batch_per_rank, image_size, world_size=1, use_graph=True, group=None, split_graphs=False,
                 collective=None, debug_poison=None):
        self.model = model
        self.world_size = world_size
        self.split = split_graphs or world_size > 1
        self.group = group
        model.require_vgg()
        self.engine = model._get_engine(batch_per_rank, image_size)
        model._master = self.engine
        self.buckets = 2 if self.engine.n_bwd_bucket0 is not None else 1
        if abs(self.engine.hp.grad_scale - 1.0 / world_size) > 1e-9:
            raise ValueError('engine was built for world_size %g' % (1.0 / self.engine.hp.grad_scale))
        self.use_graph = use_graph
        if collective is None:
            collective = ('graph' if os.environ.get('IMM_RCCL_GRAPH', '0') != '0' else
                          'native' if os.environ.get('IMM_RCCL_NATIVE', '0') != '0' else 'pg')
        if collective not in self.COLLECTIVES:
            raise ValueError('collective must be one of %r, got %r' % (self.COLLECTIVES, collective))
        if collective == 'graph' and not use_graph:
            raise ValueError("collective 'graph' needs use_graph=True")
        self.collective = collective if self.split else None
        if debug_poison is None:
            debug_poison = os.environ.get('IMM_DEBUG_POISON_GRADS', '0') != '0'
        self.debug_poison = bool(debug_poison)
        self._poison_mask = None
        self.after_backward = None
        self.graph_resident = self.split and use_graph and collective == 'graph'
        self.native_comm = None
        if self.split and collective in ('native', 'graph'):
            rank = dist.get_rank(group) if dist.is_initialized() else 0
            with torch.cuda.device(self.engine.dev):
                self.native_comm = ops.RcclComm(rank, world_size, group)
            self.comm_stream = torch.cuda.Stream(device=self.engine.dev)
        self.stream = torch.cuda.Stream(device=self.engine.dev)
        self._graphs = None
        torch.cuda.synchronize(self.engine.dev)

    def _probe(self, flat):
        if self.debug_poison:
            flat.mul_(2.0)

    def _poison(self):
        eng = self.engine
        if self._poison_mask is None:
            snap = eng.snapshot()
            eng.grads.fill_(float('nan'))
            eng.forward(True); eng.backward()
            torch.cuda.current_stream(eng.dev).synchronize()
            self._poison_mask = ~torch.isnan(eng.grads)
            eng.restore(snap)
            torch.cuda.current_stream(eng.dev).synchronize()
        eng.grads.masked_fill_(self._poison_mask, float('nan'))

    def _capture(self):
        eng = self.engine
        with torch.cuda.stream(self.stream):
            if self.debug_poison and self._poison_mask is None:
                snap0 = eng.snapshot(); self._poison(); eng.restore(snap0)
            snap = eng.snapshot()
            eng.forward(True); eng.backward(); eng.optimizer_step()
            self.stream.synchronize()
            eng.restore(snap)
            self.stream.synchronize()
            eng._training = True
            if self.graph_resident:
                self.native_comm.all_reduce_sum(eng.grads)
                self.stream.synchronize()
                g = ops.Graph()
                g.capture_begin()
                if self.buckets < 2:
                    eng.run(eng.prog_fwd); eng.run(eng.prog_bwd)
                    self.native_comm.all_reduce_sum(eng.grads); self._probe(eng.grads)
                else:
                    n0, off = eng.n_bwd_bucket0, eng.bucket0_offset
                    eng.run(eng.prog_fwd); eng.run(eng.prog_bwd[:n0])
                    fork = torch.cuda.Event(); fork.record(self.stream)
                    self.comm_stream.wait_event(fork)
                    with torch.cuda.stream(self.comm_stream):
                        self.native_comm.all_reduce_sum(eng.grads[off:]); self._probe(eng.grads[off:])
                    eng.run(eng.prog_bwd[n0:])
                    tail = torch.cuda.Event(); tail.record(self.stream)
                    self.comm_stream.wait_event(tail)
                    with torch.cuda.stream(self.comm_stream):
                        self.native_comm.all_reduce_sum(eng.grads[:off]); self._probe(eng.grads[:off])
                    join = torch.cuda.Event(); join.record(self.comm_stream)
                    self.stream.wait_event(join)
                eng.run(eng.prog_opt)
                if self.debug_poison:
                    self._poison()
                g.capture_end()
                self._graphs = (g,)
            elif not self.split:
                g = ops.Graph()
                g.capture_begin()
                eng.run(eng.prog_fwd); eng.run(eng.prog_bwd); eng.run(eng.prog_opt)
                g.capture_end()
                self._graphs = (g,)
            elif self.buckets < 2:
                g1 = ops.Graph()
                g1.capture_begin()
                eng.run(eng.prog_fwd); eng.run(eng.prog_bwd)
                g1.capture_end()
                g2 = ops.Graph()
                g2.capture_begin()
                eng.run(eng.prog_opt)
                g2.capture_end()
                self._graphs = (g1, g2)
            else:
                n0 = eng.n_bwd_bucket0
                g1 = ops.Graph()
                g1.capture_begin()
                eng.run(eng.prog_fwd); eng.run(eng.prog_bwd[:n0])
                g1.capture_end()
                g1b = ops.Graph()
                g1b.capture_begin()
                eng.run(eng.prog_bwd[n0:])
                g1b.capture_end()
                g2 = ops.Graph()
                g2.capture_begin()
                eng.run(eng.prog_opt)
                g2.capture_end()
                self._graphs = (g1, g1b, g2)

    def step(self, inputs=None):
        eng = self.engine
        self.stream.wait_stream(torch.cuda.current_stream(eng.dev))
        with torch.cuda.stream(self.stream):
            if inputs is not None:
                eng.set_inputs(inputs['image'], inputs['future_image'], inputs.get('mask'))
                for v in (inputs['image'], inputs['future_image'], inputs.get('mask')):
                    if torch.is_tensor(v) and v.is_cuda:
                        v.record_stream(self.stream)
            if self.use_graph:
                if self._graphs is None:
                    self._capture()
                self._graphs[0].launch()
                hook = self.after_backward
                if self.graph_resident:
                    pass
                elif self.split and self.native_comm is not None:
                    if hook is not None and self.buckets < 2:
                        hook(eng)
                    self._native_exchange(eng)
                elif self.split and self.buckets < 2:
                    if hook is not None:
                        hook(eng)
                    average_gradients(eng.grads, self.world_size, self.group, force=True); self._probe(eng.grads)
                    self._graphs[1].launch()
                elif self.split:
                    off = eng.bucket0_offset
                    w0 = average_gradients(eng.grads[off:], self.world_size, self.group, force=True, async_op=True)
                    self._graphs[1].launch()
                    if hook is not None:
                        hook(eng)
                    w1 = average_gradients(eng.grads[:off], self.world_size, self.group, force=True, async_op=True)
                    for w in (w0, w1):
                        if w is not None:
                            w.wait()
                    self._probe(eng.grads)
                    self._graphs[2].launch()
                if self.debug_poison and not self.graph_resident and self.split:
                    self._poison()
            else:
                eng.forward(True)
                eng.backward()
                if self.after_backward is not None:
                    self.after_backward(eng)
                average_gradients(eng.grads, self.world_size, self.group)
                eng.optimizer_step()
        torch.cuda.current_stream(eng.dev).wait_stream(self.stream)
        return eng.loss

    def _native_exchange(self, eng):
        def on_comm(flat):
            ev = torch.cuda.Event(); ev.record(self.stream)
            self.comm_stream.wait_event(ev)
            with torch.cuda.stream(self.comm_stream):
                self.native_comm.all_reduce_sum(flat); self._probe(flat)
        if self.buckets < 2:
            on_comm(eng.grads)
        else:
            off = eng.bucket0_offset
            on_comm(eng.grads[off:])
            self._graphs[1].launch()
            on_comm(eng.grads[:off])
        done = torch.cuda.Event(); done.record(self.comm_stream)
        self.stream.wait_event(done)
        self._graphs[-1].launch()

    def forward_only(self, inputs=None):
        eng = self.engine
        self.stream.wait_stream(torch.cuda.current_stream(eng.dev))
        with torch.cuda.stream(self.stream):
            if inputs is not None:
                eng.set_inputs(inputs['image'], inputs['future_image'], inputs.get('mask'))
                for v in (inputs['image'], inputs['future_image'], inputs.get('mask')):
                    if torch.is_tensor(v) and v.is_cuda:
                        v.record_stream(self.stream)
            if self.use_graph:
                if getattr(self, '_fwd_graph', None) is None:
                    snap = eng.snapshot()
                    eng.forward(True)
                    self.stream.synchronize()
                    eng.restore(snap)
                    self.stream.synchronize()
                    g = ops.Graph()
                    g.capture_begin()
                    eng._training = True
                    eng.run(eng.prog_fwd)
                    g.capture_end()
                    self._fwd_graph = g
                eng._training = True
                self._fwd_graph.launch()
            else:
                eng.forward(True)
        torch.cuda.current_stream(eng.dev).wait_stream(self.stream)
        return eng.loss

    def measure_phases(self, steps=5):
        eng = self.engine
        old_mode, old_buf = eng._stamp_mode, eng._stamp_buf
        eng._stamp_mode = 'marks'
        if eng._stamp_buf is None:
            eng._stamp_buf = torch.zeros(8192, dtype=torch.int64, device=eng.dev)
        self._graphs = None
        rows = []
        try:
            for _ in range(max(1, steps)):
                self.step(None)
                self.synchronize()
                rep = eng.stamp_report()
                t = {}
                for us, _lane, label in rep:
                    t[label] = us
                bwd_end = t.get('bwd2:end', t.get('bwd:end'))
                if None in (t.get('fwd:start'), t.get('fwd:end'), t.get('bwd:start'), bwd_end, t.get('opt:start'), t.get('opt:end')):
                    continue
                rows.append(((t['fwd:end'] - t['fwd:start']) / 1e3, (bwd_end - t['bwd:start']) / 1e3,
                             (t['opt:start'] - bwd_end) / 1e3, (t['opt:end'] - t['opt:start']) / 1e3))
        finally:
            eng._stamp_mode, eng._stamp_buf = old_mode, old_buf
            self._graphs = None
            self.synchronize()
        if not rows:
            return None
        med = [sorted(r[i] for r in rows)[len(rows) // 2] for i in range(4)]
        return {'forward': round(med[0], 4), 'backward': round(med[1], 4), 'exchange_exposed': round(med[2], 4),
                'optimizer': round(med[3], 4), 'steps': len(rows)}

    def synchronize(self):
        self.stream.synchronize()


def setup_training(opts, model_factory, clip_value=None, use_graph=True):
    world = int(os.environ.get('WORLD_SIZE', '1'))
    assert opts['batch_size'] % world == 0, 'Batch size must be divisible by number of GPUs'
    model = model_factory.create()
    return TrainStep(model, opts['batch_size'] // world, opts['image_size'], world_size=world, use_graph=use_graph)


class SummaryWriter(object):

    def __init__(self, log_dir):
        from ..utils.tf_events import EventFileWriter
        os.makedirs(log_dir, exist_ok=True)
        self.path = os.path.join(log_dir, 'summaries.jsonl')
        self._f = open(self.path, 'a')
        self.events = EventFileWriter(log_dir)

    def add_summary(self, record, step, images=None):
        rec = {'step': int(step), 'time': time.time()}
        rec.update(record)
        self._f.write(json.dumps(rec) + '\n')
        family = str(record.get('tag', 'train'))
        scalars = {}
        for k, v in record.items():
            if k == 'tag':
                continue
            if isinstance(v, (list, tuple)):
                for i, x in enumerate(v):
                    scalars['%s/%s/%d' % (family, k, i)] = float(x)
            else:
                scalars['%s/%s' % (family, k)] = float(v)
        self.events.add_scalars(scalars, step, images={'%s/%s' % (family, k): v for k, v in (images or {}).items()})

    def flush(self):
        self._f.flush()
        self.events.flush()

    def close(self):
        self._f.close()
        self.events.close()


def image_summaries(eng, max_outputs=3):
    from ..models.imm_model import colorize_landmark_maps
    n = min(int(max_outputs), eng.B)
    S = eng.S

    def tile(x):
        x = x[:n].float().clamp(0, 255).to(torch.uint8).cpu().numpy()
        return x.transpose(1, 0, 2, 3).reshape(S, n * S, 3)

    full = torch.empty(eng.B, S, S, eng.K, device=eng.dev)
    ops.gauss_render_f32(eng.mu, eng.B, eng.K, eng.inv_std, S, full, eng.cfg.gauss_mode)
    maps = colorize_landmark_maps(full[:n])
    maps = maps / maps.amax().clamp_min(1e-12) * 255.0
    return {'im': tile(eng.in_image), 'future_im': tile(eng.in_future), 'future_im_pred': tile(eng.future_im_pred),
            'pose_embedding': tile(maps)}


def run_test_pass(model, test_dataset, step, writer=None, verbose=True):
    total, count, it_n = 0.0, 0, 0
    for inputs in test_dataset:
        t0 = time.time()
        _, loss, _ = model.build(inputs, training_pl=False, build_loss=True)
        value = float(loss)
        n = int(inputs['image'].shape[0])
        total, count = total + value * n, count + n
        if verbose:
            dt = time.time() - t0
            print('test: step %d, loss = %.4f (%.1f examples/sec) %.3f sec/batch' % (step, value, n / dt, dt))
# ... 88 lines not shown
```

### include/imm_hip.h

```cpp
#ifndef IMM_HIP_H
#define IMM_HIP_H

#include <stdint.h>

#ifdef __cplusplus
extern "C" {
#endif

#define IMM_ABI_VERSION 35

enum imm_dtype { IMM_BF16 = 0, IMM_F16 = 1, IMM_F32 = 2 };

enum imm_error {
  IMM_OK = 0,
  IMM_E_INVALID = -1,
  IMM_E_UNSUPPORTED = -2,
  IMM_E_HIP = -3
};

#define IMM_CONV_BIAS 1
#define IMM_CONV_RELU 2
#define IMM_CONV_STATS 4
#define IMM_CONV_MASK 8
#define IMM_CONV_OUT_F32 16

typedef struct imm_conv_desc {
  int32_t batch, hi, wi, ci;
  int32_t ldx;
  int32_t ho, wo, co;
  int32_t ldy;
  int32_t kh, kw, stride, pad_t, pad_l;
  int32_t updiv;
  int32_t kpad;
  int32_t flags;
  int32_t ldmask;
  int32_t out_scale, out_off_y, out_off_x;
} imm_conv_desc;

int imm_abi_version(void);
const char* imm_last_error(void);
const char* imm_source_digest(void);
int imm_device_info(int32_t* out2_host);
int imm_set_cu_limit(int cus);
int imm_get_cu_limit(void);
int imm_debug_stamp(uint64_t* slots, int index, void* stream);
int imm_copy_f32(float* dst, const float* src, int64_t n, void* stream);
int imm_graph_begin(void* stream);
int imm_graph_end(void* stream, void** graph_exec_out_host);
int imm_graph_launch(void* graph_exec, void* stream);
int imm_graph_destroy(void* graph_exec);

int imm_pack_weights(const float* w, void* wt, int dtype, int mode, int kh, int kw, int ci_real, int co_real,
                     int c_pad, int rows, int kpad, void* stream);

int imm_pack_weights_multi_blocks(int mode, int rows, int kpad);
int imm_pack_weights_multi(const int64_t* jobs, const int32_t* blk_first, int n_jobs, int n_blocks, int dtype,
                           void* stream);
int imm_wgrad_reduce_multi(const int64_t* jobs, const int32_t* blk_first, int n_jobs, int n_blocks, void* stream);

int imm_conv2d_group(const imm_conv_desc* descs, int n, int dtype, const void* x, const void* const* wts, void* y,
                     float* stats_partial, const void* mask_ref, void* stream);
int imm_conv2d_group_stats_blocks(const imm_conv_desc* descs, int n);
int imm_conv2d_nol_supported(const imm_conv_desc* desc_host);
int imm_conv2d_nol_stats_blocks(const imm_conv_desc* desc_host);
int imm_conv2d_nol(const imm_conv_desc* desc_host, int dtype, const void* x_raw, const float* x_scale, const float* x_shift,
                   int x_relu, const void* wt, const float* bias, void* y, float* stats_partial, void* stream);
int imm_conv2d_dgrad_s2_supported(int batch, int h, int w, int lddy, int c_dx, int lddx);
int imm_conv2d_dgrad_s2(const void* dy, int lddy, const void* wt, int kpad, void* dx, int lddx, int c_dx, int dtype, int batch,
                        int h, int w, void* stream);
int imm_conv2d(const imm_conv_desc* desc_host, int dtype, const void* x, const void* wt, const float* bias,
               void* y, float* stats_partial, const void* mask_ref, void* stream);
int imm_conv_stats_blocks(const imm_conv_desc* desc_host);
int imm_conv2d_variant(const imm_conv_desc* desc_host, int dtype);
int imm_conv2d_tap_supported(const imm_conv_desc* desc_host);
int imm_conv2d_tap(const imm_conv_desc* desc_host, int dtype, const void* x, const void* wt, void* y, const void* a_pred,
                   const void* a_gt, int lda, const float* loss_mask, int S, const float* coef, int idx, int l1, void* stream);
int imm_conv2d_wgrad(const imm_conv_desc* desc_host, int dtype, const void* x, const void* dy, int lddy,
                     float* slab, int nsplit, void* stream);
int imm_conv2d_wgrad_splits(const imm_conv_desc* desc_host, int lddy);
int imm_conv2d_wgrad_reduce(const float* slab, int nsplit, int kh, int kw, int ci_pad, int ci_real, int co,
                            int kpad, float* dw, void* stream);
typedef struct imm_wgrad_job {
  imm_conv_desc desc;
  const void* x; const void* dy; float* slab;
  int32_t lddy, nsplit;
  const float* x_scale; const float* x_shift;
  int32_t x_relu, reserved;
} imm_wgrad_job;
int64_t imm_conv2d_wgrad_multi_table_bytes(int n);
int imm_conv2d_wgrad_variant(const imm_conv_desc* desc_host, int lddy, int dtype, int* wg_per_split_host, int* units_host,
                             int* wg_per_cu_host);
int imm_conv2d_wgrad_multi_plan(const imm_wgrad_job* jobs_host, int n, int dtype, void* table_host);
int imm_conv2d_wgrad_multi(const void* table_host, const void* table_dev, void* stream);
int imm_colsum(const void* dy, int dtype, int64_t npix, int c, int c_out, int ld, float* partial, float* out,
               void* stream);
int imm_colsum_blocks(int64_t npix, int c);

int imm_bn_finalize(const float* partial, int nblk, int c, int64_t count, const float* gamma, const float* beta,
                    float eps, float momentum, int training, float* moving_mean, float* moving_var,
                    float* scale, float* shift, float* mean, float* rstd, void* stream);
int imm_bn_apply_relu(const void* y, int dtype, int64_t npix, int c, int ldy, const float* scale,
                      const float* shift, int relu, void* x_out, int ldx, void* stream);
int imm_bn_apply_fused(const float* partial, int nblk, int c, int64_t count, const float* gamma, const float* beta, float eps,
                       float momentum, int training, float* moving_mean, float* moving_var, float* scale, float* shift,
                       float* mean, float* rstd, const void* y, int dtype, int ldy, int relu, void* x_out, int ldx,
                       void* up2x_out, int ldu, int h, int w, void* stream);
int imm_rows_reduce(const float* in, int rows, int width, int group, float* out, void* stream);
int imm_bn_bwd_reduce(const void* dout, int lddo, const void* y, int ldy, int dtype, int64_t npix, int c,
                      const float* scale, const float* shift, const float* mean, const float* rstd, int relu,
                      float* partial, void* stream);
int imm_bn_bwd_blocks(int64_t npix, int c);
int imm_bn_bwd_reduce_up(const void* dy_up, int lddy, void* dprev, int lddp, const void* y, int ldy, int dtype, int batch, int h,
                         int w, int c, const float* scale, const float* shift, const float* mean, const float* rstd, int relu,
                         float* partial, void* stream);
int imm_bn_bwd_finalize(const float* partial, int nblk, int c, int ldp, int64_t count, const float* gamma, const float* beta,
                        const float* rstd, int from_out, float* dgamma, float* dbeta, float* coef, void* stream);
int imm_bn_bwd_apply(const void* dout, int lddo, const void* y, int ldy, int dtype, int64_t npix, int c,
                     const float* scale, const float* shift, const float* mean, const float* rstd, int relu,
                     const float* coef, void* dy_out, int lddy, void* stream);
int imm_bn_bwd_apply_fused(const float* partial, int nblk, int c, int64_t count, const float* gamma, const void* dout, int lddo,
                           const void* y, int ldy, int dtype, const float* scale, const float* shift, const float* mean,
                           const float* rstd, int relu, float* dgamma, float* dbeta, void* dy_out, int lddy, void* stream);

int imm_upsample2x_fwd(const void* x, void* y, int dtype, int batch, int h, int w, int c, int ldx, int ldy,
                       void* stream);
int imm_upsample2x_bwd(const void* dy, void* dx, int dtype, int batch, int h, int w, int c, int lddy, int lddx,
                       void* stream);
int imm_upsample2x_bwd_bn(const void* dy, void* dx, int dtype, int batch, int h, int w, int c, int lddy, int lddx,
                          const void* out, int ldo, float* partial, void* stream);
int imm_upsample2x_bwd_bn_blocks(int batch, int h, int w, int c);
int imm_resize_ac_fwd(const void* x, void* y, int dtype, int batch, int hi, int wi, int ho, int wo, int c,
                      int ldx, int ldy, void* stream);
int imm_resize_ac_bwd(const void* dy, void* dx, int dtype, int batch, int hi, int wi, int ho, int wo, int c,
                      int lddy, int lddx, void* stream);
int imm_maxpool2_fwd(const void* x, void* y, int dtype, int batch, int h, int w, int c, void* stream);
int imm_maxpool2_bwd(const void* x, const void* dy, void* dx, int dtype, int batch, int h, int w, int c,
                     int relu_mask, void* stream);

int imm_pack_image(const float* src, void* dst, int dtype, int64_t npix, void* stream);
int imm_pack_image_taps(const float* src, void* dst, int dtype, int batch, int h, int w, int kw, int pad_l, int ld,
                        void* stream);

int imm_conv_first_supported(int batch, int s, int co, int ldy);
int imm_conv_first_stats_blocks(int batch, int s);
int imm_conv_first(const float* image, const void* wt, int kpad, const float* bias, void* y, int ldy, float* stats_partial, int dtype,
                   int batch, int s, int co, int flags, void* stream);

#define IMM_GAUSS_ROT 0
#define IMM_GAUSS_FLAT 1
#define IMM_GAUSS_ANKUSH 2
int imm_softargmax_gauss_fwd(const float* heat, int ldh, int batch, int h, int w, int k, float inv_std, int s,
                             float* mu, float* py, float* px, void* gauss_out, int ldg, int dtype, int gauss_mode,
                             void* stream);
int imm_softargmax_gauss_bwd(const void* dgauss, int ldg, int dtype, int batch, int h, int w, int k, float inv_std,
                             int s, const float* mu, const float* py, const float* px, void* dheat, int lddh,
                             int gauss_mode, void* stream);
typedef struct imm_keypoint_desc {
  const float* w;
  const float* b;
  const float* geom;
  float* keypoints;
  int32_t m;
  int32_t image_size;
} imm_keypoint_desc;
int imm_pose_head_fwd(const void* feat, int ldf, int c, const void* wt, int kpad, const float* bias, int dtype, int batch, int h,
                      int w, int k, float inv_std, int s, float* heat, int ldh, float* mu, float* py, float* px, void* gauss_out,
                      int ldg, int gauss_mode, const imm_keypoint_desc* kp, void* stream);
int imm_pose_head_bwd(const void* dgauss, int ldg, int dtype, int batch, int h, int w, int k, float inv_std, int s, const float* mu,
                      const float* py, const float* px, void* dheat, int lddh, int gauss_mode, const void* wt_dgrad, int kpad_d,
                      int c, void* dfeat, int lddf, float* bias_partial, void* stream);
int imm_gauss_render_f32(const float* mu, int batch, int k, float inv_std, int s, float* out, int gauss_mode, void* stream);

int imm_vgg_conv1_1_fwd(const float* gt, const float* pred, int ldp, int batch, int s, const float* w9x64,
                        const float* b64, void* out, int dtype, int halves, void* stream);
int imm_vgg_head_supported(int batch, int s, int dtype);
int64_t imm_vgg_head_scratch_bytes(int batch, int s);
int imm_vgg_head_fwd(const float* gt, const float* pred, int ldp, int batch, int s, const float* w9x64, const float* b64,
                     const void* wt12, int kpad12, const float* b12, void* a11, int store_from, void* y12, void* gray_scratch,
                     int dtype, void* stream);
int imm_vgg_conv1_1_bwd(const void* dz, int dtype, int batch, int s, const float* w9x64, const float* gt,
                        const float* pred, int ldp, const float* mask, const float* coef, int input_idx, int l1,
                        void* dpred, int lddp, void* stream);
int imm_image_loss_grad(const float* gt, const float* pred, int ldp, int batch, int s, const float* mask,
                        const float* coef, int idx, int l1, void* dpred, int lddp, int dtype, void* stream);

#define IMM_SSE_BLOCKS 512
int imm_masked_sse_multi(int n, const void* const* a, const void* const* b, const int32_t* s_host, const int32_t* c_host,
                         float* const* partial, int dtype, int batch, const float* mask, int S, int l1, void* stream);
int imm_masked_sse_all(int n, const void* const* a, const void* const* b, const int32_t* s_host, const int32_t* c_host,
                       float* const* partial, int dtype, int batch, const float* mask, int S, int l1,
                       const float* img_a, int lda, const float* img_b, int ldb, int img_c, float* img_partial, void* stream);
int imm_masked_sse(const void* a, const void* b, int dtype, int batch, int s, int c, const float* mask, int S, int l1,
                   float* partial, void* stream);
int imm_masked_sse_pool(const void* a, const void* b, int dtype, int batch, int s, int c, const float* mask, int S,
                        float* partial, void* pool_a, void* pool_b, void* stream);
int imm_masked_sse_f32(const float* a, int lda, const float* b, int ldb, int batch, int s, int c, const float* mask,
                       int l1, float* partial, void* stream);
#define IMM_LOSS_PERCEPTUAL 0
#define IMM_LOSS_L2 1
int imm_perceptual_finalize(const float* partial, int nfeat, const float* nel, float* agg, int training,
                            const float* wd_loss, int l1, int mode, const float* loss_scale, float* out, void* stream);
int imm_cost_ema(const float* cost3, float* state4, float decay, void* stream);
int imm_rms16(const void* x, int64_t n, int dtype, float* partial, int nblk, float* out, void* stream);
int imm_unpool_tap_grad(void* da, const void* dpool, const void* a_pred, const void* a_gt, int dtype, int batch, int s, int c,
                        const float* mask, int S, const float* coef, int idx, void* stream);
int imm_tap_grad(void* da, int has_in, const void* a_pred, const void* a_gt, int dtype, int batch, int s, int c,
                 const float* mask, int S, const float* coef, int idx, int relu, int l1, void* stream);

#define IMM_OPT_ADAM 0
#define IMM_OPT_ADADELTA 1
#define IMM_OPT_ADAGRAD 2
typedef struct imm_opt_hparams {
  float lr_start, lr_decay; int32_t lr_step; float lr_multiple;
  float beta1, beta2, eps, clip;
  float grad_scale;
  int32_t optim;
  int32_t scale_growth_interval;
  float scale_max;
} imm_opt_hparams;
int imm_weight_decay_loss(const float* params, const int32_t* blk_seg, const int32_t* blk_begin,
                          const int32_t* blk_end, int nblk, const float* seg_wd, float* blk_partial, float* out,
                          void* stream);
int imm_clip_adam_step(float* params, float* grads, float* m, float* v, const int32_t* blk_seg,
                       const int32_t* blk_begin, const int32_t* blk_end, int nblk, int nseg,
                       const int32_t* seg_first_blk, const float* seg_wd, float* blk_partial, float* seg_norm2,
                       int32_t* step_count, int32_t* adam_t, float* lr_state, const imm_opt_hparams* hp_host,
                       float* loss_scale_state, void* stream);

int imm_rccl_unique_id(void* out128_host);
int imm_rccl_init(int rank, int world, const void* unique_id128_host, void** comm_out_host);
int imm_rccl_allreduce(void* comm, float* buf, int64_t count, void* stream);
int imm_rccl_destroy(void* comm);

int64_t imm_conv2d_workspace_bytes(const imm_conv_desc* desc_host);
int64_t imm_conv2d_group_workspace_bytes(const imm_conv_desc* descs, int n);
int64_t imm_conv2d_wgrad_workspace_bytes(const imm_conv_desc* desc_host, int lddy, int nsplit);
int64_t imm_colsum_workspace_bytes(int64_t npix, int c);
int64_t imm_bn_bwd_workspace_bytes(int64_t npix, int c);
int64_t imm_upsample2x_bwd_bn_workspace_bytes(int batch, int h, int w, int c);
int64_t imm_masked_sse_workspace_bytes(int nfeat);

int imm_tps_warp(const float* src, int ld_src, int batch, int h, int w, int c, const float* basis_t, int m3,
                 const float* w_tps, float* dst, int ld_dst, float* dst_c0, float* dst_rest, int ld_rest, void* stream);
int imm_tps_warp_pad(const float* src, int ld_src, int batch, int h, int w, int c, int pad_y, int pad_x, int grid_h, int grid_w,
                     int crop_y, int crop_x, int out_h, int out_w, const float* basis_t, int m3, const float* w_tps,
                     float* dst, int ld_dst, void* stream);

int imm_resize_crop_u8(const uint8_t* src, const int64_t* offsets, const int32_t* hw, const int32_t* boxes, int batch, int c,
                       int resize_h, int resize_w, int crop_y0, int crop_x0, int out_h, int out_w, float* dst, int ld_dst,
                       void* stream);












int imm_crc32c(const void* data, uint64_t n, uint32_t* crc_inout);

#ifdef __cplusplus
}
#endif
#include "imm_align.h"
#include "imm_compose.h"
#include "imm_unalign.h"
#include "imm_track.h"
#include "imm_retarget.h"
#include "imm_warp.h"
#include "imm_morph.h"
#include "imm_colour.h"
#include "imm_hull.h"
#include "imm_seam.h"
#include "imm_clip.h"
#endif
```

Baseline: 10340 images/s.

## Overlap optimizer update with backward by fusing wgrad reduce into per-segment Adam

Adds a 'shadow' step program that interleaves backward with the optimizer. Filter-gradient launches are issued in parameter-size order, and the split-K slab reduction is folded into a combined reduce+prepare kernel that writes the scaled and weight-decayed gradients and their norm partials. Adam/clip updates then run per range of segments instead of as one tail pass over all parameters. The aim is to cut the separate wgrad-reduce kernel and the serialized optimizer tail after backward, at the cost of more launches, extra staging through LDS, and new planning complexity.

```diff
diff --git a/imm_amd/_lib.py b/imm_amd/_lib.py
--- a/imm_amd/_lib.py
+++ b/imm_amd/_lib.py
@@ -11,7 +11,7 @@
 SSE_BLOCKS = 512
 OPTIMIZERS = {'adam': 0, 'adadelta': 1, 'adagrad': 2}
 GAUSS_MODES = {'rot': 0, 'flat': 1, 'ankush': 2}
-ABI_VERSION = 35
+ABI_VERSION = 36
 
 
 class ImmHipError(RuntimeError):
@@ -205,6 +205,13 @@
     'imm_clip_ema': [_P, _P, _P, _P, _P, _I, _I, _F, _P],
 })
 
+_header('imm_opt_parts.h', {
+    'imm_conv2d_wgrad_multi_part': [_P, _P, _I, _I, _P],
+    'imm_conv2d_wgrad_multi_launches': [_P, _P, _I],
+    'imm_opt_reduce_prepare': [_P, _P, _P, _P, _P, _I, _I, _P, _P, _P, _P, _P, _P, _I, _I, _P, _P, _P, C.POINTER(OptHParams), _P],
+    'imm_opt_update': [_P, _P, _P, _P, _P, _P, _P, _I, _I, _P, _P, _P, _P, _P, _P, _P, C.POINTER(OptHParams), _P, _I, _I, _P],
+})
+
 _lib = None
 
 
diff --git a/imm_amd/csrc/conv_wgrad.hip b/imm_amd/csrc/conv_wgrad.hip
--- a/imm_amd/csrc/conv_wgrad.hip
+++ b/imm_amd/csrc/conv_wgrad.hip
@@ -306,7 +306,10 @@
 constexpr uint32_t WGM_MAGIC = 0x57474d31u;
 constexpr int WGM_MAX_LAUNCH = 16, WGM_MAX_JOBS = 64, WGM_ARG_STRIDE = 192, WGM_HEADER = 1024;
 struct WgmLaunch { int32_t kind, variant, n, arg_off, first_off, blocks, job0, pad; };
-struct WgmHeader { uint32_t magic; int32_t dtype, n_jobs, n_launch; WgmLaunch launch[WGM_MAX_LAUNCH]; };
+struct WgmHeader {
+  uint32_t magic; int32_t dtype, n_jobs, n_launch; WgmLaunch launch[WGM_MAX_LAUNCH];
+  uint8_t by_params[WGM_MAX_LAUNCH], job_launch[WGM_MAX_JOBS];
+};
 static_assert(sizeof(WgmHeader) <= WGM_HEADER, "header");
 
 int wgm_check_job(const imm_wgrad_job* j) {
@@ -365,6 +368,8 @@
   }
   int64_t off = WGM_HEADER;
   int job_slot = 0;
+  double l_params[WGM_MAX_LAUNCH];
+  int l_of_job[WGM_MAX_JOBS];
   for (int i = 0; i < n; ++i) {
     if (done[i]) continue;
     IMM_REQUIRE(h->n_launch < WGM_MAX_LAUNCH, "wgrad_multi_plan: more than %d kernel variants", WGM_MAX_LAUNCH);
@@ -373,6 +378,12 @@
     int idx[WGM_MAX_JOBS], m = 0;
     for (int k = i; k < n; ++k)
       if (!done[k] && kind[k] == kind[i] && variant[k] == variant[i] && (kind[i] != WGM_SINGLE || k == i)) { idx[m++] = k; done[k] = true; }
+    l_params[h->n_launch - 1] = 0.0;
+    for (int k = 0; k < m; ++k) {
+      const imm_conv_desc* d = &jobs[idx[k]].desc;
+      l_params[h->n_launch - 1] += (double)d->kh * d->kw * d->ci * d->co;
+      l_of_job[idx[k]] = h->n_launch - 1;
+    }
     L->n = m;
     L->arg_off = (int32_t)off;
     if (kind[i] == WGM_SINGLE) {
@@ -408,17 +419,33 @@
     L->job0 = job_slot; job_slot += m;
   }
   IMM_REQUIRE(off <= imm_conv2d_wgrad_multi_table_bytes(n), "wgrad_multi_plan: table overflow");
-  return 0;
-}
-
-extern "C" int imm_conv2d_wgrad_multi(const void* table_host, const void* table_dev, void* stream) {
+  int pos[WGM_MAX_LAUNCH], rank[WGM_MAX_LAUNCH];
+  for (int l = 0; l < h->n_launch; ++l) pos[l] = l;
+  for (int a = 1; a < h->n_launch; ++a)
+    for (int b = a; b > 0 && l_params[pos[b]] > l_params[pos[b - 1]]; --b) { const int t = pos[b]; pos[b] = pos[b - 1]; pos[b - 1] = t; }
+  for (int l = 0; l < h->n_launch; ++l) { h->by_params[l] = (uint8_t)pos[l]; rank[pos[l]] = l; }
+  for (int i = 0; i < n; ++i) h->job_launch[i] = (uint8_t)rank[l_of_job[i]];
+  return 0;
+}
+
+extern "C" int imm_conv2d_wgrad_multi_launches(const void* table_host, int32_t* job_launch_host, int n) {
+  IMM_REQUIRE(table_host && job_launch_host, "wgrad_multi_launches: null");
+  const WgmHeader* h = (const WgmHeader*)table_host;
+  IMM_REQUIRE(h->magic == WGM_MAGIC && h->n_jobs == n, "wgrad_multi_launches: not a planned table of %d jobs", n);
+  for (int i = 0; i < n; ++i) job_launch_host[i] = h->job_launch[i];
+  return 0;
+}
+
+static int wgm_issue(const void* table_host, const void* table_dev, int l0, int l1, bool ranked, void* stream) {
   IMM_REQUIRE(table_host && table_dev, "wgrad_multi: null");
   const char* hb = (const char*)table_host;
   const char* db = (const char*)table_dev;
   const WgmHeader* h = (const WgmHeader*)hb;
   IMM_REQUIRE(h->magic == WGM_MAGIC && h->n_launch >= 1 && h->n_launch <= WGM_MAX_LAUNCH, "wgrad_multi: not a planned table");
-  for (int l = 0; l < h->n_launch; ++l) {
-    const WgmLaunch* L = &h->launch[l];
+  if (l1 < 0) l1 = h->n_launch;
+  IMM_REQUIRE(l0 >= 0 && l0 < l1 && l1 <= h->n_launch, "wgrad_multi: launches [%d, %d) of %d", l0, l1, h->n_launch);
+  for (int l = l0; l < l1; ++l) {
+    const WgmLaunch* L = &h->launch[ranked ? h->by_params[l] : l];
     if (L->kind == WGM_SINGLE) {
       const imm_wgrad_job* j = (const imm_wgrad_job*)(hb + L->arg_off);
       const int rc = imm_conv2d_wgrad(&j->desc, h->dtype, j->x, j->dy, j->lddy, j->slab, j->nsplit, stream);
@@ -431,6 +458,15 @@
   }
   IMM_CHECK_LAUNCH("imm_conv2d_wgrad_multi");
   return 0;
+}
+
+extern "C" int imm_conv2d_wgrad_multi(const void* table_host, const void* table_dev, void* stream) {
+  return wgm_issue(table_host, table_dev, 0, -1, false, stream);
+}
+
+extern "C" int imm_conv2d_wgrad_multi_part(const void* table_host, const void* table_dev, int l0, int l1, void* stream) {
+  IMM_REQUIRE(l1 >= 0, "wgrad_multi_part: launches [%d, %d)", l0, l1);
+  return wgm_issue(table_host, table_dev, l0, l1, true, stream);
 }
 
 __global__ void wgrad_reduce_kernel(const float* __restrict__ slab, int nsplit, int ntaps, int ci_pad, int ci_real,
diff --git a/imm_amd/csrc/loss_optim.hip b/imm_amd/csrc/loss_optim.hip
--- a/imm_amd/csrc/loss_optim.hip
+++ b/imm_amd/csrc/loss_optim.hip
@@ -582,6 +582,37 @@
   *lr = (float)l;
 }
 
+__device__ __forceinline__ void grad_prepare_chunk(const float* __restrict__ params, float* __restrict__ grads,
+                                                   const float* stage, int sbase, int blk, const int32_t* __restrict__ blk_seg,
+                                                   const int32_t* __restrict__ blk_begin, const int32_t* __restrict__ blk_end,
+                                                   const float* __restrict__ seg_wd, float grad_scale,
+                                                   float* __restrict__ blk_partial, float* red) {
+  const float wd = seg_wd[blk_seg[blk]];
+  float acc = 0.f;
+  const int b0 = blk_begin[blk], b1 = blk_end[blk];
+  const int a0 = min((b0 + 3) & ~3, b1), a1 = max(a0, b1 & ~3);
+  for (int i = b0 + threadIdx.x; i < a0; i += LO_THREADS) {
+    const float g = (stage ? stage[i - sbase] : grads[i]) * grad_scale + wd * params[i];
+    grads[i] = g; acc += g * g;
+  }
+  for (int i = a0 + 4 * threadIdx.x; i < a1; i += 4 * LO_THREADS) {
+    float4 g;
+    if (stage) { const float* sp = stage + (i - sbase); g = make_float4(sp[0], sp[1], sp[2], sp[3]); }
+    else g = *(const float4*)(grads + i);
+    const float4 w = *(const float4*)(params + i);
+    g.x = g.x * grad_scale + wd * w.x; g.y = g.y * grad_scale + wd * w.y;
+    g.z = g.z * grad_scale + wd * w.z; g.w = g.w * grad_scale + wd * w.w;
+    *(float4*)(grads + i) = g;
+    acc += (g.x * g.x + g.y * g.y) + (g.z * g.z + g.w * g.w);
+  }
+  for (int i = a1 + threadIdx.x; i < b1; i += LO_THREADS) {
+    const float g = (stage ? stage[i - sbase] : grads[i]) * grad_scale + wd * params[i];
+    grads[i] = g; acc += g * g;
+  }
+  acc = block_sum_256(acc, red);
+  if (threadIdx.x == 0) blk_partial[blk] = acc;
+}
+
 __global__ __launch_bounds__(LO_THREADS) void grad_prepare_kernel(const float* __restrict__ params, float* __restrict__ grads,
                                                                   const int32_t* __restrict__ blk_seg,
                                                                   const int32_t* __restrict__ blk_begin,
@@ -599,43 +630,20 @@
     return;
   }
   if (loss_scale) grad_scale *= 1.f / loss_scale[0];
-  const float wd = seg_wd[blk_seg[blk]];
-  float acc = 0.f;
-  const int b0 = blk_begin[blk], b1 = blk_end[blk];
-  const int a0 = min((b0 + 3) & ~3, b1), a1 = max(a0, b1 & ~3);
-  for (int i = b0 + threadIdx.x; i < a0; i += LO_THREADS) {
-    const float g = grads[i] * grad_scale + wd * params[i];
-    grads[i] = g; acc += g * g;
-  }
-  for (int i = a0 + 4 * threadIdx.x; i < a1; i += 4 * LO_THREADS) {
-    float4 g = *(const float4*)(grads + i);
-    const float4 w = *(const float4*)(params + i);
-    g.x = g.x * grad_scale + wd * w.x; g.y = g.y * grad_scale + wd * w.y;
-    g.z = g.z * grad_scale + wd * w.z; g.w = g.w * grad_scale + wd * w.w;
-    *(float4*)(grads + i) = g;
-    acc += (g.x * g.x + g.y * g.y) + (g.z * g.z + g.w * g.w);
-  }
-  for (int i = a1 + threadIdx.x; i < b1; i += LO_THREADS) {
-    const float g = grads[i] * grad_scale + wd * params[i];
-    grads[i] = g; acc += g * g;
-  }
-  acc = block_sum_256(acc, red);
-  if (threadIdx.x == 0) blk_partial[blk] = acc;
-}
-
-__global__ __launch_bounds__(LO_THREADS) void clip_adam_kernel(float* __restrict__ params, const float* __restrict__ grads,
-                                                               float* __restrict__ m, float* __restrict__ v,
-                                                               const int32_t* __restrict__ blk_seg,
-                                                               const int32_t* __restrict__ blk_begin,
-                                                               const int32_t* __restrict__ blk_end,
-                                                               const int32_t* __restrict__ seg_first_blk,
-                                                               const float* __restrict__ blk_partial, int nblk,
-                                                               float* __restrict__ seg_norm2, int32_t* __restrict__ step_count,
-                                                               int32_t* __restrict__ adam_t, const float* __restrict__ lr_state,
-                                                               float* __restrict__ ls, imm_opt_hparams hp) {
-  __shared__ double dred[LO_THREADS / 64];
-  const int blk = blockIdx.x, tid = threadIdx.x;
-  const bool extra = blk == nblk;
+  grad_prepare_chunk(params, grads, nullptr, 0, blk, blk_seg, blk_begin, blk_end, seg_wd, grad_scale, blk_partial, red);
+}
+
+__device__ __forceinline__ void clip_adam_chunk(int blk, bool extra, float* __restrict__ params, const float* __restrict__ grads,
+                                                float* __restrict__ m, float* __restrict__ v,
+                                                const int32_t* __restrict__ blk_seg,
+                                                const int32_t* __restrict__ blk_begin,
+                                                const int32_t* __restrict__ blk_end,
+                                                const int32_t* __restrict__ seg_first_blk,
+                                                const float* __restrict__ blk_partial, int nblk,
+                                                float* __restrict__ seg_norm2, int32_t* __restrict__ step_count,
+                                                int32_t* __restrict__ adam_t, const float* __restrict__ lr_state,
+                                                float* __restrict__ ls, const imm_opt_hparams& hp, double* dred) {
+  const int tid = threadIdx.x;
   const int seg = extra ? 0 : blk_seg[blk];
   const int b0 = extra ? 0 : blk_begin[blk], b1 = extra ? 0 : blk_end[blk];
   const int a0 = min((b0 + 3) & ~3, b1), a1 = max(a0, b1 & ~3);
@@ -716,6 +724,196 @@
   for (int i = a1 + tid; i < b1; i += LO_THREADS) one(grads[i], m[i], v[i], params[i]);
 }
 
+__global__ __launch_bounds__(LO_THREADS) void clip_adam_kernel(float* __restrict__ params, const float* __restrict__ grads,
+                                                               float* __restrict__ m, float* __restrict__ v,
+                                                               const int32_t* __restrict__ blk_seg,
+                                                               const int32_t* __restrict__ blk_begin,
+                                                               const int32_t* __restrict__ blk_end,
+                                                               const int32_t* __restrict__ seg_first_blk,
+                                                               const float* __restrict__ blk_partial, int nblk,
+                                                               float* __restrict__ seg_norm2, int32_t* __restrict__ step_count,
+                                                               int32_t* __restrict__ adam_t, const float* __restrict__ lr_state,
+                                                               float* __restrict__ ls, imm_opt_hparams hp) {
+  __shared__ double dred[LO_THREADS / 64];
+  const int blk = blockIdx.x;
+  clip_adam_chunk(blk, blk == nblk, params, grads, m, v, blk_seg, blk_begin, blk_end, seg_first_blk, blk_partial, nblk, seg_norm2,
+                  step_count, adam_t, lr_state, ls, hp, dred);
+}
+
+#define OPT_MAX_RANGES IMM_OPT_MAX_RANGES
+#define OPT_SEG_FIELDS 12
+struct OptRanges { int32_t n = 0, total = 0; int32_t first[OPT_MAX_RANGES + 1] = {}; int32_t blk0[OPT_MAX_RANGES] = {}; };
+
+__device__ __forceinline__ int opt_range_blk(const OptRanges& R, int wg) {
+  int r = 0;
+  while (r + 1 < R.n && R.first[r + 1] <= wg) ++r;
+  return R.blk0[r] + (wg - R.first[r]);
+}
+
+__device__ __forceinline__ float4 opt_slab_sum4(const int64_t* __restrict__ jb, int64_t idx, int64_t total) {
+  const float* __restrict__ slab = (const float*)jb[0];
+  const int nsplit = (int)jb[2], ci_pad = (int)jb[4], ci_real = (int)jb[5], co = (int)jb[6], kpad = (int)jb[7];
+  const int SL = (int)jb[8] > 0 ? (int)jb[8] : 16;
+  const int64_t sstride = (int64_t)kpad * co;
+  float4 tot = make_float4(0.f, 0.f, 0.f, 0.f);
+  if ((co & 3) == 0) {
+    const int n = (int)(idx % co);
+    const int64_t tc = idx / co;
+    const int c = (int)(tc % ci_real), tap = (int)(tc / ci_real);
+    const float* sp = slab + ((int64_t)tap * ci_pad + c) * co + n;
+    for (int sl = 0; sl < SL; ++sl) {
+      float4 acc = make_float4(0.f, 0.f, 0.f, 0.f), a1 = acc;
+      int s = sl;
+      for (; s + SL < nsplit; s += 2 * SL) {
+        const float4 v0 = *(const float4*)(sp + (int64_t)s * sstride), v1 = *(const float4*)(sp + (int64_t)(s + SL) * sstride);
+        acc.x += v0.x; acc.y += v0.y; acc.z += v0.z; acc.w += v0.w;
+        a1.x += v1.x; a1.y += v1.y; a1.z += v1.z; a1.w += v1.w;
+      }
+      if (s < nsplit) {
+        const float4 v0 = *(const float4*)(sp + (int64_t)s * sstride);
+        acc.x += v0.x; acc.y += v0.y; acc.z += v0.z; acc.w += v0.w;
+      }
+      acc.x += a1.x; acc.y += a1.y; acc.z += a1.z; acc.w += a1.w;
+      if (sl == 0) tot = acc;
+      else { tot.x += acc.x; tot.y += acc.y; tot.z += acc.z; tot.w += acc.w; }
+    }
+  } else {
+    float* tp = &tot.x;
+    for (int e = 0; e < 4; ++e) {
+      const int64_t id = idx + e;
+      if (id >= total) break;
+      const int n = (int)(id % co);
+      const int64_t tc = id / co;
+      const int c = (int)(tc % ci_real), tap = (int)(tc / ci_real);
+      const float* sp = slab + ((int64_t)tap * ci_pad + c) * co + n;
+      float te = 0.f;
+      for (int sl = 0; sl < SL; ++sl) {
+        float t = 0.f;
+        for (int s = sl; s < nsplit; s += SL) t += sp[s * sstride];
+        if (sl == 0) te = t; else te += t;
+      }
+      tp[e] = te;
+    }
+  }
+  return tot;
+}
+
+__global__ __launch_bounds__(LO_THREADS) void reduce_prepare_kernel(const float* __restrict__ params, float* __restrict__ grads,
+                                                                    const int32_t* __restrict__ blk_seg,
+                                                                    const int32_t* __restrict__ blk_begin,
+                                                                    const int32_t* __restrict__ blk_end,
+                                                                    const int32_t* __restrict__ seg_first_blk,
+                                                                    const float* __restrict__ seg_wd,
+                                                                    const int64_t* __restrict__ seg_red, float grad_scale,
+                                                                    float* __restrict__ blk_partial, OptRanges R,
+                                                                    const int32_t* __restrict__ step_count,
+                                                                    const int32_t* __restrict__ adam_t, float* __restrict__ lr_state,
+                                                                    imm_opt_hparams hp) {
+  __shared__ float red[4];
+  __shared__ float4 stage4[IMM_OPT_MAX_CHUNK / 4 + 1];
+  const int wg = blockIdx.x, tid = threadIdx.x;
+  if (wg == R.total) {
+    if (tid == 0) opt_learning_rate(hp, step_count[0], adam_t[0] + 1, lr_state, lr_state + 1);
+    return;
+  }
+  const int blk = opt_range_blk(R, wg);
+  const int seg = blk_seg[blk];
+  const int64_t* jb = seg_red + (int64_t)seg * OPT_SEG_FIELDS;
+  const float* stage = nullptr;
+  int sbase = 0;
+  if (jb[0] != 0) {
+    const int f0 = seg_first_blk[seg];
+    const int off = blk_begin[f0];
+    const int r0 = blk_begin[blk] - off, r1 = blk_end[blk] - off, q0 = r0 & ~3;
+    if (r1 - q0 > IMM_OPT_MAX_CHUNK + 4) return;
+    const int64_t total = (int64_t)jb[3] * jb[5] * jb[6];
+    for (int q = tid; q0 + 4 * q < r1; q += LO_THREADS) stage4[q] = opt_slab_sum4(jb, q0 + 4 * q, total);
+    __syncthreads();
+    stage = (const float*)stage4; sbase = off + q0;
+  }
+  grad_prepare_chunk(params, grads, stage, sbase, blk, blk_seg, blk_begin, blk_end, seg_wd, grad_scale, blk_partial, red);
+}
+
+template <bool ADVANCE>
+__global__ __launch_bounds__(LO_THREADS) void update_parts_kernel(float* __restrict__ params, const float* __restrict__ grads,
+                                                                  float* __restrict__ m, float* __restrict__ v,
+                                                                  const int32_t* __restrict__ blk_seg,
+                                                                  const int32_t* __restrict__ blk_begin,
+                                                                  const int32_t* __restrict__ blk_end,
+                                                                  const int32_t* __restrict__ seg_first_blk,
+                                                                  const float* __restrict__ blk_partial, int nblk,
+                                                                  float* __restrict__ seg_norm2, int32_t* __restrict__ step_count,
+                                                                  int32_t* __restrict__ adam_t, const float* __restrict__ lr_state,
+                                                                  OptRanges R, imm_opt_hparams hp) {
+  __shared__ double dred[LO_THREADS / 64];
+  const int wg = blockIdx.x;
+  const bool extra = ADVANCE && wg == R.total;
+  clip_adam_chunk(extra ? nblk : opt_range_blk(R, wg), extra, params, grads, m, v, blk_seg, blk_begin, blk_end, seg_first_blk,
+                  blk_partial, nblk, seg_norm2, step_count, adam_t, lr_state, nullptr, hp, dred);
+}
+
+static int opt_ranges(const int32_t* ranges, int n_ranges, const int32_t* seg_first_blk_host, int nblk, int nseg, OptRanges* R,
+                      const char* who) {
+  IMM_REQUIRE(ranges && seg_first_blk_host, "%s: null", who);
+  IMM_REQUIRE(n_ranges >= 1 && n_ranges <= OPT_MAX_RANGES, "%s: %d ranges (1..%d)", who, n_ranges, OPT_MAX_RANGES);
+  IMM_REQUIRE(seg_first_blk_host[0] == 0 && seg_first_blk_host[nseg] == nblk, "%s: seg_first_blk_host is not the table's", who);
+  *R = OptRanges();
+  R->n = n_ranges;
+  int s = 0;
+  for (int r = 0; r < n_ranges; ++r) {
+    const int b0 = ranges[2 * r], b1 = ranges[2 * r + 1];
+    IMM_REQUIRE(b0 >= 0 && b0 < b1 && b1 <= nblk, "%s: range %d = [%d, %d) of %d chunks", who, r, b0, b1, nblk);
+    IMM_REQUIRE(r == 0 || b0 >= ranges[2 * r - 1], "%s: range %d overlaps the one before it or is out of order", who, r);
+    while (s < nseg && seg_first_blk_host[s] < b0) ++s;
+    IMM_REQUIRE(seg_first_blk_host[s] == b0, "%s: range %d starts inside a tensor (chunk %d)", who, r, b0);
+    while (s < nseg && seg_first_blk_host[s] < b1) ++s;
+    IMM_REQUIRE(seg_first_blk_host[s] == b1, "%s: range %d ends inside a tensor (chunk %d)", who, r, b1);
+    R->blk0[r] = b0;
+    R->first[r + 1] = R->first[r] + (b1 - b0);
+  }
+  R->total = R->first[n_ranges];
+  return 0;
+}
+
+extern "C" int imm_opt_reduce_prepare(const float* params, float* grads, const int32_t* blk_seg, const int32_t* blk_begin,
+                                      const int32_t* blk_end, int nblk, int nseg, const int32_t* seg_first_blk,
+                                      const int32_t* seg_first_blk_host, const float* seg_wd, const int64_t* seg_red,
+                                      float* blk_partial, const int32_t* ranges_host, int n_ranges, int compute_lr,
+                                      const int32_t* step_count, const int32_t* adam_t, float* lr_state,
+                                      const imm_opt_hparams* hp, void* stream) {
+  IMM_REQUIRE(params && grads && blk_seg && blk_begin && blk_end && seg_first_blk && seg_wd && seg_red && blk_partial &&
+                  step_count && adam_t && lr_state && hp, "opt_reduce_prepare: null");
+  IMM_REQUIRE(nblk > 0 && nseg > 0 && hp->lr_step > 0, "opt_reduce_prepare: dims");
+  OptRanges R;
+  if (opt_ranges(ranges_host, n_ranges, seg_first_blk_host, nblk, nseg, &R, "opt_reduce_prepare")) return IMM_E_INVALID;
+  hipLaunchKernelGGL(reduce_prepare_kernel, dim3(R.total + (compute_lr ? 1 : 0)), dim3(LO_THREADS), 0, (hipStream_t)stream, params,
+                     grads, blk_seg, blk_begin, blk_end, seg_first_blk, seg_wd, seg_red, hp->grad_scale, blk_partial, R, step_count,
+                     adam_t, lr_state, *hp);
+  IMM_CHECK_LAUNCH("imm_opt_reduce_prepare");
+  return 0;
+}
+
+extern "C" int imm_opt_update(float* params, const float* grads, float* m, float* v, const int32_t* blk_seg,
+                              const int32_t* blk_begin, const int32_t* blk_end, int nblk, int nseg, const int32_t* seg_first_blk,
+                              const int32_t* seg_first_blk_host, const float* blk_partial, float* seg_norm2, int32_t* step_count,
+                              int32_t* adam_t, const float* lr_state, const imm_opt_hparams* hp, const int32_t* ranges_host,
+                              int n_ranges, int advance, void* stream) {
+  IMM_REQUIRE(params && grads && m && v && blk_seg && blk_begin && blk_end && seg_first_blk && blk_partial && seg_norm2 &&
+                  step_count && adam_t && lr_state && hp, "opt_update: null");
+  IMM_REQUIRE(nblk > 0 && nseg > 0, "opt_update: dims");
+  IMM_REQUIRE(hp->optim >= IMM_OPT_ADAM && hp->optim <= IMM_OPT_ADAGRAD, "opt_update: optim %d", hp->optim);
+  OptRanges R;
+  if (opt_ranges(ranges_host, n_ranges, seg_first_blk_host, nblk, nseg, &R, "opt_update")) return IMM_E_INVALID;
+  if (advance)
+    hipLaunchKernelGGL(update_parts_kernel<true>, dim3(R.total + 1), dim3(LO_THREADS), 0, (hipStream_t)stream, params, grads, m, v,
+                       blk_seg, blk_begin, blk_end, seg_first_blk, blk_partial, nblk, seg_norm2, step_count, adam_t, lr_state, R, *hp);
+  else
+    hipLaunchKernelGGL(update_parts_kernel<false>, dim3(R.total), dim3(LO_THREADS), 0, (hipStream_t)stream, params, grads, m, v,
+                       blk_seg, blk_begin, blk_end, seg_first_blk, blk_partial, nblk, seg_norm2, step_count, adam_t, lr_state, R, *hp);
+  IMM_CHECK_LAUNCH("imm_opt_update");
+  return 0;
+}
+
 extern "C" int imm_clip_adam_step(float* params, float* grads, float* m, float* v, const int32_t* blk_seg,
                                   const int32_t* blk_begin, const int32_t* blk_end, int nblk, int nseg,
                                   const int32_t* seg_first_blk, const float* seg_wd, float* blk_partial, float* seg_norm2,
diff --git a/imm_amd/engine.py b/imm_amd/engine.py
--- a/imm_amd/engine.py
+++ b/imm_amd/engine.py
@@ -21,6 +21,7 @@
               ('conv5_1', 512, 512), ('conv5_2', 512, 512)]
 VGG_POOL_AFTER = ('conv1_2', 'conv2_2', 'conv3_3', 'conv4_3')
 WGRAD_MULTI_MAX_JOBS, WGRAD_MULTI_MAX_VARIANTS = 64, 16
+SHADOW_FUSE_SLABS = 8
 
 
 def plan_wgrad_chunks(groups, max_jobs, max_slots):
@@ -573,6 +574,8 @@
                 self._reduce_jobs.append((job, lay.k * lay.kw * lay.ci_real * lay.co))
         multi = ops.WgradMulti(multi_jobs, self.dt)
         self._wgrad_multis = getattr(self, '_wgrad_multis', []) + [multi]
+        self._wgrad_issued = getattr(self, '_wgrad_issued', []) + [
+            (len(self.prog_bwd), multi, [(m[0], m[5]) for _gk, members in chunk for m in members], self._cur_lane, cus)]
         self._cur_scope = name
         self._add(self.prog_bwd, lambda: ops.conv2d_wgrad_multi(multi), 'conv_wgrad', flops_total, name=name)
 
@@ -871,6 +874,93 @@
                                                             self.adam_t, self.lr_state, self.hp, self.loss_scale_state),
                   'clip_adam', 0.0, self.tab.total * 36.0)
         self.prog_opt.extend(self.prog_pack)
+        self._build_shadow()
+
+    def _build_shadow(self):
+        self.prog_shadow = None
+        issued = getattr(self, '_wgrad_issued', [])
+        if (os.environ.get('IMM_OPT_SHADOW', '0') == '0' or self.world_size != 1 or self.loss_scale_state is not None or self.f32
+                or len(issued) != 1 or self.tab.CHUNK > ops.OPT_MAX_CHUNK):
+            return
+        at, multi, lays, lane, cus = issued[0]
+        tail = [l for l in self.prog_bwd[at:] if l.fn is not None]
+        if lane != 0 or cus or [l.tag for l in tail] != ['conv_wgrad', 'wgrad_reduce'] or len(self.prog_bwd) != at + 2:
+            return
+        pos = ops.conv2d_wgrad_multi_launches(multi)
+        n_launch = max(pos) + 1
+        if n_launch < 2:
+            return
+        names = [n for n, _s, _w in self.spec]
+        first, offs = list(self.tab.first_host), self.tab.offsets
+        seg_of_job = [names.index(lay.scope + '/w') for lay, _f in lays]
+        per_launch = [sum(offs[s_ + 1] - offs[s_] for s_, p in zip(seg_of_job, pos) if p == l) for l in range(n_launch)]
+        k = int(os.environ.get('IMM_OPT_SHADOW_FORK', '0'))
+        if k <= 0:
+            k = 1
+            while sum(per_launch[:k]) < 0.5 * sum(per_launch):
+                k += 1
+        k = min(k, n_launch - 1)
+        seg_b = set(s_ for s_, p in zip(seg_of_job, pos) if p >= k)
+
+        def ranges(segs):
+            out = []
+            for s_ in segs:
+                if out and out[-1][1] == first[s_]:
+                    out[-1][1] = first[s_ + 1]
+                else:
+                    out.append([first[s_], first[s_ + 1]])
+            return out
+        part_segs = [[s_ for s_ in range(self.tab.nseg) if (s_ in seg_b) == b] for b in (False, True)]
+        parts = [ranges(segs) for segs in part_segs]
+        if any(len(r) > ops.OPT_MAX_RANGES for r in parts):
+            return
+        seg_of_g = {self.grads.data_ptr() + 4 * o: i for i, o in enumerate(offs[:-1])}
+        seg_of_w = {self.params.data_ptr() + 4 * o: i for i, o in enumerate(offs[:-1])}
+        fused = [(j, n) for j, n in self._reduce_jobs if j[2] <= SHADOW_FUSE_SLABS]
+        self.seg_red = ops.seg_reduce_table(self.tab, [j for j, _n in fused], self.grads.data_ptr(), self.dev)
+        slab_bytes = [0.0] * self.tab.nseg
+        for j, _n in self._reduce_jobs:
+            slab_bytes[seg_of_g[j[1]]] = 4.0 * j[2] * j[7] * j[6]
+        self.shadow_parts, self.shadow_fork = [], k
+        prog = list(self.prog_bwd[:at])
+        old = (getattr(self, '_cur_lane', 0), getattr(self, '_cur_scope', ''))
+        self._cur_lane, self._cur_scope = 0, 'all layers'
+        self._add(prog, lambda: ops.conv2d_wgrad_multi_part(multi, 0, k), 'conv_wgrad', sum(f for (_l, f), p in zip(lays, pos) if p < k),
+                  name='all layers [launches 0..%d]' % (k - 1))
+        self._mark(prog, 'fork', lane=3)
+        for b, (rng, segs) in enumerate(zip(parts, part_segs)):
+            n_el = float(sum(offs[s_ + 1] - offs[s_] for s_ in segs))
+            jobs = [j for j, _n in self._pack_jobs if (seg_of_w[j[0]] in seg_b) == bool(b)]
+            ptab = ops.pack_table(jobs, self.dev)
+            many = [(j, n) for j, n in self._reduce_jobs if j[2] > SHADOW_FUSE_SLABS and (seg_of_g[j[1]] in seg_b) == bool(b)]
+            rtab = ops.reduce_table([j for j, _n in many], [n for _j, n in many], self.dev) if many else None
+            self.shadow_parts.append((rng, ptab, segs, rtab))
+            self._cur_lane, self._cur_scope = (3, 'optimizer part A') if b == 0 else (0, 'optimizer part B')
+            if b == 1:
+                self._add(prog, lambda: ops.conv2d_wgrad_multi_part(multi, k, n_launch), 'conv_wgrad',
+                          sum(f for (_l, f), p in zip(lays, pos) if p >= k), name='all layers [launches %d..%d]' % (k, n_launch - 1))
+                self._mark(prog, 'join', lane=3)
+                prog.append(_Launch(None, 'phase:opt'))
+            many_bytes = sum(slab_bytes[seg_of_g[j[1]]] for j, _n in many)
+            if rtab is not None:
+                self._add(prog, (lambda rtab=rtab: ops.wgrad_reduce_multi(rtab)), 'wgrad_reduce', 0.0,
+                          many_bytes + 4.0 * sum(n for _j, n in many))
+            self._add(prog, (lambda rng=rng, b=b: ops.opt_reduce_prepare(self.params, self.grads, self.tab, self.seg_red,
+                                                                         self.opt_blk_partial, rng, b == 0, self.step_count,
+                                                                         self.adam_t, self.lr_state, self.hp)),
+                      'opt_reduce_prepare', 0.0, sum(slab_bytes[s_] for s_ in segs) - many_bytes + n_el * 8.0)
+            self._add(prog, (lambda rng=rng, b=b: ops.opt_update(self.params, self.grads, self.adam_m, self.adam_v, self.tab,
+                                                                 self.opt_blk_partial, self.seg_norm2, self.step_count, self.adam_t,
+                                                                 self.lr_state, self.hp, rng, b == 1)),
+                      'clip_adam', 0.0, n_el * 28.0)
+            self._add(prog, (lambda ptab=ptab: ops.pack_weights_multi(ptab, self.dt)), 'pack', 0.0,
+                      sum(4.0 * j[3] * j[4] * j[5] * j[6] + self.params.new_empty(0, dtype=self.dt).element_size() * j[8] * j[9]
+                          for j in jobs))
+        self._cur_lane, self._cur_scope = old
+        self.prog_shadow = prog
+
+    def step_programs(self):
+        return [self.prog_shadow] if self.prog_shadow is not None else [self.prog_bwd, self.prog_opt]
 
     def _pack_vgg(self):
         if not self.vgg_layers:
@@ -1130,6 +1220,8 @@
                 stamp(0, 'join: lane 0 arrives' if l.lane == 1 else 'join%d: lane 0 arrives' % l.lane)
                 ev = torch.cuda.Event(); ev.record(lane_stream(l.lane)); main.wait_event(ev)
                 stamp(0, 'join: lane 0 resumes' if l.lane == 1 else 'join%d: lane 0 resumes' % l.lane)
+            elif l.tag.startswith('phase:'):
+                stamp(0, 'end'); pname = l.tag[6:]; stamp(0, 'start')
             elif l.tag.startswith('record:'):
                 stamp(l.lane, l.tag)
                 ev = torch.cuda.Event(); ev.record(lane_stream(l.lane)); events[l.tag[7:]] = ev
@@ -1197,6 +1289,10 @@
     def backward(self):
         self.run(self.prog_bwd)
 
+    def backward_and_update(self):
+        for prog in self.step_programs():
+            self.run(prog)
+
     def snapshot(self):
         return {'params': self.params.clone(), 'm': self.adam_m.clone(), 'v': self.adam_v.clone(),
                 'step': self.step_count.clone(), 'adam_t': self.adam_t.clone(), 'agg': self.loss_agg.clone(), 'grads': self.grads.clone(), 'cost_ema': self.cost_ema.clone(),
diff --git a/imm_amd/ops.py b/imm_amd/ops.py
--- a/imm_amd/ops.py
+++ b/imm_amd/ops.py
@@ -213,6 +213,16 @@
 
 def conv2d_wgrad_multi(multi):
     call('imm_conv2d_wgrad_multi', C.cast(multi.host, C.c_void_p), _p(multi.dev), _s())
+
+
+def conv2d_wgrad_multi_part(multi, l0, l1):
+    call('imm_conv2d_wgrad_multi_part', C.cast(multi.host, C.c_void_p), _p(multi.dev), int(l0), int(l1), _s())
+
+
+def conv2d_wgrad_multi_launches(multi):
+    pos = (C.c_int32 * multi.n)()
+    call('imm_conv2d_wgrad_multi_launches', C.cast(multi.host, C.c_void_p), C.cast(pos, C.c_void_p), multi.n)
+    return [int(x) for x in pos]
 
 
 def conv2d_wgrad_splits(desc, lddy):
@@ -562,6 +572,43 @@
          _p(adam_t), _p(lr_state), C.byref(hp), _p(loss_scale_state), _s())
 
 
+OPT_MAX_RANGES, OPT_MAX_CHUNK = 32, 2048
+
+
+def seg_reduce_table(tab, jobs, base, device):
+    rows = [[0] * 12 for _ in range(tab.nseg)]
+    seg_of = {int(base) + 4 * o: i for i, o in enumerate(tab.offsets[:-1])}
+    for j in jobs:
+        lanes = 1
+        while lanes < min(16, int(j[2])):
+            lanes *= 2
+        s = seg_of[int(j[1])]
+        if int(j[3]) * int(j[5]) * int(j[6]) != tab.offsets[s + 1] - tab.offsets[s]:
+            raise ValueError('reduce job of tensor %d: %d x %d x %d outputs, the tensor has %d elements' % (
+                s, j[3], j[5], j[6], tab.offsets[s + 1] - tab.offsets[s]))
+        rows[s] = [int(x) for x in j[:8]] + [lanes, 0, 0, 0]
+    return torch.tensor(rows, dtype=torch.int64, device=device)
+
+
+def _ranges(ranges):
+    flat = [int(x) for r in ranges for x in r]
+    return (C.c_int32 * len(flat))(*flat), len(flat) // 2
+
+
+def opt_reduce_prepare(params, grads, tab, seg_red, blk_partial, ranges, compute_lr, step_count, adam_t, lr_state, hp):
+    arr, n = _ranges(ranges)
+    call('imm_opt_reduce_prepare', _p(params), _p(grads), _p(tab.blk_seg), _p(tab.blk_begin), _p(tab.blk_end), tab.nblk, tab.nseg,
+         _p(tab.seg_first_blk), C.cast(tab.first_host, C.c_void_p), _p(tab.seg_wd), _p(seg_red), _p(blk_partial),
+         C.cast(arr, C.c_void_p), n, int(bool(compute_lr)), _p(step_count), _p(adam_t), _p(lr_state), C.byref(hp), _s())
+
+
+def opt_update(params, grads, m, v, tab, blk_partial, seg_norm2, step_count, adam_t, lr_state, hp, ranges, advance):
+    arr, n = _ranges(ranges)
+    call('imm_opt_update', _p(params), _p(grads), _p(m), _p(v), _p(tab.blk_seg), _p(tab.blk_begin), _p(tab.blk_end), tab.nblk,
+         tab.nseg, _p(tab.seg_first_blk), C.cast(tab.first_host, C.c_void_p), _p(blk_partial), _p(seg_norm2), _p(step_count),
+         _p(adam_t), _p(lr_state), C.byref(hp), C.cast(arr, C.c_void_p), n, int(bool(advance)), _s())
+
+
 class SegmentTable:
     CHUNK = 2048
 
@@ -583,6 +630,7 @@
         self.blk_begin = torch.tensor(blk_begin, **i32)
         self.blk_end = torch.tensor(blk_end, **i32)
         self.seg_first_blk = torch.tensor(first, **i32)
+        self.first_host = (C.c_int32 * len(first))(*first)
         self.seg_wd = torch.tensor([float(w) for w in wds], dtype=torch.float32, device=device)
 
 
diff --git a/imm_amd/train/cnn_train_multi.py b/imm_amd/train/cnn_train_multi.py
--- a/imm_amd/train/cnn_train_multi.py
+++ b/imm_amd/train/cnn_train_multi.py
@@ -117,6 +117,10 @@
                 snap0 = eng.snapshot(); self._poison(); eng.restore(snap0)
             snap = eng.snapshot()
             eng.forward(True); eng.backward(); eng.optimizer_step()
+            if not self.split and eng.prog_shadow is not None:
+                self.stream.synchronize()
+                eng.restore(snap)
+                eng.forward(True); eng.backward_and_update()
             self.stream.synchronize()
             eng.restore(snap)
             self.stream.synchronize()
@@ -151,7 +155,7 @@
             elif not self.split:
                 g = ops.Graph()
                 g.capture_begin()
-                eng.run(eng.prog_fwd); eng.run(eng.prog_bwd); eng.run(eng.prog_opt)
+                eng.run(eng.prog_fwd); eng.backward_and_update()
                 g.capture_end()
                 self._graphs = (g,)
             elif self.buckets < 2:
@@ -221,11 +225,14 @@
                     self._poison()
             else:
                 eng.forward(True)
-                eng.backward()
-                if self.after_backward is not None:
-                    self.after_backward(eng)
-                average_gradients(eng.grads, self.world_size, self.group)
-                eng.optimizer_step()
+                if not self.split and self.after_backward is None:
+                    eng.backward_and_update()
+                else:
+                    eng.backward()
+                    if self.after_backward is not None:
+                        self.after_backward(eng)
+                    average_gradients(eng.grads, self.world_size, self.group)
+                    eng.optimizer_step()
         torch.cuda.current_stream(eng.dev).wait_stream(self.stream)
         return eng.loss
 
diff --git a/include/imm_hip.h b/include/imm_hip.h
--- a/include/imm_hip.h
+++ b/include/imm_hip.h
@@ -7,7 +7,7 @@
 extern "C" {
 #endif
 
-#define IMM_ABI_VERSION 35
+#define IMM_ABI_VERSION 36
 
 enum imm_dtype { IMM_BF16 = 0, IMM_F16 = 1, IMM_F32 = 2 };
 
@@ -261,6 +261,7 @@
 
 
 
+
 int imm_crc32c(const void* data, uint64_t n, uint32_t* crc_inout);
 
 #ifdef __cplusplus
@@ -277,4 +278,5 @@
 #include "imm_hull.h"
 #include "imm_seam.h"
 #include "imm_clip.h"
+#include "imm_opt_parts.h"
 #endif
diff --git a/include/imm_opt_parts.h b/include/imm_opt_parts.h
--- /dev/null
+++ b/include/imm_opt_parts.h
@@ -0,0 +1,30 @@
+#ifndef IMM_OPT_PARTS_H
+#define IMM_OPT_PARTS_H
+
+#include <stdint.h>
+
+#ifdef __cplusplus
+extern "C" {
+#endif
+
+#define IMM_OPT_MAX_RANGES 32
+#define IMM_OPT_MAX_CHUNK 2048
+
+int imm_conv2d_wgrad_multi_part(const void* table_host, const void* table_dev, int l0, int l1, void* stream);
+int imm_conv2d_wgrad_multi_launches(const void* table_host, int32_t* job_launch_host, int n);
+
+int imm_opt_reduce_prepare(const float* params, float* grads, const int32_t* blk_seg, const int32_t* blk_begin,
+                           const int32_t* blk_end, int nblk, int nseg, const int32_t* seg_first_blk,
+                           const int32_t* seg_first_blk_host, const float* seg_wd, const int64_t* seg_red, float* blk_partial,
+                           const int32_t* ranges_host, int n_ranges, int compute_lr, const int32_t* step_count,
+                           const int32_t* adam_t, float* lr_state, const imm_opt_hparams* hp_host, void* stream);
+
+int imm_opt_update(float* params, const float* grads, float* m, float* v, const int32_t* blk_seg, const int32_t* blk_begin,
+                   const int32_t* blk_end, int nblk, int nseg, const int32_t* seg_first_blk, const int32_t* seg_first_blk_host,
+                   const float* blk_partial, float* seg_norm2, int32_t* step_count, int32_t* adam_t, const float* lr_state,
+                   const imm_opt_hparams* hp_host, const int32_t* ranges_host, int n_ranges, int advance, void* stream);
+
+#ifdef __cplusplus
+}
+#endif
+#endif
```

Measured after the change: 10310 images/s. Within noise of the previous version (-0.2%).
